# IGNF/MAESTRO

Hardware: AMD Instinct MI355X
Metric: MAE-pretrain tiles/sec (higher is better)
Workload: dtype bf16

## Files before the change

### __graft_entry__.py

```python

from __future__ import annotations

import os
import subprocess
import sys
from pathlib import Path

ROOT = Path(__file__).resolve().parent
if str(ROOT) not in sys.path:
    sys.path.insert(0, str(ROOT))


def build() -> None:
    from maestro_amd.csrc.build import build as build_lib
    from maestro_amd.csrc.build import build_example

    lib = build_lib(verbose=bool(os.environ.get("MAESTRO_BUILD_VERBOSE")))
    build_example()
    import ctypes

    import maestro_amd
    from maestro_amd import hip

    handle = ctypes.CDLL(str(lib))
    import re

    for name in ("maestro_hip.h", "maestro_hip_metrics.h", "maestro_hip_det.h"):
        header = (ROOT / "include" / name).read_text()
        missing = [n for n in re.findall(r"\b(mh_[a-z0-9_]+)\s*\(", header) if not hasattr(handle, n)]
        if missing:
            raise RuntimeError(f"libmaestro_hip.so lacks symbols declared in include/{name}: {sorted(set(missing))}")
    assert hip.lib().mh_version() >= 1


def smoke() -> None:
    import torch

    import maestro_amd.conf as conf
    from maestro_amd.ssl import mae as pmae
    from maestro_amd.train.optim import FusedAdamW
    from oracle import mae as om
    from oracle.gen_golden import build_datasets, case_table, init_weights, make_batch

    if not torch.cuda.is_available():
        raise RuntimeError("smoke() needs cuda:0")
    dev = torch.device("cuda:0")
    case = case_table()["c3_aerial_s2"]
    ds = build_datasets(case, conf)
    kw = dict(interpolate="nearest", model="mae", num_levels=1, fusion_mode=case["fusion"], inter_depth=case["inter_depth"],
              **case["model_kw"])
    oracle = om.build_oracle(ds, conf.MaskConfig(), model_size=case["size"], **kw)
    init_weights(oracle, case["seed"])
    model = getattr(pmae, f"mae_{case['size']}")(datasets=ds, mask=conf.MaskConfig(), **kw)
    model.load_state_dict(oracle.state_dict(), strict=True)
    batch = make_batch(ds.dataset, case["B"], case["seed"], stress=case.get("stress", False))
    eng = model.engine(case["B"], dev, loss="l2_norm")
    torch.manual_seed(7)
    noise, struct = eng.draw_masks()
    loss = eng.forward({k: v.to(dev) for k, v in batch.items()}, noise=noise, struct=struct)
    eng.zero_grad()
    eng.backward()
    pixels, masks = eng.reconstructions()
    ob, orec, omsk, _ = oracle({k: v.clone() for k, v in batch.items()}, "pretrain", noise=noise,
                               struct_masks={g: s[:, :, None] for g, s in struct.items()})
    want = om.compute_loss_rec(ob, orec, omsk, oracle.out_grid_size, om.norm_bands_of(ds.dataset), "l2_norm")
    got = float(loss.item())
    assert abs(got - want.item()) < 3e-3 * abs(want.item()), (got, want.item())
    for m in orec:
        assert torch.equal(masks[m].cpu(), omsk[m]), f"{m}: mask indices differ from the oracle"
        rel = ((pixels[m].cpu() - orec[m]).norm() / orec[m].norm()).item()
        assert rel < 1.3e-2, (m, rel)
    FusedAdamW(eng, 1e-3).step()
    loss2 = float(eng.forward({k: v.to(dev) for k, v in batch.items()}, noise=noise, struct=struct).item())
    assert loss2 < got, (loss2, got)
    print(f"smoke ok: loss hip={got:.6f} oracle={want.item():.6f}; after one AdamW step {loss2:.6f}")


if __name__ == "__main__":
    build()
    if "--smoke" in sys.argv:
        smoke()
```

### maestro_amd/csrc/build.py

```python

from __future__ import annotations

import hashlib
import os
import shutil
import subprocess
import sys
from concurrent.futures import ThreadPoolExecutor
from pathlib import Path

CSRC = Path(__file__).resolve().parent
ROOT = CSRC.parent.parent
LIB_DIR = CSRC.parent / "lib"
LIB = LIB_DIR / "libmaestro_hip.so"
OBJ_DIR = CSRC / "build"
ARCH = "gfx950"
FLAGS = ["-O3", "-std=c++17", "-fPIC", f"--offload-arch={ARCH}", "-Wno-unused-result"] + os.environ.get("MH_BUILD_FLAGS", "").split()
FILE_FLAGS = {"attn.hip": ["-mllvm", "-amdgpu-mfma-vgpr-form", "-fno-slp-vectorize"] + os.environ.get("MH_ATTN_FLAGS", "").split(),
              "gemm_sk.hip": ["-mllvm", "-amdgpu-mfma-vgpr-form"]}
NO_PK_F32 = ["-Xclang", "-target-feature", "-Xclang", "-packed-fp32-ops"]
for _f in ("gemm.hip", "gemm_pp.hip", "gemm_dma.hip"):
    FILE_FLAGS[_f] = FILE_FLAGS.get(_f, []) + NO_PK_F32


def _hipcc() -> str:
    for cand in (shutil.which("hipcc"), "/opt/rocm/bin/hipcc"):
        if cand and Path(cand).exists():
            return cand
    raise RuntimeError("hipcc not found; the MI355X kernels cannot be built")


def _digest(src: Path) -> str:
    h = hashlib.sha256()
    for f in [src, *sorted(CSRC.glob("*.hpp")), ROOT / "include" / "maestro_hip.h",
              ROOT / "include" / "maestro_hip_metrics.h", ROOT / "include" / "maestro_hip_det.h"]:
        h.update(f.read_bytes())
    h.update(" ".join(FLAGS + FILE_FLAGS.get(src.name, [])).encode())
    return h.hexdigest()[:16]


def build(force: bool = False, verbose: bool = False) -> Path:
    hipcc = _hipcc()
    OBJ_DIR.mkdir(exist_ok=True)
    LIB_DIR.mkdir(exist_ok=True)
    sources = sorted(CSRC.glob("*.hip"))
    jobs, objs = [], []
    for src in sources:
        obj = OBJ_DIR / f"{src.stem}.{_digest(src)}.o"
        objs.append(obj)
        if force or not obj.exists():
            for old in OBJ_DIR.glob(f"{src.stem}.*.o"):
                old.unlink()
            jobs.append((src, obj))

    def compile_one(job):
        src, obj = job
        cmd = [hipcc, *FLAGS, *FILE_FLAGS.get(src.name, []), "-c", str(src), "-o", str(obj)]
        if verbose:
            print(" ".join(cmd), flush=True)
        r = subprocess.run(cmd, capture_output=True, text=True)
        if r.returncode != 0:
            raise RuntimeError(f"hipcc failed for {src.name}:\n{r.stdout}\n{r.stderr}")
        return "\n".join(ln for ln in r.stderr.splitlines() if "'-packed-fp32-ops' is not a recognized feature" not in ln)

    if jobs:
        with ThreadPoolExecutor(max_workers=min(4, os.cpu_count() or 1)) as ex:
            for warn in ex.map(compile_one, jobs):
                if verbose and warn:
                    print(warn, file=sys.stderr)
    if jobs or not LIB.exists():
        cmd = [hipcc, "-shared", "-fPIC", f"--offload-arch={ARCH}", *map(str, objs), "-o", str(LIB)]
        r = subprocess.run(cmd, capture_output=True, text=True)
        if r.returncode != 0:
            raise RuntimeError(f"link failed:\n{r.stdout}\n{r.stderr}")
    return LIB


EXAMPLE_SRC = ROOT / "examples" / "abi_smoke.cpp"
EXAMPLE_BIN = ROOT / "examples" / "abi_smoke"


def build_example(force: bool = False) -> Path:
    if not force and EXAMPLE_BIN.exists() and EXAMPLE_BIN.stat().st_mtime >= max(EXAMPLE_SRC.stat().st_mtime, LIB.stat().st_mtime):
        return EXAMPLE_BIN
    cmd = [_hipcc(), "-O2", "-std=c++17", f"--offload-arch={ARCH}", str(EXAMPLE_SRC), f"-I{ROOT / 'include'}", f"-L{LIB_DIR}",
           "-lmaestro_hip", "-Wl,-rpath,$ORIGIN/../maestro_amd/lib", "-o", str(EXAMPLE_BIN)]
    r = subprocess.run(cmd, capture_output=True, text=True)
    if r.returncode != 0:
        raise RuntimeError(f"building examples/abi_smoke failed:\n{r.stdout}\n{r.stderr}")
    return EXAMPLE_BIN


if __name__ == "__main__":
    print(build(force="--force" in sys.argv, verbose=True))
    print(build_example(force="--force" in sys.argv))
```

### maestro_amd/csrc/loss.hip

```cpp
#include "gemm_common.hpp"
#include "../../include/maestro_hip_det.h"

namespace {

template <bool DET>
__global__ __launch_bounds__(256) void masked_loss_kernel(const float* __restrict__ rec, const float* __restrict__ target,
                                                          const uint8_t* __restrict__ mask_group, const int* __restrict__ n_masked,
                                                          float weight, float* __restrict__ acc, bf16_t* __restrict__ drec,
                                                          int B, int Lm, int Lgroup, int tok_off, int PPC, int p, int tgt_C,
                                                          int tgt_c0, int n_g, int denom_is_elems, int rows_per_wave) {
    __shared__ float red[4];
    const int w = threadIdx.x >> 6, lane = threadIdx.x & 63;
    const float coef = weight / (denom_is_elems ? (float)(*n_masked) : (float)(*n_masked) * (float)PPC);
    const bool window = n_g != tgt_C;
    const int tgt_ld = window ? PPC / n_g * tgt_C : PPC;
    float s = 0.f;
    for (int rr = 0; rr < rows_per_wave; ++rr) {
        const int row = (blockIdx.x * 4 + w) * rows_per_wave + rr;
        if (row >= B * Lm) break;
        const int b = row / Lm, t = row - b * Lm;
        const bool masked = mask_group[(size_t)b * Lgroup + tok_off + t] != 0;
        const float* r = rec + (size_t)row * PPC;
        const float* g = target + (size_t)row * tgt_ld;
        bf16_t* d = drec ? drec + (size_t)row * PPC : nullptr;
        for (int c = lane * 4; c < PPC; c += 256) {
            float dd[4] = {0.f, 0.f, 0.f, 0.f};
            if (masked) {
                const f32x4 rv = *reinterpret_cast<const f32x4*>(r + c);
                f32x4 tv;
                if (!window) {
                    tv = *reinterpret_cast<const f32x4*>(g + c);
                } else {
#pragma unroll
                    for (int e = 0; e < 4; ++e) { const int pix = (c + e) / n_g; tv[e] = g[pix * tgt_C + tgt_c0 + (c + e) - pix * n_g]; }
                }
#pragma unroll
                for (int e = 0; e < 4; ++e) {
                    const float diff = rv[e] - tv[e];
                    if (p == 2) { s += diff * diff; dd[e] = 2.f * diff * coef; }
                    else { s += fabsf(diff); dd[e] = (diff > 0.f ? coef : (diff < 0.f ? -coef : 0.f)); }
                }
            }
            if (d) {
                u32x2 pk = {pack_bf2(dd[0], dd[1]), pack_bf2(dd[2], dd[3])};
                *reinterpret_cast<u32x2*>(d + c) = pk;
            }
        }
    }
    s = wave_sum(s);
    if (lane == 0) red[w] = s;
    __syncthreads();
    if (threadIdx.x == 0) {
        const float t = (red[0] + red[1]) + (red[2] + red[3]);
        if constexpr (DET) {
            acc[blockIdx.x] = (blockIdx.x == 0 && *n_masked == 0) ? __builtin_nanf("") : t * coef;
        } else {
        if (t != 0.f) atomicAdd(acc, t * coef);
        if (blockIdx.x == 0 && *n_masked == 0) atomicAdd(acc, __builtin_nanf(""));
        }
    }
}

template <bool DET>
__global__ __launch_bounds__(1024) void colsum_kernel(const void* __restrict__ x, int is_f32, float* __restrict__ out, int M,
                                                      int N, int ld, int rows_per_block) {
    __shared__ f32x4 red[16][64];
    const int w = threadIdx.x >> 6, lane = threadIdx.x & 63, nw = blockDim.x >> 6;
    const int c = (blockIdx.x * 64 + lane) * 4;
    const int r0 = blockIdx.y * rows_per_block, r1 = min(M, r0 + rows_per_block);
    f32x4 acc = {0, 0, 0, 0};
    if (c < N) {
        if (is_f32) {
#pragma unroll 8
            for (int r = r0 + w; r < r1; r += nw)
                acc += *reinterpret_cast<const f32x4*>(reinterpret_cast<const float*>(x) + (size_t)r * ld + c);
        } else {
#pragma unroll 8
            for (int r = r0 + w; r < r1; r += nw) {
                const u32x2 pk = *reinterpret_cast<const u32x2*>(reinterpret_cast<const bf16_t*>(x) + (size_t)r * ld + c);
                acc += (f32x4){__uint_as_float(pk[0] << 16), __uint_as_float(pk[0] & 0xffff0000u),
                               __uint_as_float(pk[1] << 16), __uint_as_float(pk[1] & 0xffff0000u)};
            }
        }
    }
    red[w][lane] = acc;
    __syncthreads();
    if (w == 0 && c < N) {
        f32x4 t = red[0][lane];
        for (int i = 1; i < nw; ++i) t += red[i][lane];
        if constexpr (DET) {
            *reinterpret_cast<f32x4*>(out + (size_t)blockIdx.y * N + c) = t;
        } else {
#pragma unroll
        for (int e = 0; e < 4; ++e) atomicAdd(out + c + e, t[e]);
        }
    }
}

__global__ __launch_bounds__(256) void zero_spans_kernel(float* __restrict__ base, const long* __restrict__ spans) {
    const long off = spans[2 * blockIdx.y], len = spans[2 * blockIdx.y + 1];
    for (long i = ((long)blockIdx.x * 256 + threadIdx.x) * 4; i < len; i += (long)gridDim.x * 1024) {
        float* p = base + off + i;
        if (i + 3 < len && (reinterpret_cast<uintptr_t>(p) & 15) == 0) *reinterpret_cast<f32x4*>(p) = (f32x4){0, 0, 0, 0};
        else for (long e = i; e < min(len, i + 4); ++e) base[off + e] = 0.f;
    }
}

__global__ __launch_bounds__(256) void cast_bf16_kernel(const float* __restrict__ src, bf16_t* __restrict__ dst, long n) {
    const long i = ((long)blockIdx.x * 256 + threadIdx.x) * 4;
    if (i + 3 < n) {
        const f32x4 v = *reinterpret_cast<const f32x4*>(src + i);
        u32x2 pk = {pack_bf2(v[0], v[1]), pack_bf2(v[2], v[3])};
        *reinterpret_cast<u32x2*>(dst + i) = pk;
    } else {
        for (long j = i; j < n; ++j) dst[j] = f2bf(src[j]);
    }
}

__global__ __launch_bounds__(256) void pack_rows_kernel(const float* __restrict__ w, bf16_t* __restrict__ dst, int E, int K, int Kpad) {
    const long i = (long)blockIdx.x * 256 + threadIdx.x;
    if (i >= (long)E * Kpad) return;
    const int e = i / Kpad, k = i - (long)e * Kpad;
    dst[i] = k < K ? f2bf(w[(size_t)e * K + k]) : (bf16_t)0;
}

__global__ __launch_bounds__(256) void unpack_rows_add_kernel(const float* __restrict__ src, float* __restrict__ dst, int E, int K, int Kpad) {
    const long i = (long)blockIdx.x * 256 + threadIdx.x;
    if (i >= (long)E * K) return;
    const int e = i / K, k = i - (long)e * K;
    atomicAdd(dst + i, src[(size_t)e * Kpad + k]);
}

struct Fp8Shadow { uint8_t* p8; const short* slot_map; const float* scale; float* amax; };

__device__ __forceinline__ int adamw_update(float* __restrict__ p, const float* __restrict__ g, float* __restrict__ m,
                                             float* __restrict__ v, bf16_t* __restrict__ pb, long n, float lr, float b1, float b2,
                                             float eps, float wd, float bc1, float bc2_sqrt, float gscale,
                                             Fp8Shadow f8 = Fp8Shadow{nullptr, nullptr, nullptr, nullptr},
                                             float* amax_out = nullptr) {
    const long i = ((long)blockIdx.x * 256 + threadIdx.x) * 4;
    if (i >= n) return -1;
    const f32x4 gv = __builtin_nontemporal_load(reinterpret_cast<const f32x4*>(g + i)) * gscale;
    f32x4 pv = __builtin_nontemporal_load(reinterpret_cast<const f32x4*>(p + i));
    f32x4 mv = __builtin_nontemporal_load(reinterpret_cast<const f32x4*>(m + i));
    f32x4 vv = __builtin_nontemporal_load(reinterpret_cast<const f32x4*>(v + i));
#pragma unroll
    for (int e = 0; e < 4; ++e) {
        pv[e] *= 1.f - lr * wd;
        mv[e] = b1 * mv[e] + (1.f - b1) * gv[e];
        vv[e] = b2 * vv[e] + (1.f - b2) * gv[e] * gv[e];
        const float denom = sqrtf(vv[e]) / bc2_sqrt + eps;
        pv[e] -= (lr / bc1) * (mv[e] / denom);
    }
    __builtin_nontemporal_store(pv, reinterpret_cast<f32x4*>(p + i));
    __builtin_nontemporal_store(mv, reinterpret_cast<f32x4*>(m + i));
    __builtin_nontemporal_store(vv, reinterpret_cast<f32x4*>(v + i));
    if (pb) {
        u32x2 pk = {pack_bf2(pv[0], pv[1]), pack_bf2(pv[2], pv[3])};
        __builtin_nontemporal_store(pk, reinterpret_cast<u32x2*>(pb + i));
    }
    if (f8.p8) {
        const int slot = f8.slot_map[i >> 6];
        if (slot >= 0) {
            const float s8 = f8.scale[slot];
            float mx = 0.f;
#pragma unroll
            for (int e = 0; e < 4; ++e) mx = amax_fold(mx, pv[e]);
            __builtin_nontemporal_store(pack_e4m3x4(pv, s8), reinterpret_cast<uint32_t*>(f8.p8 + i));
            *amax_out = mx;
            return slot;
        }
    }
    return -1;
}
__global__ __launch_bounds__(256) void adamw_kernel(float* __restrict__ p, const float* __restrict__ g, float* __restrict__ m,
                                                    float* __restrict__ v, bf16_t* __restrict__ pb, long n, float lr, float b1,
                                                    float b2, float eps, float wd, float bc1, float bc2_sqrt, float gscale) {
    adamw_update(p, g, m, v, pb, n, lr, b1, b2, eps, wd, bc1, bc2_sqrt, gscale);
}
__global__ __launch_bounds__(256) void adamw_fp8_kernel(float* __restrict__ p, const float* __restrict__ g, float* __restrict__ m,
                                                        float* __restrict__ v, bf16_t* __restrict__ pb, long n, float lr, float b1,
                                                        float b2, float eps, float wd, float bc1, float bc2_sqrt, float gscale,
                                                        Fp8Shadow f8) {
    __shared__ float red_mx[4];
    __shared__ int red_slot[4];
    float mx = 0.f;
    const int slot = adamw_update(p, g, m, v, pb, n, lr, b1, b2, eps, wd, bc1, bc2_sqrt, gscale, f8, &mx);
    const int w = threadIdx.x >> 6;
    const int slot0 = __builtin_amdgcn_readfirstlane(slot);
    const bool uniform = __all(slot == slot0);
    if (uniform) {
        mx = wave_amax(mx);
    } else if (slot >= 0 && amax_nonzero(mx)) {
        atomic_max_pos(f8.amax + (size_t)slot * MH_FP8_AMAX_PITCH, mx);
    }
    if ((threadIdx.x & 63) == 0) { red_mx[w] = uniform ? mx : 0.f; red_slot[w] = uniform ? slot0 : -1; }
    __syncthreads();
    if (threadIdx.x == 0) {
        if (red_slot[0] == red_slot[1] && red_slot[0] == red_slot[2] && red_slot[0] == red_slot[3]) {
            const float m4 = amax_fold(amax_fold(amax_fold(red_mx[0], red_mx[1]), red_mx[2]), red_mx[3]);
            if (red_slot[0] >= 0 && amax_nonzero(m4)) atomic_max_pos(f8.amax + (size_t)red_slot[0] * MH_FP8_AMAX_PITCH, m4);
        } else {
            for (int k = 0; k < 4; ++k)
                if (red_slot[k] >= 0 && amax_nonzero(red_mx[k])) atomic_max_pos(f8.amax + (size_t)red_slot[k] * MH_FP8_AMAX_PITCH, red_mx[k]);
        }
    }
}
__global__ __launch_bounds__(256) void adamw_dev_kernel(float* __restrict__ p, const float* __restrict__ g, float* __restrict__ m,
                                                        float* __restrict__ v, bf16_t* __restrict__ pb, long n, float b1, float b2,
                                                        float eps, float wd, const float* __restrict__ hyper) {
    if (hyper[4] == 0.f) return;
    adamw_update(p, g, m, v, pb, n, hyper[0], b1, b2, eps, wd, hyper[1], hyper[2], hyper[3]);
}

__global__ __launch_bounds__(256) void scale_dev_kernel(float* __restrict__ x, long n, const float* __restrict__ scale) {
    const float s = *scale;
    if (s == 1.f) return;
    const long i = ((long)blockIdx.x * 256 + threadIdx.x) * 4;
    if (i + 4 <= n) {
        *reinterpret_cast<f32x4*>(x + i) = *reinterpret_cast<const f32x4*>(x + i) * s;
    } else {
        for (long j = i; j < n; ++j) x[j] *= s;
    }
}

}

static int loss_rows_per_wave(long rows) { return (int)std::min(16L, std::max(1L, rows / 4096)); }

extern "C" int mh_scale_dev(float* x, long n, const float* scale, void* stream) {
    MH_CHECK_ARG(x && scale && n > 0 && ((uintptr_t)x % 16) == 0, "mh_scale_dev: bad arguments (x 16-byte aligned)");
    hipLaunchKernelGGL(scale_dev_kernel, dim3(ceil_div(n, 1024)), dim3(256), 0, (hipStream_t)stream, x, n, scale);
    MH_LAUNCH_CHECK();
    return 0;
}

extern "C" int mh_masked_loss(const float* rec, const float* target, const uint8_t* mask_group, const int* n_masked,
                              float weight, float* acc, void* drec, int B, int Lm, int Lgroup, int tok_off, int PPC, int p,
                              void* stream) {
    MH_CHECK_ARG(rec && target && mask_group && n_masked && acc, "mh_masked_loss: null pointer");
    MH_CHECK_ARG((p == 1 || p == 2) && PPC % 4 == 0 && tok_off + Lm <= Lgroup, "mh_masked_loss: bad arguments");
    const int rpw = loss_rows_per_wave((long)B * Lm);
    hipLaunchKernelGGL(masked_loss_kernel<false>, dim3(ceil_div((long)B * Lm, 4 * rpw)), dim3(256), 0, (hipStream_t)stream, rec, target, mask_group, n_masked,
                       weight, acc, (bf16_t*)drec, B, Lm, Lgroup, tok_off, PPC, p, 1, 0, 1, 0, rpw);
    MH_LAUNCH_CHECK();
    return 0;
}

extern "C" int mh_masked_loss_bands(const float* rec, const float* target, const uint8_t* mask_group, const int* n_elems,
                                    float weight, float* acc, void* drec, int B, int Lm, int Lgroup, int tok_off, int PPC, int p,
                                    int tgt_C, int tgt_c0, int n_g, void* stream) {
    MH_CHECK_ARG(rec && target && mask_group && n_elems && acc, "mh_masked_loss_bands: null pointer");
    MH_CHECK_ARG((p == 1 || p == 2) && PPC % 4 == 0 && tok_off + Lm <= Lgroup, "mh_masked_loss_bands: bad arguments");
    MH_CHECK_ARG(n_g > 0 && PPC % n_g == 0 && tgt_c0 >= 0 && tgt_c0 + n_g <= tgt_C, "mh_masked_loss_bands: band window [%d, %d) of %d",
                 tgt_c0, tgt_c0 + n_g, tgt_C);
    const int rpw = loss_rows_per_wave((long)B * Lm);
    hipLaunchKernelGGL(masked_loss_kernel<false>, dim3(ceil_div((long)B * Lm, 4 * rpw)), dim3(256), 0, (hipStream_t)stream, rec, target, mask_group, n_elems,
                       weight, acc, (bf16_t*)drec, B, Lm, Lgroup, tok_off, PPC, p, tgt_C, tgt_c0, n_g, 1, rpw);
    MH_LAUNCH_CHECK();
    return 0;
}

extern "C" int mh_masked_loss_partial_size(int B, int Lm) {
    const long rows = (long)B * Lm;
    return rows > 0 ? ceil_div(rows, 4 * loss_rows_per_wave(rows)) : 0;
}

extern "C" int mh_masked_loss_det(const float* rec, const float* target, const uint8_t* mask_group, const int* n_masked,
                                  float weight, float* loss_partial, void* drec, int B, int Lm, int Lgroup, int tok_off, int PPC,
                                  int p, void* stream) {
    MH_CHECK_ARG(rec && target && mask_group && n_masked && loss_partial, "mh_masked_loss_det: null pointer");
    MH_CHECK_ARG(B > 0 && Lm > 0 && (p == 1 || p == 2) && PPC % 4 == 0 && tok_off + Lm <= Lgroup, "mh_masked_loss_det: bad arguments");
    const int rpw = loss_rows_per_wave((long)B * Lm);
    hipLaunchKernelGGL(masked_loss_kernel<true>, dim3(ceil_div((long)B * Lm, 4 * rpw)), dim3(256), 0, (hipStream_t)stream, rec, target,
                       mask_group, n_masked, weight, loss_partial, (bf16_t*)drec, B, Lm, Lgroup, tok_off, PPC, p, 1, 0, 1, 0, rpw);
    MH_LAUNCH_CHECK();
    return 0;
}

extern "C" int mh_masked_loss_bands_det(const float* rec, const float* target, const uint8_t* mask_group, const int* n_elems,
                                        float weight, float* loss_partial, void* drec, int B, int Lm, int Lgroup, int tok_off,
                                        int PPC, int p, int tgt_C, int tgt_c0, int n_g, void* stream) {
    MH_CHECK_ARG(rec && target && mask_group && n_elems && loss_partial, "mh_masked_loss_bands_det: null pointer");
    MH_CHECK_ARG(B > 0 && Lm > 0 && (p == 1 || p == 2) && PPC % 4 == 0 && tok_off + Lm <= Lgroup, "mh_masked_loss_bands_det: bad arguments");
    MH_CHECK_ARG(n_g > 0 && PPC % n_g == 0 && tgt_c0 >= 0 && tgt_c0 + n_g <= tgt_C, "mh_masked_loss_bands_det: band window [%d, %d) of %d",
                 tgt_c0, tgt_c0 + n_g, tgt_C);
    const int rpw = loss_rows_per_wave((long)B * Lm);
    hipLaunchKernelGGL(masked_loss_kernel<true>, dim3(ceil_div((long)B * Lm, 4 * rpw)), dim3(256), 0, (hipStream_t)stream, rec, target,
                       mask_group, n_elems, weight, loss_partial, (bf16_t*)drec, B, Lm, Lgroup, tok_off, PPC, p, tgt_C, tgt_c0, n_g, 1, rpw);
    MH_LAUNCH_CHECK();
    return 0;
}

extern "C" int mh_colsum_partial_rows(int M) { return M > 0 ? ceil_div(M, MH_COLSUM_PARTIAL_ROWS) : 0; }

extern "C" int mh_colsum_partial(const void* x, int x_is_f32, float* partial, int M, int N, int ld, void* stream) {
    MH_CHECK_ARG(x && partial && ((uintptr_t)partial % 16) == 0, "mh_colsum_partial: null pointer / partial not 16-byte aligned");
    MH_CHECK_ARG(M > 0 && N > 0 && N % 4 == 0 && ld % 4 == 0 && N <= ld, "mh_colsum_partial: bad sizes M=%d N=%d ld=%d", M, N, ld);
    hipLaunchKernelGGL(colsum_kernel<true>, dim3(ceil_div(N, 256), ceil_div(M, MH_COLSUM_PARTIAL_ROWS)), dim3(1024), 0,
                       (hipStream_t)stream, x, x_is_f32, partial, M, N, ld, MH_COLSUM_PARTIAL_ROWS);
    MH_LAUNCH_CHECK();
    return 0;
}

extern "C" int mh_colsum(const void* x, int x_is_f32, float* out, int M, int N, int ld, void* stream) {
    MH_CHECK_ARG(x && out && N % 4 == 0 && ld % 4 == 0, "mh_colsum: bad arguments");
    const int col_blocks = ceil_div(N, 256);
    int rows_per_block = 1024;
    while (rows_per_block > 128 && (long)col_blocks * ceil_div(M, rows_per_block) < 128) rows_per_block >>= 1;
    hipLaunchKernelGGL(colsum_kernel<false>, dim3(col_blocks, ceil_div(M, rows_per_block)), dim3(1024), 0, (hipStream_t)stream, x,
                       x_is_f32, out, M, N, ld, rows_per_block);
    MH_LAUNCH_CHECK();
    return 0;
}

extern "C" int mh_zero_spans(float* base, const long* spans_device, int n_spans, long max_len, void* stream) {
    MH_CHECK_ARG(base && spans_device && n_spans > 0 && max_len > 0, "mh_zero_spans: bad arguments");
    dim3 grid((unsigned)min(64L, (max_len + 1023) / 1024), n_spans);
    hipLaunchKernelGGL(zero_spans_kernel, grid, dim3(256), 0, (hipStream_t)stream, base, spans_device);
    MH_LAUNCH_CHECK();
    return 0;
}

extern "C" int mh_cast_bf16(const float* src, void* dst, long n, void* stream) {
    MH_CHECK_ARG(src && dst && n > 0, "mh_cast_bf16: bad arguments");
    hipLaunchKernelGGL(cast_bf16_kernel, dim3(ceil_div(n, 1024)), dim3(256), 0, (hipStream_t)stream, src, (bf16_t*)dst, n);
    MH_LAUNCH_CHECK();
    return 0;
}

extern "C" int mh_pack_rows_bf16(const float* w, void* dst, int E, int K, int Kpad, void* stream) {
    MH_CHECK_ARG(w && dst && Kpad >= K, "mh_pack_rows_bf16: bad arguments");
    hipLaunchKernelGGL(pack_rows_kernel, dim3(ceil_div((long)E * Kpad, 256)), dim3(256), 0, (hipStream_t)stream, w, (bf16_t*)dst, E, K, Kpad);
    MH_LAUNCH_CHECK();
    return 0;
}

extern "C" int mh_unpack_rows_add(const float* src, float* dst, int E, int K, int Kpad, void* stream) {
    MH_CHECK_ARG(src && dst && Kpad >= K, "mh_unpack_rows_add: bad arguments");
    hipLaunchKernelGGL(unpack_rows_add_kernel, dim3(ceil_div((long)E * K, 256)), dim3(256), 0, (hipStream_t)stream, src, dst, E, K, Kpad);
    MH_LAUNCH_CHECK();
    return 0;
}

extern "C" int mh_adamw(float* p, const float* g, float* m, float* v, void* p_bf16, long n, float lr, float b1, float b2,
                        float eps, float wd, int step, float grad_scale, void* stream) {
    MH_CHECK_ARG(p && g && m && v && n > 0 && n % 4 == 0 && step >= 1, "mh_adamw: bad arguments (n %% 4 == 0, step >= 1)");
    const float bc1 = 1.f - powf(b1, (float)step);
    const float bc2_sqrt = sqrtf(1.f - powf(b2, (float)step));
    hipLaunchKernelGGL(adamw_kernel, dim3(ceil_div(n, 1024)), dim3(256), 0, (hipStream_t)stream, p, g, m, v, (bf16_t*)p_bf16, n, lr,
                       b1, b2, eps, wd, bc1, bc2_sqrt, grad_scale);
    MH_LAUNCH_CHECK();
    return 0;
}

extern "C" int mh_adamw_fp8(float* p, const float* g, float* m, float* v, void* p_bf16, void* p_fp8, const short* slot_map,
                            const float* scale, float* amax, long n, float lr, float b1, float b2, float eps, float wd, int step,
                            float grad_scale, void* stream) {
    MH_CHECK_ARG(p && g && m && v && n > 0 && n % 4 == 0 && step >= 1, "mh_adamw_fp8: bad arguments (n %% 4 == 0, step >= 1)");
    MH_CHECK_ARG(p_fp8 && slot_map && scale && amax && ((uintptr_t)p_fp8 % 4) == 0, "mh_adamw_fp8: fp8 shadow, slot map, scale and amax tables are required");
    const float bc1 = 1.f - powf(b1, (float)step);
    const float bc2_sqrt = sqrtf(1.f - powf(b2, (float)step));
    hipLaunchKernelGGL(adamw_fp8_kernel, dim3(ceil_div(n, 1024)), dim3(256), 0, (hipStream_t)stream, p, g, m, v, (bf16_t*)p_bf16, n, lr,
                       b1, b2, eps, wd, bc1, bc2_sqrt, grad_scale, Fp8Shadow{(uint8_t*)p_fp8, slot_map, scale, amax});
    MH_LAUNCH_CHECK();
    return 0;
}

extern "C" int mh_adamw_dev(float* p, const float* g, float* m, float* v, void* p_bf16, long n, float b1, float b2, float eps,
                            float wd, const float* hyper, void* stream) {
    MH_CHECK_ARG(p && g && m && v && hyper && n > 0 && n % 4 == 0, "mh_adamw_dev: bad arguments (n %% 4 == 0)");
    hipLaunchKernelGGL(adamw_dev_kernel, dim3(ceil_div(n, 1024)), dim3(256), 0, (hipStream_t)stream, p, g, m, v, (bf16_t*)p_bf16,
                       n, b1, b2, eps, wd, hyper);
    MH_LAUNCH_CHECK();
    return 0;
}
```

### maestro_amd/csrc/mask.hip

```cpp
#include "common.hpp"
#include "../../include/maestro_hip.h"

namespace {

__global__ __launch_bounds__(1024) void mask_select_kernel(const float* __restrict__ noise, const uint8_t* __restrict__ smask,
                                                          int* __restrict__ visible_idx, int* __restrict__ masked_idx,
                                                          int* __restrict__ inv, uint8_t* __restrict__ mask, int L, int k) {
    extern __shared__ __attribute__((aligned(16))) float sm[];
    const int L4 = (L + 3) & ~3;
    int* wtot = reinterpret_cast<int*>(sm + L4);
    const int b = blockIdx.x, lane = threadIdx.x & 63, w = threadIdx.x >> 6;
    for (int i = threadIdx.x; i < L4; i += 1024) {
        float v = INFINITY;
        if (i < L) {
            v = noise[(size_t)b * L + i];
            if (smask && smask[(size_t)b * L + i]) v = 0.f;
        }
        sm[i] = v;
    }
    __syncthreads();
    int base = 0;
    for (int i0 = 0; i0 < L; i0 += 1024) {
        const int i = i0 + threadIdx.x;
        int f = 0;
        if (i < L) {
            const float v = sm[i];
            int r = 0;
            for (int j = 0; j < L4; j += 4) {
                const f32x4 u = *reinterpret_cast<const f32x4*>(sm + j);
                r += (int)((u[0] < v) | ((u[0] == v) & (j < i)));
                r += (int)((u[1] < v) | ((u[1] == v) & (j + 1 < i)));
                r += (int)((u[2] < v) | ((u[2] == v) & (j + 2 < i)));
                r += (int)((u[3] < v) | ((u[3] == v) & (j + 3 < i)));
            }
            f = r < k;
        }
        const unsigned long long bal = __ballot(f);
        const int before = __popcll(bal & ((1ull << lane) - 1ull));
        __syncthreads();
        if (lane == 0) wtot[w] = __popcll(bal);
        __syncthreads();
        int nm = base + before, tot = 0;
#pragma unroll
        for (int x = 0; x < 16; ++x) {
            const int c = wtot[x];
            nm += x < w ? c : 0;
            tot += c;
        }
        base += tot;
        if (i < L) {
            mask[(size_t)b * L + i] = (uint8_t)f;
            if (f) {
                masked_idx[(size_t)b * k + nm] = i;
                inv[(size_t)b * L + i] = -1;
            } else {
                visible_idx[(size_t)b * (L - k) + (i - nm)] = i;
                inv[(size_t)b * L + i] = i - nm;
            }
        }
    }
}

__global__ __launch_bounds__(256) void gather_rows_kernel(const float* __restrict__ src, const int* __restrict__ idx,
                                                          float* __restrict__ dst, int B, int src_L, int n_idx, int dim,
                                                          int dst_L, int dst_off) {
    const int row = blockIdx.x * 4 + (threadIdx.x >> 6), lane = threadIdx.x & 63;
    if (row >= B * n_idx) return;
    const int b = row / n_idx, j = row - b * n_idx;
    const float* s = src + ((size_t)b * src_L + idx[row]) * dim;
    float* d = dst + ((size_t)b * dst_L + dst_off + j) * dim;
    for (int c = lane * 4; c < dim; c += 256) *reinterpret_cast<f32x4*>(d + c) = *reinterpret_cast<const f32x4*>(s + c);
}

__global__ __launch_bounds__(256) void scatter_rows_kernel(const float* __restrict__ ddst, const int* __restrict__ idx,
                                                           float* __restrict__ dsrc, int B, int src_L, int n_idx, int dim,
                                                           int dst_L, int dst_off) {
    const int row = blockIdx.x * 4 + (threadIdx.x >> 6), lane = threadIdx.x & 63;
    if (row >= B * n_idx) return;
    const int b = row / n_idx, j = row - b * n_idx;
    float* s = dsrc + ((size_t)b * src_L + idx[row]) * dim;
    const float* d = ddst + ((size_t)b * dst_L + dst_off + j) * dim;
    for (int c = lane * 4; c < dim; c += 256) *reinterpret_cast<f32x4*>(s + c) = *reinterpret_cast<const f32x4*>(d + c);
}

__global__ __launch_bounds__(256) void expand_rows_kernel(const float* __restrict__ src, const int* __restrict__ inv,
                                                          float* __restrict__ dst, int B, int L, int n, int dim) {
    const int row = blockIdx.x * 4 + (threadIdx.x >> 6), lane = threadIdx.x & 63;
    if (row >= B * L) return;
    const int b = row / L, iv = inv[row];
    float* o = dst + (size_t)row * dim;
    const float* s = src + ((size_t)b * n + (iv < 0 ? 0 : iv)) * dim;
    for (int c = lane * 4; c < dim; c += 256) {
        f32x4 v = {0.f, 0.f, 0.f, 0.f};
        if (iv >= 0) v = *reinterpret_cast<const f32x4*>(s + c);
        *reinterpret_cast<f32x4*>(o + c) = v;
    }
}

__global__ __launch_bounds__(256) void unmask_kernel(const float* __restrict__ y, const int* __restrict__ inv,
                                                     const float* __restrict__ mask_token, const int* __restrict__ tok_slot,
                                                     const float* __restrict__ pos, const float* __restrict__ date,
                                                     const int* __restrict__ date_row, int n_date_rows,
                                                     float* __restrict__ xdec, int B, int L, int n_vis, int Dd, int slot_stride) {
    const int row = blockIdx.x * 4 + (threadIdx.x >> 6), lane = threadIdx.x & 63;
    if (row >= B * L) return;
    const int b = row / L, t = row - b * L;
    const int iv = inv[row];
    const float* s = iv < 0 ? mask_token + (size_t)tok_slot[(size_t)b * slot_stride + t] * Dd : y + ((size_t)b * n_vis + iv) * Dd;
    const float* pr = pos + (size_t)t * Dd;
    const float* dr = date ? date + ((size_t)b * n_date_rows + date_row[t]) * 8 : nullptr;
    float* o = xdec + (size_t)row * Dd;
    for (int c = lane * 4; c < Dd; c += 256) {
        f32x4 v = *reinterpret_cast<const f32x4*>(s + c) + *reinterpret_cast<const f32x4*>(pr + c);
        if (dr && c >= Dd - 8) v += *reinterpret_cast<const f32x4*>(dr + (c - (Dd - 8)));
        *reinterpret_cast<f32x4*>(o + c) = v;
    }
}

constexpr int UM_ROWS = 512, UM_NT = 1024;
template <bool DET>
__global__ __launch_bounds__(UM_NT) void unmask_bwd_token_kernel(const float* __restrict__ dxdec, const uint8_t* __restrict__ mask,
                                                                 const int* __restrict__ tok_slot, float* __restrict__ dmask_token,
                                                                 int B, int L, int Dd, int slot, int t_lo, int t_hi, int slot_stride) {
    __shared__ __attribute__((aligned(16))) float red[UM_NT * 4];
    __shared__ int row_off[UM_ROWS];
    const int span = t_hi - t_lo, total = B * span;
    const int cols = Dd >> 2, lanes = UM_NT / cols;
    const int col = threadIdx.x % cols, sub = threadIdx.x / cols;
    const int r0 = blockIdx.x * UM_ROWS;
    for (int rr = threadIdx.x; rr < UM_ROWS; rr += UM_NT) {
        const int r = r0 + rr;
        int off = -1;
        if (r < total) {
            const int b = r / span, t = t_lo + (r - b * span);
            if (mask[(size_t)b * L + t] && tok_slot[(size_t)b * slot_stride + t] == slot) off = b * L + t;
        }
        row_off[rr] = off;
    }
    __syncthreads();
    f32x4 acc = {0, 0, 0, 0};
    if (sub < lanes) {
#pragma unroll 2
        for (int rr = sub; rr < UM_ROWS; rr += 4 * lanes) {
            f32x4 v[4];
#pragma unroll
            for (int u = 0; u < 4; ++u) {
                v[u] = (f32x4){0, 0, 0, 0};
                const int ri = rr + u * lanes;
                const int off = ri < UM_ROWS ? row_off[ri] : -1;
                if (off >= 0) v[u] = *reinterpret_cast<const f32x4*>(dxdec + (size_t)off * Dd + 4 * col);
            }
            acc += (v[0] + v[1]) + (v[2] + v[3]);
        }
    }
    *reinterpret_cast<f32x4*>(red + 4 * threadIdx.x) = acc;
    __syncthreads();
    if (sub == 0) {
        for (int s = 1; s < lanes; ++s) acc += *reinterpret_cast<const f32x4*>(red + 4 * (s * cols + col));
        if constexpr (DET) {
            *reinterpret_cast<f32x4*>(dmask_token + (size_t)blockIdx.x * Dd + 4 * col) = acc;
        } else {
#pragma unroll
        for (int e = 0; e < 4; ++e) if (acc[e] != 0.f) atomicAdd(dmask_token + 4 * col + e, acc[e]);
        }
    }
}

__global__ __launch_bounds__(1024) void count_masked_kernel(const uint8_t* __restrict__ mask, int B, int L, int t_lo, int t_hi,
                                                            int* __restrict__ out, int mult, int accumulate) {
    __shared__ float red[16];
    const int span = t_hi - t_lo, w = threadIdx.x >> 6, lane = threadIdx.x & 63;
    float c = 0.f;
    for (int b = w; b < B; b += 16) {
        const uint8_t* row = mask + (size_t)b * L + t_lo;
        for (int t = lane; t < span; t += 64) c += row[t] ? 1.f : 0.f;
    }
    c = block_sum<16>(c, red);
    if (threadIdx.x == 0) *out = (accumulate ? *out : 0) + (int)(c + 0.5f) * mult;
}

}

extern "C" int mh_mask_select(const float* noise, const uint8_t* struct_mask, int* visible_idx, int* masked_idx, int* inv,
                              uint8_t* mask, int B, int L, int k, void* stream) {
    MH_CHECK_ARG(noise && visible_idx && masked_idx && inv && mask, "mh_mask_select: null pointer");
    MH_CHECK_ARG(B > 0 && L > 0 && k >= 0 && k <= L && L <= 8192, "mh_mask_select: bad sizes B=%d L=%d k=%d", B, L, k);
    hipLaunchKernelGGL(mask_select_kernel, dim3(B), dim3(1024), (size_t)((L + 3) & ~3) * 4 + 64, (hipStream_t)stream, noise, struct_mask,
                       visible_idx, masked_idx, inv, mask, L, k);
    MH_LAUNCH_CHECK();
    return 0;
}

extern "C" int mh_gather_rows(const float* src, const int* idx, float* dst, int B, int src_L, int n_idx, int dim, int dst_L,
                              int dst_off, void* stream) {
    MH_CHECK_ARG(src && idx && dst && dim % 4 == 0 && dst_off + n_idx <= dst_L, "mh_gather_rows: bad arguments");
    hipLaunchKernelGGL(gather_rows_kernel, dim3(ceil_div((long)B * n_idx, 4)), dim3(256), 0, (hipStream_t)stream, src, idx, dst, B,
                       src_L, n_idx, dim, dst_L, dst_off);
    MH_LAUNCH_CHECK();
    return 0;
}

extern "C" int mh_scatter_rows(const float* ddst, const int* idx, float* dsrc, int B, int src_L, int n_idx, int dim,
                               int dst_L, int dst_off, void* stream) {
    MH_CHECK_ARG(ddst && idx && dsrc && dim % 4 == 0 && dst_off + n_idx <= dst_L, "mh_scatter_rows: bad arguments");
    hipLaunchKernelGGL(scatter_rows_kernel, dim3(ceil_div((long)B * n_idx, 4)), dim3(256), 0, (hipStream_t)stream, ddst, idx, dsrc,
                       B, src_L, n_idx, dim, dst_L, dst_off);
    MH_LAUNCH_CHECK();
    return 0;
}

extern "C" int mh_expand_rows(const float* src, const int* inv, float* dst, int B, int L, int n, int dim, void* stream) {
    MH_CHECK_ARG(src && inv && dst && B > 0 && L > 0 && n > 0 && dim % 4 == 0, "mh_expand_rows: bad arguments");
    hipLaunchKernelGGL(expand_rows_kernel, dim3(ceil_div((long)B * L, 4)), dim3(256), 0, (hipStream_t)stream, src, inv, dst, B, L,
                       n, dim);
    MH_LAUNCH_CHECK();
    return 0;
}

extern "C" int mh_unmask_assemble(const float* y, const int* inv, const float* mask_token, const int* tok_slot,
                                  const float* pos, const float* date, const int* date_row, int n_date_rows, float* xdec,
                                  int B, int L, int n_vis, int Dd, void* stream) {
    MH_CHECK_ARG(y && inv && mask_token && tok_slot && pos && xdec && Dd % 4 == 0 && Dd >= 8, "mh_unmask_assemble: bad arguments");
    MH_CHECK_ARG(!date || date_row, "mh_unmask_assemble: date without date_row");
    hipLaunchKernelGGL(unmask_kernel, dim3(ceil_div((long)B * L, 4)), dim3(256), 0, (hipStream_t)stream, y, inv, mask_token,
                       tok_slot, pos, date, date_row, n_date_rows, xdec, B, L, n_vis, Dd, 0);
    MH_LAUNCH_CHECK();
    return 0;
}

extern "C" int mh_unmask_assemble_per_sample(const float* y, const int* inv, const float* mask_token, const int* tok_slot_bl,
                                             const float* pos, const float* date, const int* date_row, int n_date_rows,
                                             float* xdec, int B, int L, int n_vis, int Dd, void* stream) {
    MH_CHECK_ARG(y && inv && mask_token && tok_slot_bl && pos && xdec && Dd % 4 == 0 && Dd >= 8, "mh_unmask_assemble_per_sample: bad arguments");
    MH_CHECK_ARG(!date || date_row, "mh_unmask_assemble_per_sample: date without date_row");
    hipLaunchKernelGGL(unmask_kernel, dim3(ceil_div((long)B * L, 4)), dim3(256), 0, (hipStream_t)stream, y, inv, mask_token,
                       tok_slot_bl, pos, date, date_row, n_date_rows, xdec, B, L, n_vis, Dd, L);
    MH_LAUNCH_CHECK();
    return 0;
}

extern "C" int mh_unmask_token_grad(const float* dxdec, const uint8_t* mask, const int* tok_slot, float* dmask_token, int B,
                                    int L, int Dd, int slot, int t_lo, int t_hi, void* stream) {
    MH_CHECK_ARG(dxdec && mask && tok_slot && dmask_token && Dd % 4 == 0 && Dd <= 1024, "mh_unmask_token_grad: bad arguments");
    MH_CHECK_ARG(0 <= t_lo && t_lo < t_hi && t_hi <= L, "mh_unmask_token_grad: bad token range");
    hipLaunchKernelGGL(unmask_bwd_token_kernel<false>, dim3(ceil_div((long)B * (t_hi - t_lo), UM_ROWS)), dim3(UM_NT), 0,
                       (hipStream_t)stream, dxdec, mask, tok_slot, dmask_token, B, L, Dd, slot, t_lo, t_hi, 0);
    MH_LAUNCH_CHECK();
    return 0;
}

extern "C" int mh_unmask_token_grad_per_sample(const float* dxdec, const uint8_t* mask, const int* tok_slot_bl, float* dmask_token,
                                               int B, int L, int Dd, int slot, void* stream) {
    MH_CHECK_ARG(dxdec && mask && tok_slot_bl && dmask_token && Dd % 4 == 0 && Dd <= 1024 && B > 0 && L > 0,
                 "mh_unmask_token_grad_per_sample: bad arguments");
    hipLaunchKernelGGL(unmask_bwd_token_kernel<false>, dim3(ceil_div((long)B * L, UM_ROWS)), dim3(UM_NT), 0, (hipStream_t)stream, dxdec, mask,
                       tok_slot_bl, dmask_token, B, L, Dd, slot, 0, L, L);
    MH_LAUNCH_CHECK();
    return 0;
}

extern "C" int mh_unmask_token_grad_partial_rows(long n_rows) { return n_rows > 0 ? ceil_div(n_rows, UM_ROWS) : 0; }

extern "C" int mh_unmask_token_grad_det(const float* dxdec, const uint8_t* mask, const int* tok_slot, float* partial, int B, int L,
                                        int Dd, int slot, int t_lo, int t_hi, void* stream) {
    MH_CHECK_ARG(dxdec && mask && tok_slot && partial && ((uintptr_t)partial % 16) == 0 && B > 0 && Dd > 0 && Dd % 4 == 0 && Dd <= 1024,
                 "mh_unmask_token_grad_det: bad arguments");
    MH_CHECK_ARG(0 <= t_lo && t_lo < t_hi && t_hi <= L, "mh_unmask_token_grad_det: bad token range");
    hipLaunchKernelGGL(unmask_bwd_token_kernel<true>, dim3(ceil_div((long)B * (t_hi - t_lo), UM_ROWS)), dim3(UM_NT), 0,
                       (hipStream_t)stream, dxdec, mask, tok_slot, partial, B, L, Dd, slot, t_lo, t_hi, 0);
    MH_LAUNCH_CHECK();
    return 0;
}

extern "C" int mh_unmask_token_grad_per_sample_det(const float* dxdec, const uint8_t* mask, const int* tok_slot_bl, float* partial,
                                                   int B, int L, int Dd, int slot, void* stream) {
    MH_CHECK_ARG(dxdec && mask && tok_slot_bl && partial && ((uintptr_t)partial % 16) == 0 && Dd > 0 && Dd % 4 == 0 && Dd <= 1024 &&
                 B > 0 && L > 0, "mh_unmask_token_grad_per_sample_det: bad arguments");
    hipLaunchKernelGGL(unmask_bwd_token_kernel<true>, dim3(ceil_div((long)B * L, UM_ROWS)), dim3(UM_NT), 0, (hipStream_t)stream, dxdec,
                       mask, tok_slot_bl, partial, B, L, Dd, slot, 0, L, L);
    MH_LAUNCH_CHECK();
    return 0;
}

extern "C" int mh_count_masked_elems(const uint8_t* mask, int B, int L, int t_lo, int t_hi, int* out, int mult, int accumulate,
                                     void* stream) {
    MH_CHECK_ARG(mask && out && 0 <= t_lo && t_lo < t_hi && t_hi <= L && mult > 0, "mh_count_masked_elems: bad arguments");
    hipLaunchKernelGGL(count_masked_kernel, dim3(1), dim3(1024), 0, (hipStream_t)stream, mask, B, L, t_lo, t_hi, out, mult,
                       accumulate);
    MH_LAUNCH_CHECK();
    return 0;
}

extern "C" int mh_count_masked(const uint8_t* mask, int B, int L, int t_lo, int t_hi, int* out, void* stream) {
    MH_CHECK_ARG(mask && out && 0 <= t_lo && t_lo < t_hi && t_hi <= L, "mh_count_masked: bad arguments");
    hipLaunchKernelGGL(count_masked_kernel, dim3(1), dim3(1024), 0, (hipStream_t)stream, mask, B, L, t_lo, t_hi, out, 1, 0);
    MH_LAUNCH_CHECK();
    return 0;
}
```

### maestro_amd/csrc/norm.hip

```cpp
#include "gemm_common.hpp"

namespace {

struct RowMap { int L, off; };
__device__ __forceinline__ size_t map_row(RowMap m, int b, int j) { return (size_t)b * m.L + m.off + j; }

template <int NV>
__global__ __launch_bounds__(256) void ln_fwd_kernel(const float* __restrict__ x, RowMap xm, const float* __restrict__ gamma,
                                                     const float* __restrict__ beta, void* __restrict__ y, RowMap ym,
                                                     int y_is_f32, float* __restrict__ mean, float* __restrict__ rstd,
                                                     int B, int n, int dim, float eps, uint8_t* __restrict__ y8,
                                                     const float* __restrict__ y8_scale, float* __restrict__ y8_amax,
                                                     uint8_t* __restrict__ y8s, int ld_y8s) {
    const int row = blockIdx.x * 4 + (threadIdx.x >> 6);
    const int lane = threadIdx.x & 63;
    if (row >= B * n) return;
    const int b = row / n, j = row - b * n;
    const float* xr = x + map_row(xm, b, j) * dim;
    const int nv = dim >> 2;
    f32x4 v[NV];
    float s = 0.f;
#pragma unroll
    for (int i = 0; i < NV; ++i) {
        const int c = lane + 64 * i;
        v[i] = (f32x4){0, 0, 0, 0};
        if (c < nv) v[i] = *reinterpret_cast<const f32x4*>(xr + 4 * c);
        s += (v[i][0] + v[i][1]) + (v[i][2] + v[i][3]);
    }
    const float mu = wave_sum(s) / dim;
    float q = 0.f;
#pragma unroll
    for (int i = 0; i < NV; ++i) {
        if (lane + 64 * i < nv) {
#pragma unroll
            for (int e = 0; e < 4; ++e) { const float d = v[i][e] - mu; q += d * d; }
        }
    }
    const float rs = rsqrtf(wave_sum(q) / dim + eps);
    if (lane == 0) { mean[row] = mu; rstd[row] = rs; }
    const size_t yrow = map_row(ym, b, j) * dim;
    const bool t8 = y8 && !y8s;
    const float s8 = t8 ? *y8_scale : 0.f;
    float amax8 = 0.f;
#pragma unroll
    for (int i = 0; i < NV; ++i) {
        const int c = lane + 64 * i;
        u32x2 pk16 = {0u, 0u};
        if (c < nv) {
            const f32x4 g = *reinterpret_cast<const f32x4*>(gamma + 4 * c);
            const f32x4 bt = *reinterpret_cast<const f32x4*>(beta + 4 * c);
            f32x4 o;
#pragma unroll
            for (int e = 0; e < 4; ++e) o[e] = (v[i][e] - mu) * rs * g[e] + bt[e];
            if (y_is_f32) {
                *reinterpret_cast<f32x4*>(reinterpret_cast<float*>(y) + yrow + 4 * c) = o;
            } else {
                u32x2 pk = {pack_bf2(o[0], o[1]), pack_bf2(o[2], o[3])};
                *reinterpret_cast<u32x2*>(reinterpret_cast<bf16_t*>(y) + yrow + 4 * c) = pk;
                pk16 = pk;
            }
            if (t8) {
#pragma unroll
                for (int e = 0; e < 4; ++e) amax8 = amax_fold(amax8, o[e]);
                *reinterpret_cast<uint32_t*>(y8 + yrow + 4 * c) = pack_e4m3x4(o, s8);
            }
        }
        if (y8s) {
            const f32x4 q = bf2x2_to_f32x4(pk16[0], pk16[1]);
            float a = 0.f;
#pragma unroll
            for (int e = 0; e < 4; ++e) a = amax_fold(a, q[e]);
            const uint32_t sbyte = mx_scale_byte(group_amax<8>(a));
            if (c < nv) {
                *reinterpret_cast<uint32_t*>(y8 + yrow + 4 * c) = pack_e4m3x4(q, mx_inv_scale(sbyte));
                if ((lane & 7) == 0) y8s[map_row(ym, b, j) * ld_y8s + (c >> 3)] = (uint8_t)sbyte;
            }
        }
    }
    if (t8 && y8_amax) {
        amax8 = wave_amax(amax8);
        if (lane == 0 && amax_nonzero(amax8)) atomic_max_pos(y8_amax, amax8);
    }
}

#ifndef MH_LN_FAST
#define MH_LN_FAST 1
#endif
#ifndef MH_LN_DPP
#define MH_LN_DPP 1
#endif
__device__ __forceinline__ float ln_wave_sum(float v) {
#if MH_LN_DPP
#define MH_ROR(n) __builtin_bit_cast(float, __builtin_amdgcn_update_dpp(0, __builtin_bit_cast(int, v), 0x120 + (n), 0xf, 0xf, false))
    v += MH_ROR(8); v += MH_ROR(4); v += MH_ROR(2); v += MH_ROR(1);
#undef MH_ROR
    const int iv = __builtin_bit_cast(int, v);
    const float r0 = __builtin_bit_cast(float, __builtin_amdgcn_readlane(iv, 0)), r1 = __builtin_bit_cast(float, __builtin_amdgcn_readlane(iv, 16));
    const float r2 = __builtin_bit_cast(float, __builtin_amdgcn_readlane(iv, 32)), r3 = __builtin_bit_cast(float, __builtin_amdgcn_readlane(iv, 48));
    return (r0 + r1) + (r2 + r3);
#else
    return wave_sum(v);
#endif
}
enum { LN_Y8_NONE = 0, LN_Y8_TENSOR = 1, LN_Y8_MX = 2 };
template <int NV, int Y8>
__device__ __forceinline__ void ln_fwd_fast_body(const float* __restrict__ x, RowMap xm, const float* __restrict__ gamma,
                                                          const float* __restrict__ beta, bf16_t* __restrict__ y, RowMap ym,
                                                          float* __restrict__ mean, float* __restrict__ rstd, int B, int n,
                                                          float eps, uint8_t* __restrict__ y8, const float* __restrict__ y8_scale,
                                                          float* __restrict__ y8_amax, uint8_t* __restrict__ y8s, int ld_y8s) {
    constexpr int dim = 256 * NV;
    constexpr bool FP8 = Y8 == LN_Y8_TENSOR;
    const int row = blockIdx.x * 4 + __builtin_amdgcn_readfirstlane(threadIdx.x >> 6);
    const int lane = threadIdx.x & 63;
    if (row >= B * n) return;
    const int b = row / n, j = row - b * n;
    const float* xr = x + map_row(xm, b, j) * dim;
    f32x4 v[NV], g[NV], bt[NV];
#pragma unroll
    for (int i = 0; i < NV; ++i) v[i] = *reinterpret_cast<const f32x4*>(xr + 4 * (lane + 64 * i));
#pragma unroll
    for (int i = 0; i < NV; ++i) {
        g[i] = *reinterpret_cast<const f32x4*>(gamma + 4 * (lane + 64 * i));
        bt[i] = *reinterpret_cast<const f32x4*>(beta + 4 * (lane + 64 * i));
    }
    float s = 0.f;
#pragma unroll
    for (int i = 0; i < NV; ++i) s += (v[i][0] + v[i][1]) + (v[i][2] + v[i][3]);
    const float mu = ln_wave_sum(s) / dim;
    float q = 0.f;
#pragma unroll
    for (int i = 0; i < NV; ++i) {
#pragma unroll
        for (int e = 0; e < 4; ++e) { const float d = v[i][e] - mu; q += d * d; }
    }
    const float rs = rsqrtf(ln_wave_sum(q) / dim + eps);
    const size_t yrow = map_row(ym, b, j) * dim;
    bf16_t* yr = y + yrow;
    float s8 = 0.f;
    if constexpr (FP8) s8 = *y8_scale;
    float amax8 = 0.f;
#pragma unroll
    for (int i = 0; i < NV; ++i) {
        f32x4 o;
#pragma unroll
        for (int e = 0; e < 4; ++e) o[e] = (v[i][e] - mu) * rs * g[i][e] + bt[i][e];
        const u32x2 pk = {pack_bf2(o[0], o[1]), pack_bf2(o[2], o[3])};
        *reinterpret_cast<u32x2*>(yr + 4 * (lane + 64 * i)) = pk;
        if constexpr (Y8 == LN_Y8_MX) {
            const f32x4 q = bf2x2_to_f32x4(pk[0], pk[1]);
            float a = 0.f;
#pragma unroll
            for (int e = 0; e < 4; ++e) a = amax_fold(a, q[e]);
            const uint32_t sbyte = mx_scale_byte(group_amax<8>(a));
            *reinterpret_cast<uint32_t*>(y8 + yrow + 4 * (lane + 64 * i)) = pack_e4m3x4(q, mx_inv_scale(sbyte));
            if ((lane & 7) == 0) y8s[map_row(ym, b, j) * ld_y8s + ((lane + 64 * i) >> 3)] = (uint8_t)sbyte;
        }
        if constexpr (FP8) {
#pragma unroll
            for (int e = 0; e < 4; ++e) amax8 = amax_fold(amax8, o[e]);
            *reinterpret_cast<uint32_t*>(y8 + yrow + 4 * (lane + 64 * i)) = pack_e4m3x4(o, s8);
        }
    }
    if (lane == 0) { mean[row] = mu; rstd[row] = rs; }
    if constexpr (FP8) {
        if (y8_amax) {
            amax8 = wave_amax(amax8);
            if (lane == 0 && amax_nonzero(amax8)) atomic_max_pos(y8_amax, amax8);
        }
    }
}
template <int NV, bool FP8>
__global__ __launch_bounds__(256) void ln_fwd_fast_kernel(const float* __restrict__ x, RowMap xm, const float* __restrict__ gamma,
                                                          const float* __restrict__ beta, bf16_t* __restrict__ y, RowMap ym,
                                                          float* __restrict__ mean, float* __restrict__ rstd, int B, int n,
                                                          float eps, uint8_t* __restrict__ y8, const float* __restrict__ y8_scale,
                                                          float* __restrict__ y8_amax) {
    ln_fwd_fast_body<NV, FP8 ? LN_Y8_TENSOR : LN_Y8_NONE>(x, xm, gamma, beta, y, ym, mean, rstd, B, n, eps, y8, y8_scale, y8_amax,
                                                          nullptr, 0);
}
template <int NV>
__global__ __launch_bounds__(256) void ln_fwd_fast_mx_kernel(const float* __restrict__ x, RowMap xm, const float* __restrict__ gamma,
                                                             const float* __restrict__ beta, bf16_t* __restrict__ y, RowMap ym,
                                                             float* __restrict__ mean, float* __restrict__ rstd, int B, int n,
                                                             float eps, uint8_t* __restrict__ y8, uint8_t* __restrict__ y8s,
                                                             int ld_y8s) {
    ln_fwd_fast_body<NV, LN_Y8_MX>(x, xm, gamma, beta, y, ym, mean, rstd, B, n, eps, y8, nullptr, nullptr, y8s, ld_y8s);
}

#ifndef LN_ROWS
#define LN_ROWS 4
#endif
constexpr int ROWS_PER_WAVE = LN_ROWS;

template <int NV>
__global__ __launch_bounds__(256) void ln_bwd_kernel(const void* __restrict__ dy, RowMap dym, int dy_is_f32,
                                                     const float* __restrict__ x, RowMap xm,
                                                     const float* __restrict__ gamma, const float* __restrict__ mean,
                                                     const float* __restrict__ rstd, const float* __restrict__ dres,
                                                     float* __restrict__ dx, bf16_t* __restrict__ dx_bf16,
                                                     float* __restrict__ partial, int B, int n, int dim) {
    extern __shared__ __attribute__((aligned(16))) float red[];
    const int w = threadIdx.x >> 6, lane = threadIdx.x & 63;
    const int nv = dim >> 2;
    f32x4 gsum[NV], bsum[NV], csum[NV], gm[NV];
#pragma unroll
    for (int i = 0; i < NV; ++i) {
        gsum[i] = (f32x4){0, 0, 0, 0}; bsum[i] = (f32x4){0, 0, 0, 0}; csum[i] = (f32x4){0, 0, 0, 0};
        const int c = lane + 64 * i;
        gm[i] = c < nv ? *reinterpret_cast<const f32x4*>(gamma + 4 * c) : (f32x4){0, 0, 0, 0};
    }
    const int row0 = (blockIdx.x * 4 + w) * ROWS_PER_WAVE;
    const int rows = B * n;
    f32x4 xv_n[NV], rs_n[NV];
    u32x4 dy_n[NV];
    float mu_n = 0.f, rstd_n = 0.f;
    size_t xrow_n = 0;
    auto fetch = [&](int row) {
        const int b = row / n, j = row - b * n;
        xrow_n = map_row(xm, b, j) * dim;
        const size_t dyrow = map_row(dym, b, j) * dim;
        mu_n = mean[row]; rstd_n = rstd[row];
#pragma unroll
        for (int i = 0; i < NV; ++i) {
            const int c = lane + 64 * i;
            if (c < nv) {
                xv_n[i] = *reinterpret_cast<const f32x4*>(x + xrow_n + 4 * c);
                if (dy_is_f32) {
                    dy_n[i] = *reinterpret_cast<const u32x4*>(reinterpret_cast<const float*>(dy) + dyrow + 4 * c);
                } else {
                    const u32x2 pk = *reinterpret_cast<const u32x2*>(reinterpret_cast<const bf16_t*>(dy) + dyrow + 4 * c);
                    dy_n[i] = (u32x4){pk[0], pk[1], 0u, 0u};
                }
                rs_n[i] = dres ? *reinterpret_cast<const f32x4*>(dres + xrow_n + 4 * c) : (f32x4){0, 0, 0, 0};
            }
        }
    };
    if (row0 < rows) fetch(row0);
    for (int rr = 0; rr < ROWS_PER_WAVE; ++rr) {
        const int row = row0 + rr;
        if (row >= rows) break;
        const size_t xrow = xrow_n;
        const float mu = mu_n, rs = rstd_n;
        f32x4 xh[NV], dz[NV], rsd[NV];
        u32x4 dyv[NV];
#pragma unroll
        for (int i = 0; i < NV; ++i) { xh[i] = xv_n[i]; dyv[i] = dy_n[i]; rsd[i] = rs_n[i]; }
        if (rr + 1 < ROWS_PER_WAVE && row + 1 < rows) fetch(row + 1);
        float s1 = 0.f, s2 = 0.f;
#pragma unroll
        for (int i = 0; i < NV; ++i) {
            const int c = lane + 64 * i;
            const f32x4 xv = xh[i];
            xh[i] = (f32x4){0, 0, 0, 0}; dz[i] = (f32x4){0, 0, 0, 0};
            if (c < nv) {
                f32x4 d;
                if (dy_is_f32) {
                    d = __builtin_bit_cast(f32x4, dyv[i]);
                } else {
                    d = (f32x4){__uint_as_float(dyv[i][0] << 16), __uint_as_float(dyv[i][0] & 0xffff0000u),
                                __uint_as_float(dyv[i][1] << 16), __uint_as_float(dyv[i][1] & 0xffff0000u)};
                }
#pragma unroll
                for (int e = 0; e < 4; ++e) {
                    xh[i][e] = (xv[e] - mu) * rs;
                    dz[i][e] = d[e] * gm[i][e];
                    s1 += dz[i][e];
                    s2 += dz[i][e] * xh[i][e];
                    gsum[i][e] += d[e] * xh[i][e];
                    bsum[i][e] += d[e];
                }
            }
        }
        const float c1 = wave_sum(s1) / dim, c2 = wave_sum(s2) / dim;
#pragma unroll
        for (int i = 0; i < NV; ++i) {
            const int c = lane + 64 * i;
            if (c < nv) {
                f32x4 o;
#pragma unroll
                for (int e = 0; e < 4; ++e) o[e] = rs * (dz[i][e] - c1 - xh[i][e] * c2);
                o += rsd[i];
                csum[i] += o;
                *reinterpret_cast<f32x4*>(dx + xrow + 4 * c) = o;
                if (dx_bf16) {
                    u32x2 pk = {pack_bf2(o[0], o[1]), pack_bf2(o[2], o[3])};
                    *reinterpret_cast<u32x2*>(dx_bf16 + xrow + 4 * c) = pk;
                }
            }
        }
    }
    if (!partial) return;
    float* rg = red + (size_t)w * 3 * dim;
#pragma unroll
    for (int i = 0; i < NV; ++i) {
        const int c = lane + 64 * i;
        if (c < nv) {
            *reinterpret_cast<f32x4*>(rg + 4 * c) = gsum[i];
            *reinterpret_cast<f32x4*>(rg + dim + 4 * c) = bsum[i];
            *reinterpret_cast<f32x4*>(rg + 2 * dim + 4 * c) = csum[i];
        }
    }
    __syncthreads();
    float* prow = partial + (size_t)blockIdx.x * 3 * dim;
    for (int c = threadIdx.x; c < 3 * dim; c += 256)
        prow[c] = red[c] + red[3 * dim + c] + red[6 * dim + c] + red[9 * dim + c];
}

template <int NV, int DEPTH>
__global__ __launch_bounds__(256) void ln_bwd_fast_kernel(const bf16_t* __restrict__ dy, RowMap dym, const float* __restrict__ x,
                                                          RowMap xm, const float* __restrict__ gamma,
                                                          const float* __restrict__ mean, const float* __restrict__ rstd,
                                                          const float* __restrict__ dres, float* __restrict__ dx,
                                                          bf16_t* __restrict__ dx_bf16, float* __restrict__ partial, int B, int n) {
    constexpr int dim = 256 * NV;
    static_assert(DEPTH >= 1 && DEPTH <= ROWS_PER_WAVE, "prefetch distance in rows");
    extern __shared__ __attribute__((aligned(16))) float red[];
    const int w = __builtin_amdgcn_readfirstlane(threadIdx.x >> 6), lane = threadIdx.x & 63;
    f32x4 gsum[NV], bsum[NV], csum[NV], gm[NV];
#pragma unroll
    for (int i = 0; i < NV; ++i) {
        gsum[i] = (f32x4){0, 0, 0, 0}; bsum[i] = (f32x4){0, 0, 0, 0}; csum[i] = (f32x4){0, 0, 0, 0};
        gm[i] = *reinterpret_cast<const f32x4*>(gamma + 4 * (lane + 64 * i));
    }
    const int row0 = (blockIdx.x * 4 + w) * ROWS_PER_WAVE;
    if (row0 < B * n) {
        f32x4 xq[ROWS_PER_WAVE][NV], rq[ROWS_PER_WAVE][NV];
        u32x2 dq[ROWS_PER_WAVE][NV];
        float muq[ROWS_PER_WAVE], rsq[ROWS_PER_WAVE];
        size_t xrowq[ROWS_PER_WAVE];
        auto fetch = [&](int p) {
            const int row = row0 + p, b = row / n, j = row - b * n;
            xrowq[p] = map_row(xm, b, j) * dim;
            const size_t dyrow = map_row(dym, b, j) * dim;
            muq[p] = mean[row]; rsq[p] = rstd[row];
#pragma unroll
            for (int i = 0; i < NV; ++i) {
                const int c4 = 4 * (lane + 64 * i);
                xq[p][i] = *reinterpret_cast<const f32x4*>(x + xrowq[p] + c4);
                dq[p][i] = *reinterpret_cast<const u32x2*>(dy + dyrow + c4);
                rq[p][i] = *reinterpret_cast<const f32x4*>(dres + xrowq[p] + c4);
            }
        };
#pragma unroll
        for (int p = 0; p < DEPTH; ++p) fetch(p);
#pragma unroll
        for (int rr = 0; rr < ROWS_PER_WAVE; ++rr) {
            if (rr + DEPTH < ROWS_PER_WAVE) fetch(rr + DEPTH);
            __builtin_amdgcn_sched_barrier(0);
            const float mu = muq[rr], rs = rsq[rr];
            f32x4 xh[NV], dz[NV];
            float s1 = 0.f, s2 = 0.f;
#pragma unroll
            for (int i = 0; i < NV; ++i) {
                const u32x2 pk = dq[rr][i];
                const f32x4 d = {__uint_as_float(pk[0] << 16), __uint_as_float(pk[0] & 0xffff0000u),
                                 __uint_as_float(pk[1] << 16), __uint_as_float(pk[1] & 0xffff0000u)};
#pragma unroll
                for (int e = 0; e < 4; ++e) {
                    xh[i][e] = (xq[rr][i][e] - mu) * rs;
                    dz[i][e] = d[e] * gm[i][e];
                    s1 += dz[i][e];
                    s2 += dz[i][e] * xh[i][e];
                    gsum[i][e] += d[e] * xh[i][e];
                    bsum[i][e] += d[e];
                }
            }
            const float c1 = ln_wave_sum(s1) / dim, c2 = ln_wave_sum(s2) / dim;
#pragma unroll
            for (int i = 0; i < NV; ++i) {
                const int c4 = 4 * (lane + 64 * i);
                f32x4 o;
#pragma unroll
                for (int e = 0; e < 4; ++e) o[e] = rs * (dz[i][e] - c1 - xh[i][e] * c2);
                o += rq[rr][i];
                csum[i] += o;
                *reinterpret_cast<f32x4*>(dx + xrowq[rr] + c4) = o;
                const u32x2 pk = {pack_bf2(o[0], o[1]), pack_bf2(o[2], o[3])};
                *reinterpret_cast<u32x2*>(dx_bf16 + xrowq[rr] + c4) = pk;
            }
            __builtin_amdgcn_sched_barrier(0);
        }
    }
    if (!partial) return;
    float* rg = red + (size_t)w * 3 * dim;
#pragma unroll
    for (int i = 0; i < NV; ++i) {
        const int c4 = 4 * (lane + 64 * i);
        *reinterpret_cast<f32x4*>(rg + c4) = gsum[i];
        *reinterpret_cast<f32x4*>(rg + dim + c4) = bsum[i];
        *reinterpret_cast<f32x4*>(rg + 2 * dim + c4) = csum[i];
    }
    __syncthreads();
    float* prow = partial + (size_t)blockIdx.x * 3 * dim;
    for (int c = threadIdx.x; c < 3 * dim; c += 256)
        prow[c] = red[c] + red[3 * dim + c] + red[6 * dim + c] + red[9 * dim + c];
}

#ifndef LN_BWD_DEPTH
#define LN_BWD_DEPTH 4
#endif
constexpr int RED_ROWS = 8;
__global__ __launch_bounds__(256) void ln_bwd_reduce_kernel(const float* __restrict__ partial, int nblk, int dim,
                                                            float* __restrict__ dgamma, float* __restrict__ dbeta,
                                                            float* __restrict__ dcol) {
    const int c = blockIdx.x * 256 + threadIdx.x;
    if (c >= 3 * dim) return;
    const int r0 = blockIdx.y * RED_ROWS, r1 = min(nblk, r0 + RED_ROWS);
    float s = 0.f;
    for (int r = r0; r < r1; ++r) s += partial[(size_t)r * 3 * dim + c];
    if (c < dim) atomicAdd(dgamma + c, s);
    else if (c < 2 * dim) atomicAdd(dbeta + (c - dim), s);
    else if (dcol) atomicAdd(dcol + (c - 2 * dim), s);
}

__global__ __launch_bounds__(256) void colsum_batched_kernel(const MhColsumJob* __restrict__ jobs, int n_jobs,
                                                             const uint64_t* __restrict__ blocks) {
    const uint64_t e = blocks[blockIdx.x];
    const int ji = (int)(e >> 48);
    if (ji >= n_jobs) return;
    const MhColsumJob j = jobs[ji];
    const int c = (int)((e >> 32) & 0xFFFF) * 256 + threadIdx.x;
    const int r0 = (int)(e & 0xFFFFFFFFu) * MH_COLSUM_ROWS;
    if (c >= j.cols || r0 >= j.rows) return;
    const int r1 = min(j.rows, r0 + MH_COLSUM_ROWS);
    const float* src = j.src + (size_t)r0 * j.ld + c;
    float v[MH_COLSUM_ROWS];
#pragma unroll
    for (int i = 0; i < MH_COLSUM_ROWS; ++i) v[i] = r0 + i < r1 ? src[(size_t)i * j.ld] : 0.f;
    float s = 0.f;
#pragma unroll
    for (int i = 0; i < MH_COLSUM_ROWS; ++i) s += v[i];
    atomicAdd(j.dst + c, s);
}

}

static int ln_nv(int dim) { const int v = (dim / 4 + 63) / 64; return v <= 4 ? v : 8; }

static int layernorm_fwd_impl(const float* x, int x_L, int x_off, const float* gamma, const float* beta, void* y, int y_L,
                              int y_off, int y_is_f32, float* mean, float* rstd, int B, int n, int dim, float eps, void* y8,
                              const float* y8_scale, float* y8_amax, void* stream, void* y8s, int ld_y8s);

extern "C" int mh_layernorm_fwd(const float* x, int x_L, int x_off, const float* gamma, const float* beta, void* y,
                                int y_L, int y_off, int y_is_f32, float* mean, float* rstd, int B, int n, int dim,
                                float eps, void* stream) {
    return layernorm_fwd_impl(x, x_L, x_off, gamma, beta, y, y_L, y_off, y_is_f32, mean, rstd, B, n, dim, eps, nullptr, nullptr,
                              nullptr, stream, nullptr, 0);
}

extern "C" int mh_layernorm_fwd_fp8(const float* x, int x_L, int x_off, const float* gamma, const float* beta, void* y,
                                    int y_L, int y_off, float* mean, float* rstd, int B, int n, int dim, float eps, void* y8,
                                    const float* y8_scale, float* y8_amax, void* stream) {
    MH_CHECK_ARG(y8 && y8_scale && ((uintptr_t)y8 % 4) == 0, "mh_layernorm_fwd_fp8: y8 (4-byte aligned) and its scale are required");
    return layernorm_fwd_impl(x, x_L, x_off, gamma, beta, y, y_L, y_off, 0, mean, rstd, B, n, dim, eps, y8, y8_scale, y8_amax, stream,
                              nullptr, 0);
}

extern "C" int mh_layernorm_fwd_mx(const float* x, int x_L, int x_off, const float* gamma, const float* beta, void* y, int y_L,
                                   int y_off, float* mean, float* rstd, int B, int n, int dim, float eps, void* y8, void* y8_scales,
                                   int ld_y8s, void* stream) {
    MH_CHECK_ARG(y8 && ((uintptr_t)y8 % 4) == 0, "mh_layernorm_fwd_mx: y8 (4-byte aligned) is required");
    MH_CHECK_ARG(y8_scales, "mh_layernorm_fwd_mx: null scale pointer (y8_scales)");
    MH_CHECK_ARG(ld_y8s % 4 == 0 && ld_y8s >= dim / 32, "mh_layernorm_fwd_mx: ld_y8s must be a multiple of 4 and >= dim / 32 (%d)", ld_y8s);
    return layernorm_fwd_impl(x, x_L, x_off, gamma, beta, y, y_L, y_off, 0, mean, rstd, B, n, dim, eps, y8, nullptr, nullptr, stream,
                              y8_scales, ld_y8s);
}

static int layernorm_fwd_impl(const float* x, int x_L, int x_off, const float* gamma, const float* beta, void* y, int y_L,
                              int y_off, int y_is_f32, float* mean, float* rstd, int B, int n, int dim, float eps, void* y8,
                              const float* y8_scale, float* y8_amax, void* stream, void* y8s, int ld_y8s) {
    MH_CHECK_ARG(x && gamma && beta && y && mean && rstd, "mh_layernorm_fwd: null pointer");
    MH_CHECK_ARG(dim % 4 == 0 && dim >= 4 && dim <= 2048, "mh_layernorm_fwd: dim %d unsupported", dim);
    MH_CHECK_ARG(B > 0 && n > 0 && x_off + n <= x_L && y_off + n <= y_L, "mh_layernorm_fwd: bad row map");
    const int rows = B * n;
    dim3 grid(ceil_div(rows, 4)), block(256);
    hipStream_t s = (hipStream_t)stream;
#define LN_FWD(NV) hipLaunchKernelGGL(ln_fwd_kernel<NV>, grid, block, 0, s, x, RowMap{x_L, x_off}, gamma, beta, y, \
                                      RowMap{y_L, y_off}, y_is_f32, mean, rstd, B, n, dim, eps, (uint8_t*)y8, y8_scale, y8_amax, \
                                      (uint8_t*)y8s, ld_y8s)
#define LN_FWD_FAST_(NV, FP8) hipLaunchKernelGGL((ln_fwd_fast_kernel<NV, FP8>), grid, block, 0, s, x, RowMap{x_L, x_off}, gamma, beta, \
                                                 (bf16_t*)y, RowMap{y_L, y_off}, mean, rstd, B, n, eps, (uint8_t*)y8, y8_scale, y8_amax)
#define LN_FWD_FAST_MX(NV) hipLaunchKernelGGL((ln_fwd_fast_mx_kernel<NV>), grid, block, 0, s, x, RowMap{x_L, x_off}, gamma, beta, \
                                              (bf16_t*)y, RowMap{y_L, y_off}, mean, rstd, B, n, eps, (uint8_t*)y8, (uint8_t*)y8s, ld_y8s)
#define LN_FWD_FAST(NV) do { if (y8s) LN_FWD_FAST_MX(NV); else if (y8) LN_FWD_FAST_(NV, true); else LN_FWD_FAST_(NV, false); } while (0)
    const int nvs = ln_nv(dim);
    MH_CHECK_ARG(!y8s || (dim % 32 == 0 && !y_is_f32), "mh_layernorm_fwd_mx: dim %% 32 == 0 required, got %d", dim);
    if (MH_LN_FAST && nvs <= 4 && dim == 256 * nvs && !y_is_f32) {
        switch (nvs) { case 1: LN_FWD_FAST(1); break; case 2: LN_FWD_FAST(2); break; case 3: LN_FWD_FAST(3); break;
                       default: LN_FWD_FAST(4); }
    } else {
        switch (nvs) { case 1: LN_FWD(1); break; case 2: LN_FWD(2); break; case 3: LN_FWD(3); break;
                       case 4: LN_FWD(4); break; default: LN_FWD(8); }
    }
#undef LN_FWD_FAST
#undef LN_FWD_FAST_MX
#undef LN_FWD_FAST_
#undef LN_FWD
    MH_LAUNCH_CHECK();
    return 0;
}

extern "C" long mh_layernorm_bwd_workspace(int rows, int dim) {
    return (long)ceil_div(rows, 4 * ROWS_PER_WAVE) * 3 * dim;
}

static int layernorm_bwd_impl(const void* dy, int dy_L, int dy_off, int dy_is_f32, const float* x, int x_L, int x_off,
                              const float* gamma, const float* mean, const float* rstd, const float* dres, float* dx,
                              void* dx_bf16, float* dgamma, float* dbeta, float* dcol, float* workspace, bool partial_only,
                              int B, int n, int dim, void* stream) {
    const int rows = B * n, nblk = ceil_div(rows, 4 * ROWS_PER_WAVE);
    const size_t lds = (size_t)4 * 3 * dim * sizeof(float);
    dim3 grid(nblk), block(256);
    hipStream_t s = (hipStream_t)stream;
    float* part = (dgamma || partial_only) ? workspace : nullptr;
#define LN_BWD(NV) hipLaunchKernelGGL(ln_bwd_kernel<NV>, grid, block, lds, s, dy, RowMap{dy_L, dy_off}, dy_is_f32, x, \
                                      RowMap{x_L, x_off}, gamma, mean, rstd, dres, dx, (bf16_t*)dx_bf16, part, B, n, dim)
#define LN_BWD_FAST(NV, DEPTH) hipLaunchKernelGGL((ln_bwd_fast_kernel<NV, DEPTH>), grid, block, lds, s, (const bf16_t*)dy, \
                                                  RowMap{dy_L, dy_off}, x, RowMap{x_L, x_off}, gamma, mean, rstd, dres, dx, \
                                                  (bf16_t*)dx_bf16, part, B, n)
    const int nvs = ln_nv(dim);
    if (MH_LN_FAST && nvs <= 4 && dim == 256 * nvs && !dy_is_f32 && dres && dx_bf16 && rows % ROWS_PER_WAVE == 0) {
        constexpr int DEPTH = LN_BWD_DEPTH < ROWS_PER_WAVE ? LN_BWD_DEPTH : ROWS_PER_WAVE, DEPTH4 = 2 < ROWS_PER_WAVE ? 2 : ROWS_PER_WAVE;
        switch (nvs) { case 1: LN_BWD_FAST(1, DEPTH); break; case 2: LN_BWD_FAST(2, DEPTH); break;
                       case 3: LN_BWD_FAST(3, DEPTH); break; default: LN_BWD_FAST(4, DEPTH4); }
    } else {
        switch (nvs) { case 1: LN_BWD(1); break; case 2: LN_BWD(2); break; case 3: LN_BWD(3); break;
                       case 4: LN_BWD(4); break; default: LN_BWD(8); }
    }
#undef LN_BWD_FAST
#undef LN_BWD
    if (dgamma && !partial_only)
        hipLaunchKernelGGL(ln_bwd_reduce_kernel, dim3(ceil_div(3 * dim, 256), ceil_div(nblk, RED_ROWS)), dim3(256), 0, s,
                           workspace, nblk, dim, dgamma, dbeta, dcol);
    MH_LAUNCH_CHECK();
    return 0;
}

extern "C" int mh_layernorm_bwd(const void* dy, int dy_L, int dy_off, int dy_is_f32, const float* x, int x_L, int x_off,
                                const float* gamma, const float* mean, const float* rstd, const float* dres, float* dx,
                                void* dx_bf16, float* dgamma, float* dbeta, float* dcol, float* workspace, int B, int n,
                                int dim, void* stream) {
    MH_CHECK_ARG(dy && x && gamma && mean && rstd && dx, "mh_layernorm_bwd: null pointer");
    MH_CHECK_ARG((dgamma == nullptr) == (dbeta == nullptr), "mh_layernorm_bwd: dgamma/dbeta must come together");
    MH_CHECK_ARG(!dgamma || workspace, "mh_layernorm_bwd: parameter gradients need the workspace");
    MH_CHECK_ARG(!dcol || dgamma, "mh_layernorm_bwd: dcol needs dgamma/dbeta");
    MH_CHECK_ARG(dim % 4 == 0 && dim >= 4 && dim <= 2048, "mh_layernorm_bwd: dim %d unsupported", dim);
    MH_CHECK_ARG(B > 0 && n > 0 && x_off + n <= x_L && dy_off + n <= dy_L, "mh_layernorm_bwd: bad row map");
    return layernorm_bwd_impl(dy, dy_L, dy_off, dy_is_f32, x, x_L, x_off, gamma, mean, rstd, dres, dx, dx_bf16, dgamma, dbeta, dcol,
                              workspace, false, B, n, dim, stream);
}

extern "C" int mh_layernorm_bwd_partial(const void* dy, int dy_L, int dy_off, int dy_is_f32, const float* x, int x_L, int x_off,
                                        const float* gamma, const float* mean, const float* rstd, const float* dres, float* dx,
                                        void* dx_bf16, float* workspace, int B, int n, int dim, void* stream) {
    MH_CHECK_ARG(dy && x && gamma && mean && rstd && dx && workspace, "mh_layernorm_bwd_partial: null pointer");
    MH_CHECK_ARG(dim % 4 == 0 && dim >= 4 && dim <= 2048, "mh_layernorm_bwd_partial: dim %d unsupported", dim);
    MH_CHECK_ARG(B > 0 && n > 0 && x_off + n <= x_L && dy_off + n <= dy_L, "mh_layernorm_bwd_partial: bad row map");
    return layernorm_bwd_impl(dy, dy_L, dy_off, dy_is_f32, x, x_L, x_off, gamma, mean, rstd, dres, dx, dx_bf16, nullptr, nullptr,
                              nullptr, workspace, true, B, n, dim, stream);
}

extern "C" int mh_colsum_batched(const MhColsumJob* jobs_device, int n_jobs, const uint64_t* blocks_device, int n_blocks,
                                 void* stream) {
    MH_CHECK_ARG(jobs_device && blocks_device && n_jobs > 0 && n_jobs < 65536 && n_blocks > 0, "mh_colsum_batched: bad arguments");
    hipLaunchKernelGGL(colsum_batched_kernel, dim3(n_blocks), dim3(256), 0, (hipStream_t)stream, jobs_device, n_jobs, blocks_device);
    MH_LAUNCH_CHECK();
    return 0;
}
```

### maestro_amd/engine.py

```python

from __future__ import annotations

import contextlib
import gc
import os
import weakref
import time

import torch
from torch import nn

from maestro_amd import hip
from maestro_amd.fp8 import mx_scale_cols, resolve_scaling
from maestro_amd.layers.utils import draw_struct_masks

F32, BF16, I32, U8 = torch.float32, torch.bfloat16, torch.int32, torch.uint8
_NEVER = object()
_ROCTX = os.environ.get("MAESTRO_ROCTX", "0") == "1"
RING = 4
ALIGN = 64


class ParamStore:

# ... 434 lines not shown
        self.tile_report = None
        self.warm_passes = 0
        self.warm_passes_run = 0
        self.aux_flag = hip.AUX_U8 if os.environ.get("MAESTRO_AUX_U8", "1") == "1" else 0
        self._tuned = set()
        gc.collect()
        if os.environ.get("MAESTRO_KEEP_RETIRED_GRAPHS", "0") != "1":
            drain_retired_graphs()
        self._graphs, self._seen, self._ready_spans = {}, {}, []
        weakref.finalize(self, _retire_graphs, self._graphs)
        self._inputs = {}
        prio = int(os.environ.get("MAESTRO_SIDE_PRIORITY", "0"))
        self.side_streams = [torch.cuda.Stream(device=device, priority=prio) for _ in range(max(0, n_side_streams))]
        self._wgrad_stream = torch.cuda.Stream(device=device)
        self._wgrad_tables = {}
        self._dw_conv_clear = False

    def _stable_inputs(self, batch: dict) -> dict:
        out = {}
        for k, t in batch.items():
            if not isinstance(t, torch.Tensor) or not t.is_cuda:
                out[k] = t
                continue
            st = self._inputs.get(k)
            if st is None:
                self._inputs[k] = {"ptr": t.data_ptr(), "buf": None}
                out[k] = t
            elif st["buf"] is None and st["ptr"] == t.data_ptr():
                out[k] = t
            else:
                buf = st["buf"]
                if buf is None or buf.shape != t.shape or buf.dtype != t.dtype:
                    buf = st["buf"] = torch.empty_like(t, memory_format=torch.contiguous_format)
                if buf.data_ptr() != t.data_ptr():
                    buf.copy_(t)
                out[k] = buf
        return out

    def _alloc_embed(self) -> None:
        self.embed = {name: PatchEmbedEnd(self, s) for name, s in self.mods.items()}
        self.mb = {name: end.buf for name, end in self.embed.items()}

    def _pack_conv_weights(self) -> None:
        for end in self.embed.values():
            end.pack()

    def _stage_inputs(self, batch: dict) -> dict:
        sources = [parts[0] for parts in self.model.src_specs.values()]
        for s in sources:
            img = batch[s.src]
            if img.dtype != F32 or not img.is_contiguous() or not img.is_cuda:
                raise ValueError(f"batch[{s.src!r}] must be a contiguous float32 GPU tensor")
            d = batch[f"{s.src}_dates"]
            if d.dtype != torch.int16 or not d.is_contiguous():
                raise ValueError(f"batch['{s.src}_dates'] must be a contiguous int16 tensor [B, D, 3]")
        batch = self._stable_inputs(batch)
        for s in sources:
            img = batch[s.src]
            if tuple(img.shape[-2:]) != (s.S, s.S) or self.model.interpolate != "nearest":
                mode = {"nearest": 0, "bilinear": 1, "bicubic": 2}.get(self.model.interpolate)
                if mode is None:
                    raise ValueError(f"Invalid interpolate mode {self.model.interpolate!r} (nearest, bilinear, bicubic)")
                buf = self.mb[s.name].get("resized")
                if buf is None:
                    buf = self.mb[s.name]["resized"] = torch.empty(self.B, s.Dates, s.C_src, s.S, s.S, dtype=F32, device=self.device)
                hip.resize(img, buf, self.B * s.Dates * s.C_src, img.shape[-2], img.shape[-1], s.S, s.S, mode)
                batch[s.src] = buf
        self._staged = batch
        self._cur_key = tuple(batch[k].data_ptr() for k in sorted(batch) if isinstance(batch[k], torch.Tensor))
        return batch

    def returned_batch(self, batch: dict) -> dict:
        out = dict(batch)
        sources = [parts[0] for parts in self.model.src_specs.values()]
        out.update({s.src: self._staged[s.src] for s in sources})
        for s in sources:
            if s.rescale_elev:
                img = out[s.src]
                res = torch.empty_like(img)
                hip.rescale_elev(img, res, img.shape[0] * img.shape[1], s.C_src, s.S)
                out[s.src] = res
        return out

    def _grads_ready(self, module) -> None:
        ps = list(module.parameters())
        if ps:
            self._ready_spans.append(self.store.span(ps))

    def _run_parallel(self, fns) -> None:
        if len(fns) == 1 or not self.multi_stream or not self.group_streams:
            for fn in fns:
                fn()
            return
        main = torch.cuda.current_stream()
        sides = self.side_streams[: len(fns) - 1]
        for side in sides:
            side.wait_stream(main)
        fns[0]()
        for side, fn in zip(sides, fns[1:]):
            with torch.cuda.stream(side):
                fn()
        for side in sides:
            main.wait_stream(side)

    def _instep_tune(self, one_pass) -> None:
        self.instep_tune = False
        if (getattr(self, "fp8", None) is not None or getattr(self, "_opt", None) is not None or hip.kernel_timer_active()
                or torch.cuda.is_current_stream_capturing()):
            return
        saved = (self.use_graphs, self.multi_stream, self.grad_hook)
        self.use_graphs, self.multi_stream, self.grad_hook = False, False, None
        tuner = hip.InStepTuner()
        hip.set_instep_tuner(tuner)
        try:
            one_pass()
            for cand in tuner.CANDIDATES:
                tuner.begin(cand)
                one_pass()
            tuner.begin(None)
            self.tile_report = tuner.finish()
        finally:
            hip.set_instep_tuner(None)
            self.use_graphs, self.multi_stream, self.grad_hook = saved

    def _warm_up(self, one_pass) -> None:
        global _PROCESS_WARMED
        n, self.warm_passes = self.warm_passes, 0
        self.warm_passes_run = 0
        if (n <= 0 or _PROCESS_WARMED or getattr(self, "fp8", None) is not None or getattr(self, "_opt", None) is not None
                or hip.kernel_timer_active() or torch.cuda.is_current_stream_capturing() or not torch.is_grad_enabled()):
            return
        _PROCESS_WARMED = True
        hook, graphs = self.grad_hook, self.use_graphs
        self.use_graphs = False
        if hook is not None:
            self.grad_hook = lambda lo, hi: None
        try:
            for _ in range(n):
                one_pass()
                self.warm_passes_run += 1
        finally:
            self.grad_hook, self.use_graphs = hook, graphs

    def _first_step_passes(self, one_pass) -> None:
        if self.instep_tune:
            self._instep_tune(one_pass)
        if self.warm_passes > 0:
            self._warm_up(one_pass)

    def _launch_wgrads(self, items) -> None:
        items = [(st, lo, hi) for st, lo, hi in items if hi > lo]
        if not items:
            return
        key = tuple((st.tag, lo, hi) for st, lo, hi in items)
        table = self._wgrad_tables.get(key)
        if table is None:
            probs = [p for st, lo, hi in items for p in st.wgrad_problems(lo, hi)]
            jobs = [j for st, lo, hi in items for j in st.reduce_jobs(lo, hi)]
            table = self._wgrad_tables[key] = (hip.GroupedTN(probs, self.device), hip.ColsumBatch(jobs, self.device))
        table[1].launch()
        table[0].launch()

    @contextlib.contextmanager
    def _tuning_pass(self, what: str):
        if not self.tune_gemm or what in self._tuned or hip.kernel_timer_active():
            yield
            return
        saved = self.multi_stream
        self.multi_stream = False
        hip.set_gemm_tuning(True)
        try:
            yield
        finally:
            hip.set_gemm_tuning(False)
            self.multi_stream = saved
            self._tuned.add(what)

    def _segment(self, name: str, key, fn) -> None:
        if _ROCTX:
            torch.cuda.nvtx.range_push(f"maestro:{name.split(':')[0]}")
            try:
                return self._segment_run(name, key, fn)
            finally:
                torch.cuda.nvtx.range_pop()
        return self._segment_run(name, key, fn)

    def _segment_run(self, name: str, key, fn) -> None:
        if not self.use_graphs or hip.kernel_timer_active():
            self._ready_spans = []
            fn()
            self._flush_ready(self._ready_spans)
            return
        entry = self._graphs.get(name)
        if entry is not None and entry["key"] == key:
            entry["graph"].replay()
            self._flush_ready(entry["spans"])
            return
        seen = self._seen.get(name, _NEVER)
        self._ready_spans = []
        if seen == key:
            graph = torch.cuda.CUDAGraph()
            gc_was_on, failure = gc.isenabled(), None
            gc.disable()
            try:
                with torch.cuda.graph(graph, capture_error_mode="thread_local"):
                    fn()
            except Exception as exc:
                failure = exc
            finally:
                if gc_was_on:
                    gc.enable()
            if failure is not None:
                import warnings
                warnings.warn(f"hipGraph capture of segment {name!r} failed ({failure}); continuing with eager launches")
                self.use_graphs = False
                torch.cuda.synchronize()
                self._ready_spans = []
                fn()
                self._flush_ready(self._ready_spans)
                return
            self._graphs[name] = {"key": key, "graph": graph, "spans": list(self._ready_spans)}
            graph.replay()
        else:
            self._seen[name] = key
            fn()
        self._flush_ready(self._ready_spans)

    def _flush_ready(self, spans) -> None:
        if self.grad_hook is not None:
            for lo, hi in spans:
                self.grad_hook(lo, hi)



class MAEEngine(EngineBase):
    def __init__(self, model, batch_size: int, device, loss: str = "l2_norm", dtype: str = "bf16",
                 fp8_scaling: str | None = None, deterministic: bool = False) -> None:
        self.deterministic = bool(deterministic)
        if self.deterministic and dtype == "fp8":
            raise ValueError("deterministic=True is not available with dtype='fp8' (the amax / scale bookkeeping is not covered)")
        if loss not in ("l1", "l2", "l1_norm", "l2_norm"):
            raise ValueError(f"Invalid loss {loss}.")
        if dtype not in ("bf16", "fp8"):
            raise ValueError(f"Invalid compute dtype {dtype!r} (bf16, fp8)")
        scaling = resolve_scaling(fp8_scaling)
        self.fp8_scaling = scaling if dtype == "fp8" else None
        device = torch.device(device)
        if device.type != "cuda":
            raise hip.HipExtensionError("MAEEngine needs a GPU device; the MAE hot path has no CPU fallback")
        hip.lib()
        self.model, self.B, self.device, self.loss, self.dtype = model, batch_size, device, loss, dtype
        self.fp8, self._fp8_weights = None, {}
        self.p_loss = 1 if loss.startswith("l1") else 2
        self.normalise = loss.endswith("_norm")
        m = model
        self.e2d_identity = m.embed_dim == m.decoder_dim
        self.E, self.Dd = m.embed_dim, m.decoder_dim
        self._init_runtime(device, len(model.group_specs) - 1)
        self.wgrad_mode = os.environ.get("MAESTRO_WGRAD", "auto")
        if self.wgrad_mode not in ("auto", "fused", "deferred"):
            raise ValueError(f"MAESTRO_WGRAD={self.wgrad_mode!r}: expected auto, fused or deferred")
        self._wgrad_plans, self._zero_lists = {}, {}
        self._det_sites, self._det_tables = {"fwd": {}, "bwd": {}}, {}
        self._h2d_done = [None] * RING
        self._opt = None
        self.host_wait_s = 0.0
        self._step = 0
        self._enc_state = {}
        B = batch_size
        fold = m.fusion_mode in ("shared", "monotemp")
        self.mods, self.groups = m.mod_specs, list(m.group_specs.values())
        for s in self.mods.values():
            s.Beff = B * s.Dates if fold else B
        for g in self.groups:
            g.Beff = g.mods[0].Beff
        ordered = []
        for name in m.patch_embed:
            ordered += [(f"patch_embed.{name}.{k}", p) for k, p in m.patch_embed[name].named_parameters()]
        for name in m.encoder:
            ordered += [(f"encoder.{name}.{k}", p) for k, p in m.encoder[name].named_parameters()]
        if m.encoder_inter is not None:
            ordered += [(f"encoder_inter.{k}", p) for k, p in m.encoder_inter.named_parameters()]
        for name in m.enc_to_dec:
            ordered += [(f"enc_to_dec.{name}.{k}", p) for k, p in m.enc_to_dec[name].named_parameters()]
        ordered += [(f"mask_token.{k}", p) for k, p in m.mask_token.items()]
        for name in m.decoder:
            ordered += [(f"decoder.{name}.{k}", p) for k, p in m.decoder[name].named_parameters()]
        for name in m.embed_to_rec:
            ordered += [(f"embed_to_rec.{name}.{k}", p) for k, p in m.embed_to_rec[name].named_parameters()]
        self.store = ParamStore(ordered, device)
        for bname in ("enc_pos_encoding", "dec_pos_encoding"):
            setattr(m, bname, getattr(m, bname).to(device))
        if dtype == "fp8":
            from maestro_amd.fp8 import Fp8Plan
            self.fp8 = Fp8Plan(device, self.store.total, scaling=self.fp8_scaling)
        self._alloc()
        self._alloc_mask_upload()
        if self.fp8 is not None:
            self.fp8.finalize()
        self.store.refresh_half(force=True)
        self._pack_conv_weights()

    @property
    def grad_hook(self):
        return self._grad_hook

    @grad_hook.setter
    def grad_hook(self, fn) -> None:
        if fn is not None and getattr(self, "deterministic", False):
            raise ValueError("deterministic=True excludes a gradient hook / exchange: the order of the cross-rank sum is the "
                             "collective library's, and the ready spans would have to move behind the ordered reduce")
        self._grad_hook = fn

    def _det_site(self, phase: str, key, make, variant=None):
        site = self._det_sites[phase].get(key)
        if site is None or site[2] != variant:
            if torch.cuda.is_current_stream_capturing():
                raise hip.HipExtensionError(f"deterministic mode: site {key} first launched inside a hipGraph capture")
            site = self._det_sites[phase][key] = (*make(), variant)
            self._det_tables.pop(phase, None)
        return site[0]

    def _det_reduce(self, phase: str, extra_jobs=()) -> None:
        table = self._det_tables.get(phase)
        if table is None:
            jobs = [j for _, site_jobs, _ in self._det_sites[phase].values() for j in site_jobs] + list(extra_jobs)
            table = self._det_tables[phase] = hip.OrderedReduce(jobs, self.device)
        table.launch()

    def _det_layernorm_bwd(self, key, dy, dy_L, dy_off, x, x_L, x_off, norm, mean, rstd, dx, dx16, bias_grad, B, n, dim) -> None:
        def make():
            size = hip.layernorm_bwd_workspace(B * n, dim)
            ws, rows, g = torch.empty(size, dtype=F32, device=self.device), size // (3 * dim), self.store.g
            jobs = [(ws, g(norm.weight), rows, dim, 3 * dim), (ws[dim:], g(norm.bias), rows, dim, 3 * dim)]
            if bias_grad is not None:
                jobs.append((ws[2 * dim:], bias_grad, rows, dim, 3 * dim))
            return ws, jobs
        ws = self._det_site("bwd", key, make)
        hip.layernorm_bwd_partial(dy, dy_L, dy_off, x, x_L, x_off, norm.weight, mean, rstd, None, dx, dx16, ws, B, n, dim)

    def _det_linear_grads(self, key, dy16, x16, M, N, K, weight_grad, bias_grad) -> None:
        def make():
            e = lambda *sh: torch.empty(*sh, dtype=F32, device=self.device)
            S, cr = hip.det_slices(K), hip.colsum_partial_rows(K)
            w = dict(slabs=e(S, M, N), cs=e(cr, M))
            return w, [(w["slabs"].view(-1), weight_grad.view(-1), S, M * N, M * N), (w["cs"].view(-1), bias_grad, cr, M, M)]
        w = self._det_site("bwd", key, make)
        hip.gemm_tn_slabs(M, N, K, dy16, M, x16, N, w["slabs"])
        hip.colsum_partial(dy16, w["cs"], K, M, M)

    def _det_finish_backward(self) -> None:
        wg = self._det_tables.get("wgrad")
        if wg is None:
            probs = [p for st in self._all_stacks() for p in st.wgrad_problems()]
            n_writers: dict = {}
            for p in probs:
                n_writers[p[2].data_ptr()] = n_writers.get(p[2].data_ptr(), 0) + 1
            slabs_of, seen, slab_jobs, out = {}, {}, [], []
            for p in probs:
                dst = p[2]
                n = n_writers[dst.data_ptr()]
                if n > 1:
                    if dst.data_ptr() not in slabs_of:
                        slabs = slabs_of[dst.data_ptr()] = torch.empty(n, dst.numel(), dtype=F32, device=self.device)
                        slab_jobs.append((slabs.view(-1), dst.view(-1), n, dst.numel(), dst.numel()))
                    i = seen[dst.data_ptr()] = seen.get(dst.data_ptr(), -1) + 1
                    p = p[:2] + (slabs_of[dst.data_ptr()][i].view(dst.shape),) + p[3:]
                out.append(p)
            grouped, single = [], []
            for i, p in enumerate(out):
                try:
                    hip.GroupedTN.check(i, p)
                    grouped.append(p)
                except hip.HipExtensionError:
                    single.append(p)
            stack_jobs = [j for st in self._all_stacks() for j in st.reduce_jobs()]
            wg = self._det_tables["wgrad"] = (hip.GroupedTN(grouped, self.device) if grouped else None, single, stack_jobs + slab_jobs)
        if wg[0] is not None:
            wg[0].launch()
        for (A, B, C, M, N, K, lda, ldb, ldc) in wg[1]:
            hip.gemm(hip.GEMM_TN, M, N, K, A, lda, B, ldb, C, ldc, hip.OUT_F32)
        self._det_reduce("bwd", wg[2])
        for end in self.embed.values():
            b, s = end.buf, end.s
            hip.unpack_rows_add(b["dw_conv"], self.store.g(b["pe"].conv.weight), self.E, s.K, s.Kpad)

    def _alloc(self) -> None:
        m, dev, E, Dd = self.model, self.device, self.E, self.Dd
        e = lambda *s, dt=F32: torch.empty(*s, dtype=dt, device=dev)
        z = lambda *s, dt=F32: torch.zeros(*s, dtype=dt, device=dev)
        self._alloc_embed()
        for name, s in self.mods.items():
            T = s.Beff * s.n_tok
            first = self.mb[m.src_specs[s.src][0].name] if s.gi else None
            self.mb[name].update(
                target=first["target"] if first else e(T, s.C_src * s.P * s.P), hdec=e(T, Dd, dt=BF16), mean_f=e(T), rstd_f=e(T),
                rec=e(T, s.K), drec=e(T, s.K, dt=BF16), dh=e(T, Dd, dt=BF16), cnt=first["cnt"] if first else z(1, dt=I32))
        self.gb = {}
        self.enc, self.dec = {}, {}
        for g in self.groups:
            Bn, L, N = g.Beff, g.L, g.N
            n_dates = sum(s.D for s in g.mods)
            tok_slot = torch.cat([torch.full((s.n_tok,), s.slot, dtype=I32) for s in g.mods])
            date_row = torch.cat([(s.date_off + torch.arange(s.n_tok) // s.L).to(I32) for s in g.mods])
            pos_dec = torch.cat([m.pos_dec_rows[s.name].repeat(s.D, 1) for s in g.mods], dim=0)
            self.gb[g.name] = dict(
                xg=e(Bn, L, E), dxg=z(Bn, L, E),
                vis=e(Bn, N, dt=I32), msk=e(Bn, g.k, dt=I32), inv=e(Bn, L, dt=I32), mask=e(Bn, L, dt=U8),
                dates=z(Bn, n_dates, 8), n_dates=n_dates, tok_slot=tok_slot.to(dev), date_row=date_row.to(dev),
                pos_dec=pos_dec.to(dev).contiguous(), tok_table=e(len(g.mods), Dd),
                henc=e(Bn * N, E, dt=BF16), mean_e=e(Bn * N), rstd_e=e(Bn * N), y_e2d=e(Bn * N, Dd),
                dy_e2d=e(Bn * N, Dd), dy_e2d16=e(Bn * N, Dd, dt=BF16), dhenc=e(Bn * N, E, dt=BF16),
                mean_j=e(Bn * N), rstd_j=e(Bn * N))
            holder = m.encoder[g.model]
            self.enc[g.name] = Stack(self, holder, Bn, N, f"enc.{g.name}")
            self.dec[g.name] = Stack(self, m.decoder[g.model], Bn, L, f"dec.{g.name}")
        if m.encoder_inter is not None:
            self.joint = Stack(self, m.encoder_inter, self.B, m.joint_N, "joint")
        else:
            self.joint = None
        for g in self.groups:
            self.gb[g.name]["ln_ws"] = e(max(hip.layernorm_bwd_workspace(g.Beff * g.L, Dd),
                                             hip.layernorm_bwd_workspace(g.Beff * g.N, E)))
        self.loss_acc = z(1)
        srcs = {s.src: s for s in self.mods.values()}
        tot_w = sum(s.Dates * s.L for s in srcs.values())
        self.loss_w = {n: (s.Dates * s.L) / tot_w for n, s in srcs.items()}

    def _alloc_mask_upload(self) -> None:
        segs, off = [], 0
        for g in self.groups:
            for key, dt, esz in (("noise", F32, 4), ("struct", U8, 1)):
                n = g.Beff * g.L * esz
                segs.append((g.name, key, dt, off, n, (g.Beff, g.L)))
                off += (n + 255) // 256 * 256
        self._mask_dev = torch.zeros(off, dtype=U8, device=self.device)
        self._mask_stage = [torch.zeros(off, dtype=U8, device=self.device) for _ in range(RING)]
        self._mask_host = [torch.zeros(off, dtype=U8).pin_memory() for _ in range(RING)]
        self._upload_stream = torch.cuda.Stream(device=self.device)
        for name, key, dt, o, n, shape in segs:
            self.gb[name][key] = self._mask_dev[o: o + n].view(dt).view(shape)
            self.gb[name][key + "_h"] = [h[o: o + n].view(dt).view(shape) for h in self._mask_host]

    def _pack_conv_weights(self, fp8_done: bool = False) -> None:
        super()._pack_conv_weights()
        if self.fp8 is not None:
            if fp8_done:
                self.fp8.refresh_transposed()
            else:
                self.fp8.refresh_weights()

    def draw_masks(self, generator=None):
        struct = draw_struct_masks(self.groups, self.mods, generator)
        noise = {}
        for g in self.groups:
            if g.draw not in noise:
                noise[g.draw] = torch.rand((g.Beff * g.draw_G, g.L), generator=generator)
        return noise, struct

    @staticmethod
    def _rows_of(draws: dict, g) -> torch.Tensor:
        if g.name in draws:
            return draws[g.name]
        t = draws[g.draw]
        if g.draw_G == 1:
            return t
        D = g.mods[0].Dates
        return t.reshape(g.Beff // D, g.draw_G, D, -1)[:, g.draw_g].reshape(g.Beff, -1)

    def _reference_tie_order(self, g, gbuf, noise: torch.Tensor, struct: torch.Tensor, slot: int):
        if not getattr(self, "_tie_warned", False):
            self._tie_warned = True
            import warnings
            warnings.warn("tie_order='torch' reproduces the tie order of the CPU reference (parity tests); it adds host sorts and an "
                          "H2D copy to every step and is not what the reference does on an accelerator", RuntimeWarning, stacklevel=2)
        B, L, k = g.Beff, g.L, g.k
        nz = noise * (1 - struct.float())
        order = torch.argsort(nz, dim=-1)
        masked = torch.zeros((B, L), dtype=torch.bool)
        masked.scatter_(1, order[:, :k], True)
        place = masked.float().argsort(dim=1, descending=True)[:, :k]
        ascending = order[:, :k].sort(dim=1).values
        if "tok_slot_host" not in gbuf:
            gbuf["tok_slot_host"] = gbuf["tok_slot"].cpu()
            gbuf["tok_slot_ps"] = torch.zeros((B, L), dtype=torch.int32, device=self.device)
            gbuf["tok_slot_ps_h"] = [torch.zeros((B, L), dtype=torch.int32).pin_memory() for _ in range(RING)]
        base = gbuf["tok_slot_host"]
        ps = base[None, :].expand(B, L).clone()
        ps.scatter_(1, place, base[ascending])
        gbuf["tok_slot_ps_h"][slot].copy_(ps)
        gbuf["tok_slot_ps"].copy_(gbuf["tok_slot_ps_h"][slot], non_blocking=True)
        return (~masked).float(), torch.zeros_like(struct)

    def forward(self, batch: dict, noise: dict | None = None, struct: dict | None = None) -> torch.Tensor:
        if self.deterministic:
            self.tune_gemm = self.instep_tune = False
            with hip.shape_only_tiles():
                return self._forward(batch, noise, struct)
        return self._forward(batch, noise, struct)

    def _forward(self, batch: dict, noise: dict | None, struct: dict | None) -> torch.Tensor:
        if self.store.refresh_half():
            if self.fp8 is not None:
                self.fp8._w_ready = False
            self._pack_conv_weights()
        if noise is None or struct is None:
            n2, s2 = self.draw_masks()
            noise = noise if noise is not None else n2
            struct = struct if struct is not None else s2

        def one_pass():
            self.forward(batch, noise=noise, struct=struct)
            self.zero_grad()
            self.backward()
        self._first_step_passes(one_pass)
        slot = self._step % RING
        self._step += 1
        if self._h2d_done[slot] is not None:
            t0 = time.perf_counter()
            self._h2d_done[slot].synchronize()
            self.host_wait_s += time.perf_counter() - t0
        for g in self.groups:
            gbuf = self.gb[g.name]
            nh, sh = gbuf["noise_h"][slot], gbuf["struct_h"][slot]
            n_g, s_g = self._rows_of(noise, g), self._rows_of(struct, g).reshape(g.Beff, g.L)
            if self.tie_order == "torch":
                n_g, s_g = self._reference_tie_order(g, gbuf, n_g, s_g, slot)
            nh.copy_(n_g)
            sh.copy_(s_g)
        main = torch.cuda.current_stream()
        with torch.cuda.stream(self._upload_stream):
            self._mask_stage[slot].copy_(self._mask_host[slot], non_blocking=True)
            up = torch.cuda.Event()
            up.record(self._upload_stream)
        main.wait_event(up)
        self._mask_dev.copy_(self._mask_stage[slot], non_blocking=True)
        if self._opt is not None:
            hh = self._opt_hyper_h[slot]
            hh.copy_(torch.tensor(self._opt_pending if self._opt_pending is not None else [0.0] * 5, dtype=F32))
            self._opt_hyper.copy_(hh, non_blocking=True)
            self._opt_pending = None
        ev = torch.cuda.Event()
        ev.record()
        self._h2d_done[slot] = ev
        batch = self._stage_inputs(batch)
        with self._tuning_pass("forward"):
            self._segment("forward" if self._opt is None else "forward:opt", self._cur_key, lambda: self._forward_launches(batch))
        if self._opt is not None:
            self.store.mark_synced()
        return self.loss_acc

    def attach_optimizer(self, opt) -> None:
        if self.deterministic:
            raise ValueError("deterministic=True excludes overlap_optimizer (the update inside the next forward is not covered)")
        self._attach_optimizer(opt)

    def _attach_optimizer(self, opt) -> None:
        m, ps = self.model, self.store
        if (opt.lo, opt.hi) != (0, ps.total):
            raise ValueError("the overlapped optimizer expects an optimizer over the whole flat buffer")
        stages: dict = {}
        seen_spans = set()

        def add(key, params):
            params = list(params)
            if params:
                sp = ps.span(params)
                if sp not in seen_spans:
                    seen_spans.add(sp)
                    stages.setdefault(key, []).append(sp)

        for name in m.patch_embed:
            add(("embed", 0), m.patch_embed[name].parameters())
        for kind, holders in (("enc", [m.encoder[n] for n in m.encoder]),
                              ("joint", [m.encoder_inter] if m.encoder_inter is not None else []),
                              ("dec", [m.decoder[n] for n in m.decoder])):
            for t in holders:
                depth = len(t.layers)
                for l, layer in enumerate(t.layers):
                    add((kind, l), layer.parameters())
                add((kind, max(depth - 1, 0)), t.norm.parameters())
        add(("e2d", 0), [p for n in m.enc_to_dec for p in m.enc_to_dec[n].parameters()] + list(m.mask_token.values()))
        for name in m.embed_to_rec:
            add(("rec", 0), m.embed_to_rec[name].parameters())
        order = {"embed": 0, "enc": 1, "joint": 2, "e2d": 3, "dec": 4, "rec": 5}
        self._opt_stage_keys = sorted(stages, key=lambda k: (order[k[0]], k[1]))
        covered = sorted(sp for k in stages for sp in stages[k])
        assert covered[0][0] == 0 and all(a[1] <= b[0] for a, b in zip(covered, covered[1:])), "optimizer stages overlap"
        n_cov = sum(hi - lo for lo, hi in covered)
        n_par = sum((p.numel() + ALIGN - 1) // ALIGN * ALIGN for p in ps.params)
        assert n_cov >= n_par - ALIGN * len(ps.params) and covered[-1][1] <= ps.total, "optimizer stages miss parameters"
        self._opt_stages = stages
        self._opt = opt
        self._opt_hyper = torch.zeros(5, dtype=F32, device=self.device)
        self._opt_hyper_h = [torch.zeros(5, dtype=F32).pin_memory() for _ in range(RING)]
        self._opt_pending = None
        self._opt_events = {}
        self._opt_stream = torch.cuda.Stream(device=self.device)

    def defer_step(self, lr: float, grad_scale: float = 1.0) -> None:
        opt = self._opt
        if self._opt_pending is not None:
            raise RuntimeError("an optimizer update is already pending: call forward() or flush_optimizer() first")
        opt.t += 1
        bc1, bc2_sqrt = hip.adamw_bias_corrections(opt.betas[0], opt.betas[1], opt.t)
        self._opt_pending = [lr, bc1, bc2_sqrt, grad_scale, 1.0]

    def flush_optimizer(self) -> None:
        if self._opt is None or self._opt_pending is None:
            return
        lr, _, _, scale, _ = self._opt_pending
        self._opt_pending = None
        self._opt.t -= 1
        self._opt.step(lr=lr, grad_scale=scale)

    def _opt_launch_stages(self) -> None:
        opt, ps = self._opt, self.store
        main = torch.cuda.current_stream()
        side = self._opt_stream if self.multi_stream else main
        if side is not main:
            side.wait_stream(main)
        self._opt_events = {}
        with torch.cuda.stream(side):
            for key in self._opt_stage_keys:
                for lo, hi in self._opt_stages[key]:
                    hip.adamw_dev(ps.flat[lo:hi], ps.grad[lo:hi], opt.m[lo:hi], opt.v[lo:hi], ps.half[lo:hi], hi - lo,
                                  opt.betas[0], opt.betas[1], opt.eps, opt.wd, self._opt_hyper)
                if key[0] == "embed":
                    self._pack_conv_weights()
                if side is not main:
                    ev = torch.cuda.Event()
                    ev.record(side)
                    self._opt_events[key] = ev

    def _opt_wait(self, kind: str, l: int = 0) -> None:
        if self._opt is None:
            return
        ev = self._opt_events.get((kind, l))
        if ev is not None:
            torch.cuda.current_stream().wait_event(ev)

    def _forward_launches(self, batch: dict) -> None:
        m, E, Dd = self.model, self.E, self.Dd
        self.loss_acc.zero_()
        if self._opt is not None:
            self._opt_launch_stages()

        def head(g):
            def run():
                gbuf, st = self.gb[g.name], self.enc[g.name]
                self._opt_wait("embed")
                for s in g.mods:
                    self.embed[s.name].forward(batch, gbuf, gbuf["xg"], g.L, self.mb[s.name]["target"], self.normalise)
                hip.mask_select(gbuf["noise"], gbuf["struct"], gbuf["vis"], gbuf["msk"], gbuf["inv"], gbuf["mask"], g.Beff,
                                g.L, g.k)
                hip.gather_rows(gbuf["xg"], gbuf["vis"], st.x0, g.Beff, g.L, g.N, E, g.N, 0)
                st.forward(lambda l: self._opt_wait("enc", l))
                head_post(g, gbuf, st)
            return run

        def head_post(g, gbuf, st):
            nrm = st.t.norm
            self._opt_wait("enc", max(st.depth - 1, 0))
            if self.joint is not None:
                hip.layernorm_fwd(st.x_last, g.N, 0, nrm.weight, nrm.bias, self.joint.x0, m.joint_N, g.joint_off,
                                  gbuf["mean_e"], gbuf["rstd_e"], g.Beff, g.N, E)
            else:
                hip.layernorm_fwd(st.x_last, g.N, 0, nrm.weight, nrm.bias, gbuf["y_e2d" if self.e2d_identity else "henc"], g.N, 0,
                                  gbuf["mean_e"], gbuf["rstd_e"], g.Beff, g.N, E)

        def tail(g):
            def run():
                gbuf, st = self.gb[g.name], self.dec[g.name]
                self._opt_wait("e2d")
                if self.joint is not None:
                    nrm = self.joint.t.norm
                    hip.layernorm_fwd(self.joint.x_last, m.joint_N, g.joint_off, nrm.weight, nrm.bias,
                                      gbuf["y_e2d" if self.e2d_identity else "henc"], g.N, 0, gbuf["mean_j"], gbuf["rstd_j"],
                                      g.Beff, g.N, E)
                lin = m.enc_to_dec[g.model]
                M = g.Beff * g.N
                if not self.e2d_identity:
                    hip.gemm(hip.GEMM_NT, M, Dd, E, gbuf["henc"], E, self.store.h(lin.weight), E, gbuf["y_e2d"], Dd,
                             hip.OUT_F32 | hip.BIAS, bias=lin.bias)
                for s in g.mods:
                    gbuf["tok_table"][s.slot].copy_(m.mask_token[s.src].view(s.G, Dd)[s.gi])
                if self.tie_order == "torch":
                    hip.unmask_assemble_per_sample(gbuf["y_e2d"], gbuf["inv"], gbuf["tok_table"], gbuf["tok_slot_ps"], gbuf["pos_dec"],
                                                   gbuf["dates"], gbuf["date_row"], gbuf["n_dates"], st.x0, g.Beff, g.L, g.N, Dd)
                else:
                    hip.unmask_assemble(gbuf["y_e2d"], gbuf["inv"], gbuf["tok_table"], gbuf["tok_slot"], gbuf["pos_dec"],
                                        gbuf["dates"], gbuf["date_row"], gbuf["n_dates"], st.x0, g.Beff, g.L, g.N, Dd)
                st.forward(lambda l: self._opt_wait("dec", l))
                tail_post(g, gbuf, st)
            return run

        def tail_post(g, gbuf, st):
            nrm = st.t.norm
            self._opt_wait("rec")
            for s in g.mods:
                b = self.mb[s.name]
                T = s.Beff * s.n_tok
                conv = m.embed_to_rec[s.embed].pixelify_bands[s.gi].conv
                hip.layernorm_fwd(st.x_last, g.L, s.tok_off, nrm.weight, nrm.bias, b["hdec"], s.n_tok, 0, b["mean_f"],
                                  b["rstd_f"], s.Beff, s.n_tok, Dd)
                hip.gemm(hip.GEMM_NT, T, s.K, Dd, b["hdec"], Dd, self.store.h(conv.weight).view(s.K, Dd), Dd, b["rec"],
                         s.K, hip.OUT_F32 | hip.BIAS, bias=conv.bias)
                if s.G == 1:
                    hip.count_masked(gbuf["mask"], g.Beff, g.L, s.tok_off, s.tok_off + s.n_tok, b["cnt"])
            for s in g.mods:
                b = self.mb[s.name]
                if self.deterministic:
                    def make(s=s):
                        part = torch.empty(hip.masked_loss_partial_size(s.Beff, s.n_tok), dtype=F32, device=self.device)
                        return part, [(part, self.loss_acc, part.numel(), 1, 1)]
                    part = self._det_site("fwd", ("loss", s.name), make)
                    if s.G == 1:
                        hip.masked_loss_det(b["rec"], b["target"], gbuf["mask"], b["cnt"], self.loss_w[s.src], part,
                                            b["drec"], s.Beff, s.n_tok, g.L, s.tok_off, s.K, self.p_loss)
                    else:
                        hip.masked_loss_bands_det(b["rec"], b["target"], gbuf["mask"], b["cnt"], self.loss_w[s.src], part,
                                                  b["drec"], s.Beff, s.n_tok, g.L, s.tok_off, s.K, self.p_loss, s.C_src, s.c0, s.C)
                elif s.G == 1:
                    hip.masked_loss(b["rec"], b["target"], gbuf["mask"], b["cnt"], self.loss_w[s.src], self.loss_acc,
                                    b["drec"], s.Beff, s.n_tok, g.L, s.tok_off, s.K, self.p_loss)
                else:
                    hip.masked_loss_bands(b["rec"], b["target"], gbuf["mask"], b["cnt"], self.loss_w[s.src], self.loss_acc,
                                          b["drec"], s.Beff, s.n_tok, g.L, s.tok_off, s.K, self.p_loss, s.C_src, s.c0, s.C)

        self._run_parallel([head(g) for g in self.groups])
        if self.joint is not None:
            self.joint.forward(lambda l: self._opt_wait("joint", l))
        for parts in m.src_specs.values():
            if len(parts) > 1:
                for s in parts:
                    g = m.group_specs[s.group]
                    hip.count_masked_elems(self.gb[g.name]["mask"], g.Beff, g.L, s.tok_off, s.tok_off + s.n_tok,
                                           self.mb[s.name]["cnt"], s.K, s.gi > 0)
        self._run_parallel([tail(g) for g in self.groups])
        if self.deterministic:
            self._det_reduce("fwd")
        if self._opt is not None and self._opt_events:
            torch.cuda.current_stream().wait_stream(self._opt_stream)
        if self.fp8 is not None:
            self.fp8.end_of_forward()

    def zero_grad(self) -> None:
        plan = self._wgrad_plan()
        if plan == "fused":
            self.store.grad.zero_()
            for b in self.mb.values():
                if b.get("dw_conv") is not None:
                    b["dw_conv"].zero_()
            self._dw_conv_clear = True
            return
        z = self._zero_lists.get(plan)
        if z is None:
            writers = {}
            for st in self._all_stacks():
                for prob in st.wgrad_problems():
                    c = prob[2]
                    writers.setdefault(c.data_ptr(), [0, c.numel()])[0] += 1
            base = self.store.grad.data_ptr()
            stored = sorted(((ptr - base) // 4, n) for ptr, (cnt, n) in writers.items() if cnt == 1)
            spans, cur = [], 0
            for off, n in stored:
                if off > cur:
                    spans.append((cur, off - cur))
                cur = off + n
            if cur < self.store.total:
                spans.append((cur, self.store.total - cur))
            for b in self.mb.values():
                if b.get("dw_conv") is not None:
                    spans.append(((b["dw_conv"].data_ptr() - base) // 4, b["dw_conv"].numel()))
            dev = torch.tensor([v for sp in spans for v in sp], dtype=torch.int64, device=self.device)
            z = self._zero_lists[plan] = (dev, len(spans), max(n for _, n in spans))
        hip.zero_spans(self.store.grad, z[0], z[1], z[2])
        self._dw_conv_clear = True

    WGRAD_MIN_TILES = 256

    def _wgrad_plan(self) -> str:
        if self.deterministic:
            return "all"
        if self.wgrad_mode == "fused":
            return "fused"
        hooked = self.grad_hook is not None
        plan = self._wgrad_plans.get((self.wgrad_mode, hooked))
        if plan is not None:
            return plan
        try:
            every = {st.tag: hip.GroupedTN.count_tiles(st.wgrad_problems()) for st in self._all_stacks()}
            tiles = [every[st.tag] for st in self.enc.values()] if hooked else list(every.values())
            ok = True
        except hip.HipExtensionError:
            tiles, ok = [], False
        if not ok:
            if self.wgrad_mode == "deferred":
                raise hip.HipExtensionError("MAESTRO_WGRAD=deferred: a weight-gradient problem is not eligible for the grouped GEMM")
            plan = "fused"
        elif hooked:
            n_seg = len(self._enc_cuts()) - 1
            plan = "enc" if self.wgrad_mode == "deferred" or sum(tiles) // n_seg >= self.WGRAD_MIN_TILES else "fused"
        else:
            plan = "all" if self.wgrad_mode == "deferred" or sum(tiles) >= self.WGRAD_MIN_TILES else "fused"
            if plan == "all" and os.environ.get("MAESTRO_WGRAD_OVERLAP", "0") == "1":
                plan = "ovl"
        self._wgrad_plans[(self.wgrad_mode, hooked)] = plan
        return plan

    def _all_stacks(self) -> list:
        return list(self.dec.values()) + ([self.joint] if self.joint is not None else []) + list(self.enc.values())

    def _with_overlapped_wgrads(self, fn, previous, own):
        def run():
            if previous and self.multi_stream:
                main = torch.cuda.current_stream()
                side = self._wgrad_stream
                side.wait_stream(main)
                with torch.cuda.stream(side):
                    self._launch_wgrads(previous)
                fn()
                main.wait_stream(side)
            else:
                if previous:
                    self._launch_wgrads(previous)
                fn()
            if own:
                self._launch_wgrads(own)
        return run

    def _enc_cuts(self) -> list:
        depth = max(st.depth for st in self.enc.values())
        n = max(1, min(4, int(os.environ.get("MAESTRO_ENC_CUTS", "3"))))
        cut = self.grad_hook is not None or getattr(self, "_plan", None) == "ovl"
        if not cut or depth < 3 or n == 1:
            return [depth, 0]
        return [depth] + [depth - (i * depth) // n for i in range(1, n)] + [0]

    def backward(self, grad_scale: float = 1.0) -> None:
        if grad_scale != 1.0:
            raise NotImplementedError("loss scaling is not needed for bf16 (SURVEY §8(f) AMP row)")
        if self.deterministic:
            with hip.shape_only_tiles():
                return self._backward()
        return self._backward()

    def _backward(self) -> None:
        key = getattr(self, "_cur_key", None)
        plan = self._plan = self._wgrad_plan()
        sfx = f":{plan}:{'h' if self.grad_hook is not None else 'n'}"
        if not self._dw_conv_clear:
            sfx += ":nz"
        if self.fp8 is not None and self.fp8.dgrad:
            sfx += ":f8" if self.fp8.grad_ready else ":cal"
        cuts = self._enc_cuts()
        segs = [("bwd_dec", self._bwd_decoder_side, [(st, 0, st.depth) for st in self.dec.values()])]
        if self.joint is not None:
            segs.append(("bwd_joint", self._bwd_joint, [(self.joint, 0, self.joint.depth)]))
        for i in range(len(cuts) - 1):
            segs.append((f"bwd_enc{i}", lambda hi=cuts[i], lo=cuts[i + 1], first=(i == 0), last=(i == len(cuts) - 2):
                         self._bwd_encoder_side(hi, lo, first, last),
                         [(st, min(cuts[i + 1], st.depth), min(cuts[i], st.depth)) for st in self.enc.values()]))
        with self._tuning_pass("backward"):
            for i, (name, fn, items) in enumerate(segs):
                if plan == "ovl":
                    fn = self._with_overlapped_wgrads(fn, segs[i - 1][2] if i else None, items if i == len(segs) - 1 else None)
                self._segment(name + sfx, key, fn)
        self._dw_conv_clear = False
        if self.fp8 is not None:
            self.fp8.end_of_backward()

    def _bwd_decoder_side(self) -> None:
        m, E, Dd, ps = self.model, self.E, self.Dd, self.store
        AT = hip.OUT_F32 | hip.ATOMIC

        def side(g):
            def run():
                gbuf, st = self.gb[g.name], self.dec[g.name]
                nrm = st.t.norm
                dx, dx16 = st.dxa, st.top16
                for s in g.mods:
                    b = self.mb[s.name]
                    T = s.Beff * s.n_tok
                    conv = m.embed_to_rec[s.embed].pixelify_bands[s.gi].conv
                    w16 = ps.h(conv.weight).view(s.K, Dd)
                    hip.gemm(hip.GEMM_NN, T, Dd, s.K, b["drec"], s.K, w16, Dd, b["dh"], Dd)
                    if self.deterministic:
                        self._det_linear_grads(("rec", s.name), b["drec"], b["hdec"], s.K, Dd, T, ps.g(conv.weight), ps.g(conv.bias))
                        self._det_layernorm_bwd(("ln_dec", s.name), b["dh"], s.n_tok, 0, st.x_last, g.L, s.tok_off, nrm, b["mean_f"],
                                                b["rstd_f"], dx, dx16, st.top_bias_grad(), s.Beff, s.n_tok, Dd)
                        self._grads_ready(m.embed_to_rec[s.embed])
                        continue
                    hip.gemm(hip.GEMM_TN, s.K, Dd, T, b["drec"], s.K, b["hdec"], Dd, ps.g(conv.weight).view(s.K, Dd), Dd, AT)
                    hip.colsum(b["drec"], ps.g(conv.bias), T, s.K, s.K)
                    hip.layernorm_bwd(b["dh"], s.n_tok, 0, st.x_last, g.L, s.tok_off, nrm.weight, b["mean_f"], b["rstd_f"],
                                      None, dx, dx16, ps.g(nrm.weight), ps.g(nrm.bias), st.top_bias_grad(), gbuf["ln_ws"],
                                      s.Beff, s.n_tok, Dd)
                    self._grads_ready(m.embed_to_rec[s.embed])
                dx0, _ = st.backward(dx, defer=self._plan in ("all", "enc", "ovl"))
                side_post(g, gbuf, st, dx0)
            return run

        def side_post(g, gbuf, st, dx0):
            self._grads_ready(st.t.norm)
            hip.gather_rows(dx0, gbuf["vis"], gbuf["dy_e2d"], g.Beff, g.L, g.N, Dd, g.N, 0)
            for s in g.mods:
                if self.deterministic:
                    per_sample = self.tie_order == "torch"
                    n_rows = g.Beff * (g.L if per_sample else s.n_tok)

                    def make(s=s, n_rows=n_rows):
                        rows = hip.unmask_token_grad_partial_rows(n_rows)
                        part = torch.empty(rows, Dd, dtype=F32, device=self.device)
                        return part, [(part.view(-1), ps.g(m.mask_token[s.src]).view(s.G, Dd)[s.gi], rows, Dd, Dd)]
                    part = self._det_site("bwd", ("tok", s.name), make, variant=per_sample)
                    if per_sample:
                        hip.unmask_token_grad_per_sample_det(dx0, gbuf["mask"], gbuf["tok_slot_ps"], part, g.Beff, g.L, Dd, s.slot)
                    else:
                        hip.unmask_token_grad_det(dx0, gbuf["mask"], gbuf["tok_slot"], part, g.Beff, g.L, Dd, s.slot, s.tok_off,
                                                  s.tok_off + s.n_tok)
                elif self.tie_order == "torch":
                    hip.unmask_token_grad_per_sample(dx0, gbuf["mask"], gbuf["tok_slot_ps"],
                                                     ps.g(m.mask_token[s.src]).view(s.G, Dd)[s.gi], g.Beff, g.L, Dd, s.slot)
                else:
                    hip.unmask_token_grad(dx0, gbuf["mask"], gbuf["tok_slot"], ps.g(m.mask_token[s.src]).view(s.G, Dd)[s.gi], g.Beff,
                                          g.L, Dd, s.slot, s.tok_off, s.tok_off + s.n_tok)
                self._ready_spans.append(ps.span([m.mask_token[s.src]]))
            M = g.Beff * g.N
            lin = m.enc_to_dec[g.model]
            if not self.e2d_identity:
                hip.cast_bf16(gbuf["dy_e2d"], gbuf["dy_e2d16"], M * Dd)
                hip.gemm(hip.GEMM_NN, M, E, Dd, gbuf["dy_e2d16"], Dd, ps.h(lin.weight), E, gbuf["dhenc"], E)
                if self.deterministic:
                    self._det_linear_grads(("e2d", g.name), gbuf["dy_e2d16"], gbuf["henc"], Dd, E, M, ps.g(lin.weight), ps.g(lin.bias))
                else:
                    hip.gemm(hip.GEMM_TN, Dd, E, M, gbuf["dy_e2d16"], Dd, gbuf["henc"], E, ps.g(lin.weight), E, AT)
                    hip.colsum(gbuf["dy_e2d16"], ps.g(lin.bias), M, Dd, Dd)
                self._grads_ready(lin)
            if self.joint is not None:
                jt = self.joint
                jn = jt.t.norm
                dy = gbuf["dy_e2d" if self.e2d_identity else "dhenc"]
                if self.deterministic:
                    self._det_layernorm_bwd(("ln_joint", g.name), dy, g.N, 0, jt.x_last, m.joint_N, g.joint_off, jn, gbuf["mean_j"],
                                            gbuf["rstd_j"], jt.dxa, jt.top16, jt.top_bias_grad(), g.Beff, g.N, E)
                else:
                    hip.layernorm_bwd(dy, g.N, 0, jt.x_last, m.joint_N, g.joint_off, jn.weight, gbuf["mean_j"],
                                      gbuf["rstd_j"], None, jt.dxa, jt.top16, ps.g(jn.weight), ps.g(jn.bias),
                                      jt.top_bias_grad(), gbuf["ln_ws"], g.Beff, g.N, E)

        self._run_parallel([side(g) for g in self.groups])
        if self._plan == "enc":
            self._launch_wgrads([(st, 0, st.depth) for st in self.dec.values()])

    def _bwd_joint(self) -> None:
        jt = self.joint
        self._djoint, _ = jt.backward(jt.dxa, defer=self._plan in ("all", "enc", "ovl"))
        self._grads_ready(jt.t.norm)
        if self._plan == "enc":
            self._launch_wgrads([(jt, 0, jt.depth)])

    def _bwd_encoder_side(self, hi: int, lo: int, first: bool, last: bool) -> None:
        m, E, ps = self.model, self.E, self.store

        def side(g):
            def run():
                gbuf, st = self.gb[g.name], self.enc[g.name]
                nrm = st.t.norm
                s_hi, s_lo = min(hi, st.depth), min(lo, st.depth)
                if first and self.deterministic:
                    dy, dy_L, dy_off = ((self._djoint, m.joint_N, g.joint_off) if self.joint is not None else
                                        (gbuf["dy_e2d" if self.e2d_identity else "dhenc"], g.N, 0))
                    self._det_layernorm_bwd(("ln_enc", g.name), dy, dy_L, dy_off, st.x_last, g.N, 0, nrm, gbuf["mean_e"], gbuf["rstd_e"],
                                            st.dxa, st.top16, st.top_bias_grad(), g.Beff, g.N, E)
                    self._grads_ready(nrm)
                    self._enc_state[g.name] = (st.dxa, st.top16)
                elif first:
                    if self.joint is not None:
                        hip.layernorm_bwd(self._djoint, m.joint_N, g.joint_off, st.x_last, g.N, 0, nrm.weight, gbuf["mean_e"],
                                          gbuf["rstd_e"], None, st.dxa, st.top16, ps.g(nrm.weight), ps.g(nrm.bias),
                                          st.top_bias_grad(), gbuf["ln_ws"], g.Beff, g.N, E)
                    else:
                        hip.layernorm_bwd(gbuf["dy_e2d" if self.e2d_identity else "dhenc"], g.N, 0, st.x_last, g.N, 0, nrm.weight,
                                          gbuf["mean_e"],
                                          gbuf["rstd_e"], None, st.dxa, st.top16, ps.g(nrm.weight), ps.g(nrm.bias),
                                          st.top_bias_grad(), gbuf["ln_ws"], g.Beff, g.N, E)
                    self._grads_ready(nrm)
                    self._enc_state[g.name] = (st.dxa, st.top16)
                cur, _ = self._enc_state[g.name]
                self._enc_state[g.name] = st.backward(cur, s_hi, s_lo, defer=self._plan != "fused")
                if last:
                    side_post(g, gbuf, st)
            return run

        def side_post(g, gbuf, st):
            dx0 = self._enc_state[g.name][0]
            hip.expand_rows(dx0, gbuf["inv"], gbuf["dxg"], g.Beff, g.L, g.N, E)
            for s in g.mods:
                self.embed[s.name].backward(gbuf["dxg"], g.L, not self._dw_conv_clear)

        self._run_parallel([side(g) for g in self.groups])
        if self._plan == "enc":
            self._launch_wgrads([(st, min(lo, st.depth), min(hi, st.depth)) for st in self.enc.values()])
        elif self.deterministic and last:
            self._det_finish_backward()
        elif self._plan == "all" and last:
            self._launch_wgrads([(st, 0, st.depth) for st in self._all_stacks()])
        if last:
            for name in m.patch_embed:
                self._grads_ready(m.patch_embed[name])

    def reconstructions(self):
        pixels, masks = {}, {}
        for g in self.groups:
            mask = self.gb[g.name]["mask"]
            for s in g.mods:
                b = self.mb[s.name]
                BD = s.Beff * s.D
                img = torch.empty(BD, s.C, s.S, s.S, dtype=F32, device=self.device)
                hip.depatchify(b["rec"], img, BD, s.C, s.S, s.P)
                pixels[s.name] = img.view(self.B, s.Dates, s.C, s.S, s.S)
                tok = mask[:, s.tok_off: s.tok_off + s.n_tok].bool().reshape(self.B, s.Dates, 1, s.g, 1, s.g, 1)
                masks[s.name] = tok.expand(self.B, s.Dates, s.C, s.g, s.P, s.g, s.P).reshape(self.B, s.Dates, s.C, s.S, s.S)
        for src, parts in self.model.src_specs.items():
            if len(parts) > 1:
                pixels[src] = torch.cat([pixels.pop(s.name) for s in parts], dim=2)
                masks[src] = torch.cat([masks.pop(s.name) for s in parts], dim=2)
        return pixels, masks

    def logged_sample(self, name_mod: str):
        parts = self.model.src_specs[name_mod]
        s0 = parts[0]
        recs, msks = [], []
        for s in parts:
            g = next(g for g in self.groups if s in g.mods)
            rec = torch.empty(1, s.C, s.S, s.S, dtype=F32, device=self.device)
            hip.depatchify(self.mb[s.name]["rec"][: s.L], rec, 1, s.C, s.S, s.P)
            tok = self.gb[g.name]["mask"][0, s.tok_off: s.tok_off + s.L].bool().reshape(1, s.g, 1, s.g, 1)
            recs.append(rec[0])
            msks.append(tok.expand(s.C, s.g, s.P, s.g, s.P).reshape(s.C, s.S, s.S))
        tgt = self._staged[name_mod][0, 0]
        if s0.rescale_elev:
            res = torch.empty(1, s0.C_src, s0.S, s0.S, dtype=F32, device=self.device)
            hip.rescale_elev(tgt.contiguous(), res, 1, s0.C_src, s0.S)
            tgt = res[0]
        return tgt, (recs[0] if len(parts) == 1 else torch.cat(recs)), (msks[0] if len(parts) == 1 else torch.cat(msks))

    def token_masks(self) -> dict:
        return {g.name: self.gb[g.name]["mask"].bool() for g in self.groups}
```

### maestro_amd/hip.py

```python

from __future__ import annotations

import contextlib
import ctypes
import os
from pathlib import Path

import torch

_LIB_PATH = Path(__file__).resolve().parent / "lib" / "libmaestro_hip.so"
_lib = None

GEMM_NT, GEMM_NN, GEMM_TN = 0, 1, 2
OUT_F32, BIAS, GELU, RESIDUAL, DGELU, ATOMIC, COLSUM, AUX_DGELU, MULAUX, C8_E5M2, AUX_U8 = 1, 2, 4, 8, 16, 32, 64, 128, 256, 512, 1024


class HipExtensionError(RuntimeError):
    pass


def lib() -> ctypes.CDLL:
    global _lib
    if _lib is None:
        if not _LIB_PATH.exists():
# ... 178 lines not shown
        rc = _gemm_tile(tile, *args)
        if rc == -2:
            continue
        _check(rc, "mh_gemm_bf16_tile")
        _gemm_tile(tile, *args)
        e0, e1 = torch.cuda.Event(enable_timing=True), torch.cuda.Event(enable_timing=True)
        e0.record()
        for _ in range(4):
            _gemm_tile(tile, *args)
        e1.record()
        e1.synchronize()
        ms = e0.elapsed_time(e1)
        if ms < best_ms:
            best, best_ms = tile, ms
    _tile_choice[key] = best
    return best


_shape_only = 0


@contextlib.contextmanager
def shape_only_tiles():
    global _shape_only
    _shape_only += 1
    try:
        yield
    finally:
        _shape_only -= 1


def _pick_tile(layout, M, N, K, flags, args) -> int:
    if _shape_only:
        return TILE_AUTO
    tflags = flags & ~COLSUM
    key = (layout, M, N, K, tflags)
    tile = _tile_choice.get(key)
    if tile is None:
        forced = os.environ.get("MH_GEMM_TILE")
        if forced is not None:
            t = int(forced)
            if TILE_PP_128 < t <= TILE_PP_128 + 5 and os.environ.get("MH_ALLOW_DIAG_TILES") != "1":
                raise HipExtensionError(f"MH_GEMM_TILE={t} selects a diagnostic build of the ping-pong tile that writes wrong "
                                        "outputs (present only in a -DMH_DIAG_TILES library); set MH_ALLOW_DIAG_TILES=1 to run it on purpose")
            return t
        dma = os.environ.get("MH_GEMM_DMA", "")[:1]
        if os.environ.get("MH_GEMM_PP", "")[:1] == "0" and dma == "":
            return _resolve(TILE_AUTO, args, FAMILY_DMA)
        if dma == "0":
            return TILE_REG_128
        lockstep = os.environ.get("MH_DMA_STAGGER", "")[:1] == "0"
        if (dma == "1" and layout != GEMM_TN and not (flags & ATOMIC)) or (
                lockstep and _resolve(TILE_AUTO, args, FAMILY_DMA) == TILE_DMA_256):
            return TILE_DMA_256_LOCKSTEP if lockstep else TILE_DMA_256
        if _tuning and not (flags & ATOMIC):
            targs = list(args)
            targs[10], targs[17] = tflags, None
            tile = _tune_gemm(key, tuple(targs))
        else:
            tile = TILE_AUTO
    return tile


def gemm(layout: int, M: int, N: int, K: int, A, lda: int, B, ldb: int, C, ldc: int, flags: int = 0, bias=None,
         res=None, ldr: int = 0, aux_in=None, aux_out=None, ldaux: int = 0, colsum=None, tile: int | None = None) -> None:
    args = (layout, M, N, K, A, lda, B, ldb, C, ldc, flags, bias, res, ldr, aux_in, aux_out, ldaux, colsum)
    explicit = tile is not None
    if _instep is not None and _instep.cand is not None and not explicit and not (flags & ATOMIC):
        key = (layout, M, N, K, flags & ~COLSUM)
        e0, e1 = _instep.open(key)
        e0.record()
        rc = _gemm_tile(_instep.cand, *args)
        if rc == -2:
            _instep.reject(key)
            rc = _gemm_tile(TILE_AUTO, *args)
        _check(rc, "mh_gemm_bf16_tile")
        e1.record()
        return
    if not explicit:
        tile = _pick_tile(layout, M, N, K, flags, args)
    ev = None
    if _timer is not None:
        named = tile if tile in SK_TILES else _resolve(tile, args)
        if named == -2:
            named = tile
        ev = _timer.record(_TILE_NAME[named].format(_LAYOUT_NAME[layout]), 2.0 * M * N * K, (M, N, K))
        ev[0].record()
    rc = _gemm_tile(tile, *args)
    if rc == -2 and not explicit:
        pinned = os.environ.get("MH_GEMM_DMA", "")[:1] == "1" or os.environ.get("MH_GEMM_PP", "")[:1] == "0"
        rc = _gemm_tile(TILE_REG_128 if pinned else TILE_AUTO, *args)
    if rc == -2:
        raise HipExtensionError(f"mh_gemm_bf16_tile: problem ({M}, {N}, {K}) does not qualify for tile {tile}")
    _check(rc, "mh_gemm_bf16_tile")
    if ev is not None:
        ev[1].record()


def call(name: str, *args) -> None:
    conv = []
    for a in args:
        if a is None or isinstance(a, torch.Tensor):
            conv.append(ptr(a))
        else:
            conv.append(a)
    _check(getattr(lib(), name)(*conv, stream()), name)


def _hbm_call(kind: str, nbytes: float, name: str, *args) -> None:
    if _timer is None:
        return call(name, *args)
    e0, e1 = _timer.record_bytes(kind, nbytes)
    e0.record()
    call(name, *args)
    e1.record()


def _esz(t) -> int:
    return 0 if t is None else t.element_size()


def layernorm_fwd(x, x_L, x_off, gamma, beta, y, y_L, y_off, mean, rstd, B, n, dim, eps=1e-5):
    _hbm_call(f"ln_fwd<{dim}>", float(B) * n * dim * (4 + _esz(y)), "mh_layernorm_fwd", x, _I(x_L), _I(x_off), gamma, beta, y, _I(y_L),
              _I(y_off), _I(1 if y.dtype == torch.float32 else 0), mean, rstd, _I(B), _I(n), _I(dim), _F(eps))


def layernorm_fwd_fp8(x, x_L, x_off, gamma, beta, y, y_L, y_off, mean, rstd, B, n, dim, y8, y8_scale, y8_amax, eps=1e-5):
    call("mh_layernorm_fwd_fp8", x, _I(x_L), _I(x_off), gamma, beta, y, _I(y_L), _I(y_off), mean, rstd, _I(B), _I(n), _I(dim),
         _F(eps), y8, y8_scale, y8_amax)


def layernorm_fwd_mx(x, x_L, x_off, gamma, beta, y, y_L, y_off, mean, rstd, B, n, dim, y8, y8_scales, ld_y8s, eps=1e-5):
    call("mh_layernorm_fwd_mx", x, _I(x_L), _I(x_off), gamma, beta, y, _I(y_L), _I(y_off), mean, rstd, _I(B), _I(n), _I(dim),
         _F(eps), y8, y8_scales, _I(ld_y8s))


def layernorm_bwd_workspace(rows, dim) -> int:
    f = lib().mh_layernorm_bwd_workspace
    f.restype = ctypes.c_long
    return int(f(_I(rows), _I(dim)))


def layernorm_bwd(dy, dy_L, dy_off, x, x_L, x_off, gamma, mean, rstd, dres, dx, dx_bf16, dgamma, dbeta, dcol, workspace,
                  B, n, dim):
    _hbm_call(f"ln_bwd<{dim}>", float(B) * n * dim * (_esz(dy) + 4 + _esz(dres) + 4 + _esz(dx_bf16)), "mh_layernorm_bwd", dy, _I(dy_L),
              _I(dy_off), _I(1 if dy.dtype == torch.float32 else 0), x, _I(x_L), _I(x_off), gamma, mean, rstd, dres, dx, dx_bf16,
              dgamma, dbeta, dcol, workspace, _I(B), _I(n), _I(dim))


def layernorm_bwd_partial(dy, dy_L, dy_off, x, x_L, x_off, gamma, mean, rstd, dres, dx, dx_bf16, workspace, B, n, dim):
    _hbm_call(f"ln_bwd<{dim}>", float(B) * n * dim * (_esz(dy) + 4 + _esz(dres) + 4 + _esz(dx_bf16)), "mh_layernorm_bwd_partial", dy,
              _I(dy_L), _I(dy_off), _I(1 if dy.dtype == torch.float32 else 0), x, _I(x_L), _I(x_off), gamma, mean, rstd, dres, dx,
              dx_bf16, workspace, _I(B), _I(n), _I(dim))


COLSUM_ROWS = 16


class _MhColsumJob(ctypes.Structure):
    _fields_ = [("src", ctypes.c_void_p), ("dst", ctypes.c_void_p), ("rows", ctypes.c_int), ("cols", ctypes.c_int),
                ("ld", ctypes.c_int), ("reserved", ctypes.c_int)]


class ColsumBatch:

    def __init__(self, jobs, device) -> None:
        if not jobs:
            raise HipExtensionError("ColsumBatch: no jobs")
        arr = (_MhColsumJob * len(jobs))()
        for i, (src, dst, rows, cols, ld) in enumerate(jobs):
            if src.dtype != torch.float32 or dst.dtype != torch.float32 or not src.is_cuda or not dst.is_cuda:
                raise HipExtensionError("ColsumBatch: f32 device tensors expected")
            if rows <= 0 or cols <= 0 or ld < cols or src.numel() < (rows - 1) * ld + cols or dst.numel() < cols:
                raise HipExtensionError(f"ColsumBatch job {i}: shape ({rows}, {cols}, ld {ld}) does not fit its buffers")
            arr[i] = _MhColsumJob(src.data_ptr(), dst.data_ptr(), rows, cols, ld, 0)
        self.keep = [t for job in jobs for t in job[:2]]
        self.table = torch.frombuffer(bytearray(bytes(arr)), dtype=torch.uint8).to(device)
        blocks = []
        for i, (_, _, rows, cols, _) in enumerate(jobs):
            if cols > 65535 * 256 or len(jobs) > 32767:
                raise HipExtensionError("ColsumBatch: too many jobs / columns for the work-item encoding")
            for cb in range(-(-cols // 256)):
                blocks += [(i << 48) | (cb << 32) | rc for rc in range(-(-rows // COLSUM_ROWS))]
        self.blocks = torch.tensor(blocks, dtype=torch.int64).to(device)
        self.n, self.n_blocks = len(jobs), len(blocks)

    def launch(self) -> None:
        call("mh_colsum_batched", self.table, _I(self.n), self.blocks, _I(self.n_blocks))


ORDERED_ROWS, ORDERED_ADD = 16, 1
COLSUM_PARTIAL_ROWS = 256


class _MhOrderedJob(ctypes.Structure):
    _fields_ = [("src", ctypes.c_void_p), ("dst", ctypes.c_void_p), ("rows", ctypes.c_int), ("cols", ctypes.c_int),
                ("ld", ctypes.c_int), ("flags", ctypes.c_int)]


class OrderedReduce:

    def __init__(self, jobs, device) -> None:
        if not jobs:
            raise HipExtensionError("OrderedReduce: no jobs")
        chains: dict = {}
        for i, job in enumerate(jobs):
            if len(job) not in (5, 6):
                raise HipExtensionError(f"OrderedReduce job {i}: (src, dst, rows, cols, ld[, add]) expected")
            src, dst, rows, cols, ld = job[:5]
            add = bool(job[5]) if len(job) == 6 else False
            if not (isinstance(src, torch.Tensor) and isinstance(dst, torch.Tensor)) or src.dtype != torch.float32 \
                    or dst.dtype != torch.float32 or not src.is_cuda or not dst.is_cuda:
                raise HipExtensionError(f"OrderedReduce job {i}: f32 device tensors expected")
            if rows <= 0 or cols <= 0 or ld < cols or src.numel() < (rows - 1) * ld + cols or dst.numel() < cols:
                raise HipExtensionError(f"OrderedReduce job {i}: shape ({rows}, {cols}, ld {ld}) does not fit its buffers")
            chain = chains.setdefault(dst.data_ptr(), [])
            if chain and (chain[0][3] != cols or chain[0][5] != add):
                raise HipExtensionError(f"OrderedReduce job {i}: cols / add differ from the other jobs of its destination")
            chain.append((src, dst, rows, cols, ld, add))
        spans = sorted((c[0][1].data_ptr(), c[0][1].data_ptr() + 4 * c[0][3]) for c in chains.values())
        if any(a[1] > b[0] for a, b in zip(spans, spans[1:])):
            raise HipExtensionError("OrderedReduce: two destinations overlap without being the same")
        flat = [j for chain in chains.values() for j in chain]
        arr = (_MhOrderedJob * len(flat))()
        blocks, i = [], 0
        for chain in chains.values():
            blocks += [(i << 32) | cb for cb in range(-(-chain[0][3] // 256))]
            for src, dst, rows, cols, ld, add in chain:
                arr[i] = _MhOrderedJob(src.data_ptr(), dst.data_ptr(), rows, cols, ld, ORDERED_ADD if add else 0)
                i += 1
        self.keep = [t for j in flat for t in j[:2]]
        self.host = arr
        self.table = torch.frombuffer(bytearray(bytes(arr)), dtype=torch.uint8).to(device)
        self.blocks = torch.tensor(blocks, dtype=torch.int64).to(device)
        self.n, self.n_blocks, self.n_chains = len(flat), len(blocks), len(chains)
        self.nbytes = 4.0 * (sum(j[2] * j[3] for j in flat) + sum(c[0][3] for c in chains.values()))

    def launch(self) -> None:
        ev = _timer.record_bytes("reduce_ordered", self.nbytes) if _timer is not None else None
        if ev is not None:
            ev[0].record()
        _check(lib().mh_reduce_ordered(ctypes.byref(self.host), ptr(self.table), _I(self.n), ptr(self.blocks), _I(self.n_blocks),
                                       stream()), "mh_reduce_ordered")
        if ev is not None:
            ev[1].record()


def colsum_partial_rows(M) -> int:
    return int(lib().mh_colsum_partial_rows(_I(M)))


def colsum_partial(x, partial, M, N, ld):
    call("mh_colsum_partial", x, _I(1 if x.dtype == torch.float32 else 0), partial, _I(M), _I(N), _I(ld))


def masked_loss_partial_size(B, Lm) -> int:
    return int(lib().mh_masked_loss_partial_size(_I(B), _I(Lm)))


def masked_loss_det(rec, target, mask_group, n_masked, weight, loss_partial, drec, B, Lm, Lgroup, tok_off, PPC, p):
    _hbm_call("masked_loss", float(B) * Lm * (PPC * (_esz(rec) + 4 + _esz(drec)) + 1), "mh_masked_loss_det", rec, target, mask_group,
              n_masked, _F(weight), loss_partial, drec, _I(B), _I(Lm), _I(Lgroup), _I(tok_off), _I(PPC), _I(p))


def masked_loss_bands_det(rec, target, mask_group, n_elems, weight, loss_partial, drec, B, Lm, Lgroup, tok_off, PPC, p, tgt_C,
                          tgt_c0, n_g):
    call("mh_masked_loss_bands_det", rec, target, mask_group, n_elems, _F(weight), loss_partial, drec, _I(B), _I(Lm), _I(Lgroup),
         _I(tok_off), _I(PPC), _I(p), _I(tgt_C), _I(tgt_c0), _I(n_g))


def unmask_token_grad_partial_rows(n_rows) -> int:
    return int(lib().mh_unmask_token_grad_partial_rows(_L(n_rows)))


def unmask_token_grad_det(dxdec, mask, tok_slot, partial, B, L, Dd, slot, t_lo, t_hi):
    call("mh_unmask_token_grad_det", dxdec, mask, tok_slot, partial, _I(B), _I(L), _I(Dd), _I(slot), _I(t_lo), _I(t_hi))


def unmask_token_grad_per_sample_det(dxdec, mask, tok_slot_bl, partial, B, L, Dd, slot):
    call("mh_unmask_token_grad_per_sample_det", dxdec, mask, tok_slot_bl, partial, _I(B), _I(L), _I(Dd), _I(slot))


def embed_bwd_partial_rows(BD, L) -> int:
    return int(lib().mh_embed_bwd_partial_rows(_I(BD), _I(L)))


def embed_finish_bwd_det(dxg, y, stats, gamma, dyc, param_partial, blk_sums, sums, B, D, L, E, tok_off, Lgroup):
    call("mh_embed_finish_bwd_det", dxg, y, stats, gamma, dyc, param_partial, blk_sums, sums, _I(B), _I(D), _I(L), _I(E),
         _I(tok_off), _I(Lgroup))


def det_slices(K: int) -> int:
    return max(1, min(8, K // 1024))


def gemm_tn_slabs(M, N, K, A, lda, B, ldb, slabs):
    S = slabs.shape[0]
    step = -(-(-(-K // S)) // 64) * 64
    for i in range(S):
        k0 = i * step
        kn = min(K, k0 + step) - k0
        if kn <= 0:
            raise HipExtensionError(f"gemm_tn_slabs: empty K-slice {i} of {S} (K = {K})")
        gemm(GEMM_TN, M, N, kn, A[k0:], lda, B[k0:], ldb, slabs[i], N, OUT_F32)


# ... 570 lines not shown
```

Baseline: 1873.

## Fuse model-end kernels: loss colsum, gather+cast, deferred layernorm param reductions

Adds an optional 'fused ends' path, enabled by default through MAESTRO_FUSED_ENDS. The masked loss kernel now also writes per-block column sums of drec, which replaces a separate colsum pass for the conv bias gradient. The row gather now writes a bf16 copy directly, which removes a standalone cast kernel. Layernorm backwards at the decoder, joint and encoder ends switch to partial workspaces whose parameter-gradient reductions are batched into one colsum job list. Together these cut kernel launches and extra HBM passes, at the cost of extra workspace buffers, more shared memory in the loss kernel and added code-path complexity.

After: 1869. About the same (-0.2%).

```diff
diff --git a/__graft_entry__.py b/__graft_entry__.py
--- a/__graft_entry__.py
+++ b/__graft_entry__.py
@@ -25,7 +25,7 @@
     handle = ctypes.CDLL(str(lib))
     import re
 
-    for name in ("maestro_hip.h", "maestro_hip_metrics.h", "maestro_hip_det.h"):
+    for name in ("maestro_hip.h", "maestro_hip_metrics.h", "maestro_hip_det.h", "maestro_hip_ends.h"):
         header = (ROOT / "include" / name).read_text()
         missing = [n for n in re.findall(r"\b(mh_[a-z0-9_]+)\s*\(", header) if not hasattr(handle, n)]
         if missing:
diff --git a/include/maestro_hip_ends.h b/include/maestro_hip_ends.h
--- /dev/null
+++ b/include/maestro_hip_ends.h
@@ -0,0 +1,25 @@
+#ifndef MAESTRO_HIP_ENDS_H
+#define MAESTRO_HIP_ENDS_H
+#include <stdint.h>
+#ifdef __cplusplus
+extern "C" {
+#endif
+
+int mh_layernorm_fwd_ends(const float* x, int x_L, int x_off, const float* gamma, const float* beta, void* y, int y_L, int y_off,
+                          int y_is_f32, float* mean, float* rstd, int B, int n, int dim, float eps, void* stream);
+int mh_layernorm_bwd_partial_ends(const void* dy, int dy_L, int dy_off, int dy_is_f32, const float* x, int x_L, int x_off,
+                                  const float* gamma, const float* mean, const float* rstd, const float* dres, float* dx,
+                                  void* dx_bf16, float* workspace, int B, int n, int dim, void* stream);
+
+#define MH_LOSS_COLSUM_MAX_PPC 1024
+int mh_masked_loss_v2(const float* rec, const float* target, const uint8_t* mask_group, const int* n_masked, float weight,
+                      float* acc, void* drec, float* colsum_partial, int B, int Lm, int Lgroup, int tok_off, int PPC, int p,
+                      void* stream);
+
+int mh_gather_rows_v2(const float* src, const int* idx, float* dst, void* dst_bf16, int B, int src_L, int n_idx, int dim,
+                      int dst_L, int dst_off, void* stream);
+
+#ifdef __cplusplus
+}
+#endif
+#endif
diff --git a/maestro_amd/csrc/build.py b/maestro_amd/csrc/build.py
--- a/maestro_amd/csrc/build.py
+++ b/maestro_amd/csrc/build.py
@@ -33,7 +33,8 @@
 def _digest(src: Path) -> str:
     h = hashlib.sha256()
     for f in [src, *sorted(CSRC.glob("*.hpp")), ROOT / "include" / "maestro_hip.h",
-              ROOT / "include" / "maestro_hip_metrics.h", ROOT / "include" / "maestro_hip_det.h"]:
+              ROOT / "include" / "maestro_hip_metrics.h", ROOT / "include" / "maestro_hip_det.h",
+              ROOT / "include" / "maestro_hip_ends.h"]:
         h.update(f.read_bytes())
     h.update(" ".join(FLAGS + FILE_FLAGS.get(src.name, [])).encode())
     return h.hexdigest()[:16]
diff --git a/maestro_amd/csrc/loss.hip b/maestro_amd/csrc/loss.hip
--- a/maestro_amd/csrc/loss.hip
+++ b/maestro_amd/csrc/loss.hip
@@ -1,20 +1,25 @@
 #include "gemm_common.hpp"
 #include "../../include/maestro_hip_det.h"
+#include "../../include/maestro_hip_ends.h"
 
 namespace {
 
-template <bool DET>
-__global__ __launch_bounds__(256) void masked_loss_kernel(const float* __restrict__ rec, const float* __restrict__ target,
+template <bool DET, int NJ>
+__device__ __forceinline__ void masked_loss_body(const float* __restrict__ rec, const float* __restrict__ target,
                                                           const uint8_t* __restrict__ mask_group, const int* __restrict__ n_masked,
                                                           float weight, float* __restrict__ acc, bf16_t* __restrict__ drec,
                                                           int B, int Lm, int Lgroup, int tok_off, int PPC, int p, int tgt_C,
-                                                          int tgt_c0, int n_g, int denom_is_elems, int rows_per_wave) {
+                                                          int tgt_c0, int n_g, int denom_is_elems, int rows_per_wave,
+                                                          float* __restrict__ cs_partial, float* __restrict__ cs_red) {
     __shared__ float red[4];
     const int w = threadIdx.x >> 6, lane = threadIdx.x & 63;
     const float coef = weight / (denom_is_elems ? (float)(*n_masked) : (float)(*n_masked) * (float)PPC);
     const bool window = n_g != tgt_C;
     const int tgt_ld = window ? PPC / n_g * tgt_C : PPC;
     float s = 0.f;
+    f32x4 csum[NJ > 0 ? NJ : 1];
+#pragma unroll
+    for (int j = 0; j < (NJ > 0 ? NJ : 1); ++j) csum[j] = (f32x4){0, 0, 0, 0};
     for (int rr = 0; rr < rows_per_wave; ++rr) {
         const int row = (blockIdx.x * 4 + w) * rows_per_wave + rr;
         if (row >= B * Lm) break;
@@ -23,7 +28,7 @@
         const float* r = rec + (size_t)row * PPC;
         const float* g = target + (size_t)row * tgt_ld;
         bf16_t* d = drec ? drec + (size_t)row * PPC : nullptr;
-        for (int c = lane * 4; c < PPC; c += 256) {
+        for (int c = lane * 4, jc = 0; c < PPC; c += 256, ++jc) {
             float dd[4] = {0.f, 0.f, 0.f, 0.f};
             if (masked) {
                 const f32x4 rv = *reinterpret_cast<const f32x4*>(r + c);
@@ -44,8 +49,26 @@
             if (d) {
                 u32x2 pk = {pack_bf2(dd[0], dd[1]), pack_bf2(dd[2], dd[3])};
                 *reinterpret_cast<u32x2*>(d + c) = pk;
+                if constexpr (NJ > 0) {
+                    const f32x4 q = {__uint_as_float(pk[0] << 16), __uint_as_float(pk[0] & 0xffff0000u),
+                                     __uint_as_float(pk[1] << 16), __uint_as_float(pk[1] & 0xffff0000u)};
+#pragma unroll
+                    for (int j = 0; j < NJ; ++j)
+                        if (j == jc) csum[j] += q;
+                }
             }
         }
+    }
+    if constexpr (NJ > 0) {
+        for (int c = lane * 4, jc = 0; c < PPC; c += 256, ++jc) {
+#pragma unroll
+            for (int j = 0; j < NJ; ++j)
+                if (j == jc) *reinterpret_cast<f32x4*>(cs_red + (size_t)w * PPC + c) = csum[j];
+        }
+        __syncthreads();
+        float* prow = cs_partial + (size_t)blockIdx.x * PPC;
+        for (int c = threadIdx.x; c < PPC; c += 256)
+            prow[c] = (cs_red[c] + cs_red[PPC + c]) + (cs_red[2 * PPC + c] + cs_red[3 * PPC + c]);
     }
     s = wave_sum(s);
     if (lane == 0) red[w] = s;
@@ -59,6 +82,26 @@
         if (blockIdx.x == 0 && *n_masked == 0) atomicAdd(acc, __builtin_nanf(""));
         }
     }
+}
+template <bool DET>
+__global__ __launch_bounds__(256) void masked_loss_kernel(const float* __restrict__ rec, const float* __restrict__ target,
+                                                          const uint8_t* __restrict__ mask_group, const int* __restrict__ n_masked,
+                                                          float weight, float* __restrict__ acc, bf16_t* __restrict__ drec,
+                                                          int B, int Lm, int Lgroup, int tok_off, int PPC, int p, int tgt_C,
+                                                          int tgt_c0, int n_g, int denom_is_elems, int rows_per_wave) {
+    masked_loss_body<DET, 0>(rec, target, mask_group, n_masked, weight, acc, drec, B, Lm, Lgroup, tok_off, PPC, p, tgt_C, tgt_c0, n_g,
+                             denom_is_elems, rows_per_wave, nullptr, nullptr);
+}
+template <int NJ>
+__global__ __launch_bounds__(256) void masked_loss_colsum_kernel(const float* __restrict__ rec, const float* __restrict__ target,
+                                                                 const uint8_t* __restrict__ mask_group,
+                                                                 const int* __restrict__ n_masked, float weight,
+                                                                 float* __restrict__ acc, bf16_t* __restrict__ drec, int B, int Lm,
+                                                                 int Lgroup, int tok_off, int PPC, int p, int rows_per_wave,
+                                                                 float* __restrict__ cs_partial) {
+    extern __shared__ __attribute__((aligned(16))) float cs_red[];
+    masked_loss_body<false, NJ>(rec, target, mask_group, n_masked, weight, acc, drec, B, Lm, Lgroup, tok_off, PPC, p, 1, 0, 1, 0,
+                                rows_per_wave, cs_partial, cs_red);
 }
 
 template <bool DET>
@@ -247,6 +290,25 @@
     return 0;
 }
 
+extern "C" int mh_masked_loss_v2(const float* rec, const float* target, const uint8_t* mask_group, const int* n_masked,
+                                 float weight, float* acc, void* drec, float* colsum_partial, int B, int Lm, int Lgroup, int tok_off,
+                                 int PPC, int p, void* stream) {
+    if (!colsum_partial) return mh_masked_loss(rec, target, mask_group, n_masked, weight, acc, drec, B, Lm, Lgroup, tok_off, PPC, p, stream);
+    MH_CHECK_ARG(rec && target && mask_group && n_masked && acc && drec, "mh_masked_loss_v2: null pointer (the column sums are those of drec)");
+    MH_CHECK_ARG(B > 0 && Lm > 0 && (p == 1 || p == 2) && PPC % 4 == 0 && tok_off + Lm <= Lgroup, "mh_masked_loss_v2: bad arguments");
+    MH_CHECK_ARG(PPC <= MH_LOSS_COLSUM_MAX_PPC && ((uintptr_t)colsum_partial % 16) == 0,
+                 "mh_masked_loss_v2: column sums need PPC <= %d (got %d) and a 16-byte aligned partial buffer", MH_LOSS_COLSUM_MAX_PPC, PPC);
+    const int rpw = loss_rows_per_wave((long)B * Lm);
+    const dim3 grid(ceil_div((long)B * Lm, 4 * rpw));
+    const size_t lds = (size_t)4 * PPC * sizeof(float);
+#define LOSS_CS(NJ) hipLaunchKernelGGL(masked_loss_colsum_kernel<NJ>, grid, dim3(256), lds, (hipStream_t)stream, rec, target, mask_group, \
+                                       n_masked, weight, acc, (bf16_t*)drec, B, Lm, Lgroup, tok_off, PPC, p, rpw, colsum_partial)
+    switch (ceil_div(PPC, 256)) { case 1: LOSS_CS(1); break; case 2: LOSS_CS(2); break; case 3: LOSS_CS(3); break; default: LOSS_CS(4); }
+#undef LOSS_CS
+    MH_LAUNCH_CHECK();
+    return 0;
+}
+
 extern "C" int mh_masked_loss_bands(const float* rec, const float* target, const uint8_t* mask_group, const int* n_elems,
                                     float weight, float* acc, void* drec, int B, int Lm, int Lgroup, int tok_off, int PPC, int p,
                                     int tgt_C, int tgt_c0, int n_g, void* stream) {
diff --git a/maestro_amd/csrc/mask.hip b/maestro_amd/csrc/mask.hip
--- a/maestro_amd/csrc/mask.hip
+++ b/maestro_amd/csrc/mask.hip
@@ -1,5 +1,6 @@
 #include "common.hpp"
 #include "../../include/maestro_hip.h"
+#include "../../include/maestro_hip_ends.h"
 
 namespace {
 
@@ -70,6 +71,22 @@
     const float* s = src + ((size_t)b * src_L + idx[row]) * dim;
     float* d = dst + ((size_t)b * dst_L + dst_off + j) * dim;
     for (int c = lane * 4; c < dim; c += 256) *reinterpret_cast<f32x4*>(d + c) = *reinterpret_cast<const f32x4*>(s + c);
+}
+
+__global__ __launch_bounds__(256) void gather_rows_bf16_kernel(const float* __restrict__ src, const int* __restrict__ idx,
+                                                               float* __restrict__ dst, bf16_t* __restrict__ dst16, int B, int src_L,
+                                                               int n_idx, int dim, int dst_L, int dst_off) {
+    const int row = blockIdx.x * 4 + (threadIdx.x >> 6), lane = threadIdx.x & 63;
+    if (row >= B * n_idx) return;
+    const int b = row / n_idx, j = row - b * n_idx;
+    const float* s = src + ((size_t)b * src_L + idx[row]) * dim;
+    const size_t drow = ((size_t)b * dst_L + dst_off + j) * dim;
+    for (int c = lane * 4; c < dim; c += 256) {
+        const f32x4 v = *reinterpret_cast<const f32x4*>(s + c);
+        *reinterpret_cast<f32x4*>(dst + drow + c) = v;
+        const u32x2 pk = {pack_bf2(v[0], v[1]), pack_bf2(v[2], v[3])};
+        *reinterpret_cast<u32x2*>(dst16 + drow + c) = pk;
+    }
 }
 
 __global__ __launch_bounds__(256) void scatter_rows_kernel(const float* __restrict__ ddst, const int* __restrict__ idx,
@@ -200,6 +217,18 @@
     return 0;
 }
 
+extern "C" int mh_gather_rows_v2(const float* src, const int* idx, float* dst, void* dst_bf16, int B, int src_L, int n_idx, int dim,
+                                 int dst_L, int dst_off, void* stream) {
+    if (!dst_bf16) return mh_gather_rows(src, idx, dst, B, src_L, n_idx, dim, dst_L, dst_off, stream);
+    MH_CHECK_ARG(src && idx && dst && B > 0 && n_idx > 0 && dim % 4 == 0 && dst_off >= 0 && dst_off + n_idx <= dst_L,
+                 "mh_gather_rows_v2: bad arguments");
+    MH_CHECK_ARG(((uintptr_t)dst_bf16 % 8) == 0, "mh_gather_rows_v2: dst_bf16 must be 8-byte aligned");
+    hipLaunchKernelGGL(gather_rows_bf16_kernel, dim3(ceil_div((long)B * n_idx, 4)), dim3(256), 0, (hipStream_t)stream, src, idx, dst,
+                       (bf16_t*)dst_bf16, B, src_L, n_idx, dim, dst_L, dst_off);
+    MH_LAUNCH_CHECK();
+    return 0;
+}
+
 extern "C" int mh_scatter_rows(const float* ddst, const int* idx, float* dsrc, int B, int src_L, int n_idx, int dim,
                                int dst_L, int dst_off, void* stream) {
     MH_CHECK_ARG(ddst && idx && dsrc && dim % 4 == 0 && dst_off + n_idx <= dst_L, "mh_scatter_rows: bad arguments");
diff --git a/maestro_amd/csrc/norm.hip b/maestro_amd/csrc/norm.hip
--- a/maestro_amd/csrc/norm.hip
+++ b/maestro_amd/csrc/norm.hip
@@ -1,4 +1,6 @@
 #include "gemm_common.hpp"
+#include "../../include/maestro_hip_ends.h"
+#include <type_traits>
 
 namespace {
 
@@ -103,9 +105,9 @@
 #endif
 }
 enum { LN_Y8_NONE = 0, LN_Y8_TENSOR = 1, LN_Y8_MX = 2 };
-template <int NV, int Y8>
+template <int NV, int Y8, bool YF32 = false>
 __device__ __forceinline__ void ln_fwd_fast_body(const float* __restrict__ x, RowMap xm, const float* __restrict__ gamma,
-                                                          const float* __restrict__ beta, bf16_t* __restrict__ y, RowMap ym,
+                                                          const float* __restrict__ beta, void* __restrict__ y, RowMap ym,
                                                           float* __restrict__ mean, float* __restrict__ rstd, int B, int n,
                                                           float eps, uint8_t* __restrict__ y8, const float* __restrict__ y8_scale,
                                                           float* __restrict__ y8_amax, uint8_t* __restrict__ y8s, int ld_y8s) {
@@ -127,16 +129,16 @@
     float s = 0.f;
 #pragma unroll
     for (int i = 0; i < NV; ++i) s += (v[i][0] + v[i][1]) + (v[i][2] + v[i][3]);
-    const float mu = ln_wave_sum(s) / dim;
+    const float mu = (YF32 ? wave_sum(s) : ln_wave_sum(s)) / dim;
     float q = 0.f;
 #pragma unroll
     for (int i = 0; i < NV; ++i) {
 #pragma unroll
         for (int e = 0; e < 4; ++e) { const float d = v[i][e] - mu; q += d * d; }
     }
-    const float rs = rsqrtf(ln_wave_sum(q) / dim + eps);
+    const float rs = rsqrtf((YF32 ? wave_sum(q) : ln_wave_sum(q)) / dim + eps);
     const size_t yrow = map_row(ym, b, j) * dim;
-    bf16_t* yr = y + yrow;
+    bf16_t* yr = reinterpret_cast<bf16_t*>(y) + yrow;
     float s8 = 0.f;
     if constexpr (FP8) s8 = *y8_scale;
     float amax8 = 0.f;
@@ -145,6 +147,11 @@
         f32x4 o;
 #pragma unroll
         for (int e = 0; e < 4; ++e) o[e] = (v[i][e] - mu) * rs * g[i][e] + bt[i][e];
+        if constexpr (YF32) {
+            static_assert(Y8 == LN_Y8_NONE, "the fp8 copies belong to the bf16 output");
+            *reinterpret_cast<f32x4*>(reinterpret_cast<float*>(y) + yrow + 4 * (lane + 64 * i)) = o;
+            continue;
+        }
         const u32x2 pk = {pack_bf2(o[0], o[1]), pack_bf2(o[2], o[3])};
         *reinterpret_cast<u32x2*>(yr + 4 * (lane + 64 * i)) = pk;
         if constexpr (Y8 == LN_Y8_MX) {
@@ -178,6 +185,13 @@
                                                           float* __restrict__ y8_amax) {
     ln_fwd_fast_body<NV, FP8 ? LN_Y8_TENSOR : LN_Y8_NONE>(x, xm, gamma, beta, y, ym, mean, rstd, B, n, eps, y8, y8_scale, y8_amax,
                                                           nullptr, 0);
+}
+template <int NV>
+__global__ __launch_bounds__(256) void ln_fwd_fast_f32_kernel(const float* __restrict__ x, RowMap xm, const float* __restrict__ gamma,
+                                                              const float* __restrict__ beta, float* __restrict__ y, RowMap ym,
+                                                              float* __restrict__ mean, float* __restrict__ rstd, int B, int n,
+                                                              float eps) {
+    ln_fwd_fast_body<NV, LN_Y8_NONE, true>(x, xm, gamma, beta, y, ym, mean, rstd, B, n, eps, nullptr, nullptr, nullptr, nullptr, 0);
 }
 template <int NV>
 __global__ __launch_bounds__(256) void ln_fwd_fast_mx_kernel(const float* __restrict__ x, RowMap xm, const float* __restrict__ gamma,
@@ -397,6 +411,105 @@
         prow[c] = red[c] + red[3 * dim + c] + red[6 * dim + c] + red[9 * dim + c];
 }
 
+template <int NV, int DEPTH, bool DYF32, bool RES, bool DX16>
+__global__ __launch_bounds__(256) void ln_bwd_fast_end_kernel(const void* __restrict__ dy_, RowMap dym, const float* __restrict__ x,
+                                                              RowMap xm, const float* __restrict__ gamma,
+                                                              const float* __restrict__ mean, const float* __restrict__ rstd,
+                                                              const float* __restrict__ dres, float* __restrict__ dx,
+                                                              bf16_t* __restrict__ dx_bf16, float* __restrict__ partial, int B, int n) {
+    constexpr int dim = 256 * NV;
+    static_assert(DEPTH >= 1 && DEPTH <= ROWS_PER_WAVE, "prefetch distance in rows");
+    extern __shared__ __attribute__((aligned(16))) float red[];
+    using dy_elem_t = std::conditional_t<DYF32, float, bf16_t>;
+    using dy_vec_t = std::conditional_t<DYF32, f32x4, u32x2>;
+    const dy_elem_t* __restrict__ dy = reinterpret_cast<const dy_elem_t*>(dy_);
+    const int w = __builtin_amdgcn_readfirstlane(threadIdx.x >> 6), lane = threadIdx.x & 63;
+    f32x4 gsum[NV], bsum[NV], csum[NV], gm[NV];
+#pragma unroll
+    for (int i = 0; i < NV; ++i) {
+        gsum[i] = (f32x4){0, 0, 0, 0}; bsum[i] = (f32x4){0, 0, 0, 0}; csum[i] = (f32x4){0, 0, 0, 0};
+        gm[i] = *reinterpret_cast<const f32x4*>(gamma + 4 * (lane + 64 * i));
+    }
+    const int row0 = (blockIdx.x * 4 + w) * ROWS_PER_WAVE;
+    if (row0 < B * n) {
+        f32x4 xq[ROWS_PER_WAVE][NV], rq[RES ? ROWS_PER_WAVE : 1][NV];
+        dy_vec_t dq[ROWS_PER_WAVE][NV];
+        float muq[ROWS_PER_WAVE], rsq[ROWS_PER_WAVE];
+        size_t xrowq[ROWS_PER_WAVE];
+        auto fetch = [&](int p) {
+            const int row = row0 + p, b = row / n, j = row - b * n;
+            xrowq[p] = map_row(xm, b, j) * dim;
+            const size_t dyrow = map_row(dym, b, j) * dim;
+            muq[p] = mean[row]; rsq[p] = rstd[row];
+#pragma unroll
+            for (int i = 0; i < NV; ++i) {
+                const int c4 = 4 * (lane + 64 * i);
+                xq[p][i] = *reinterpret_cast<const f32x4*>(x + xrowq[p] + c4);
+                dq[p][i] = *reinterpret_cast<const dy_vec_t*>(dy + dyrow + c4);
+                if constexpr (RES) rq[p][i] = *reinterpret_cast<const f32x4*>(dres + xrowq[p] + c4);
+            }
+        };
+#pragma unroll
+        for (int p = 0; p < DEPTH; ++p) fetch(p);
+#pragma unroll
+        for (int rr = 0; rr < ROWS_PER_WAVE; ++rr) {
+            if (rr + DEPTH < ROWS_PER_WAVE) fetch(rr + DEPTH);
+            __builtin_amdgcn_sched_barrier(0);
+            const float mu = muq[rr], rs = rsq[rr];
+            f32x4 xh[NV], dz[NV];
+            float s1 = 0.f, s2 = 0.f;
+#pragma unroll
+            for (int i = 0; i < NV; ++i) {
+                f32x4 d;
+                if constexpr (DYF32) {
+                    d = dq[rr][i];
+                } else {
+                    const u32x2 pk = dq[rr][i];
+                    d = (f32x4){__uint_as_float(pk[0] << 16), __uint_as_float(pk[0] & 0xffff0000u),
+                                __uint_as_float(pk[1] << 16), __uint_as_float(pk[1] & 0xffff0000u)};
+                }
+#pragma unroll
+                for (int e = 0; e < 4; ++e) {
+                    xh[i][e] = (xq[rr][i][e] - mu) * rs;
+                    dz[i][e] = d[e] * gm[i][e];
+                    s1 += dz[i][e];
+                    s2 += dz[i][e] * xh[i][e];
+                    gsum[i][e] += d[e] * xh[i][e];
+                    bsum[i][e] += d[e];
+                }
+            }
+            const float c1 = wave_sum(s1) / dim, c2 = wave_sum(s2) / dim;
+#pragma unroll
+            for (int i = 0; i < NV; ++i) {
+                const int c4 = 4 * (lane + 64 * i);
+                f32x4 o;
+#pragma unroll
+                for (int e = 0; e < 4; ++e) o[e] = rs * (dz[i][e] - c1 - xh[i][e] * c2);
+                if constexpr (RES) o += rq[rr][i];
+                csum[i] += o;
+                *reinterpret_cast<f32x4*>(dx + xrowq[rr] + c4) = o;
+                if constexpr (DX16) {
+                    const u32x2 pk = {pack_bf2(o[0], o[1]), pack_bf2(o[2], o[3])};
+                    *reinterpret_cast<u32x2*>(dx_bf16 + xrowq[rr] + c4) = pk;
+                }
+            }
+            __builtin_amdgcn_sched_barrier(0);
+        }
+    }
+    if (!partial) return;
+    float* rg = red + (size_t)w * 3 * dim;
+#pragma unroll
+    for (int i = 0; i < NV; ++i) {
+        const int c4 = 4 * (lane + 64 * i);
+        *reinterpret_cast<f32x4*>(rg + c4) = gsum[i];
+        *reinterpret_cast<f32x4*>(rg + dim + c4) = bsum[i];
+        *reinterpret_cast<f32x4*>(rg + 2 * dim + c4) = csum[i];
+    }
+    __syncthreads();
+    float* prow = partial + (size_t)blockIdx.x * 3 * dim;
+    for (int c = threadIdx.x; c < 3 * dim; c += 256)
+        prow[c] = red[c] + red[3 * dim + c] + red[6 * dim + c] + red[9 * dim + c];
+}
 #ifndef LN_BWD_DEPTH
 #define LN_BWD_DEPTH 4
 #endif
@@ -440,7 +553,7 @@
 
 static int layernorm_fwd_impl(const float* x, int x_L, int x_off, const float* gamma, const float* beta, void* y, int y_L,
                               int y_off, int y_is_f32, float* mean, float* rstd, int B, int n, int dim, float eps, void* y8,
-                              const float* y8_scale, float* y8_amax, void* stream, void* y8s, int ld_y8s);
+                              const float* y8_scale, float* y8_amax, void* stream, void* y8s, int ld_y8s, bool ends = false);
 
 extern "C" int mh_layernorm_fwd(const float* x, int x_L, int x_off, const float* gamma, const float* beta, void* y,
                                 int y_L, int y_off, int y_is_f32, float* mean, float* rstd, int B, int n, int dim,
@@ -469,7 +582,7 @@
 
 static int layernorm_fwd_impl(const float* x, int x_L, int x_off, const float* gamma, const float* beta, void* y, int y_L,
                               int y_off, int y_is_f32, float* mean, float* rstd, int B, int n, int dim, float eps, void* y8,
-                              const float* y8_scale, float* y8_amax, void* stream, void* y8s, int ld_y8s) {
+                              const float* y8_scale, float* y8_amax, void* stream, void* y8s, int ld_y8s, bool ends) {
     MH_CHECK_ARG(x && gamma && beta && y && mean && rstd, "mh_layernorm_fwd: null pointer");
     MH_CHECK_ARG(dim % 4 == 0 && dim >= 4 && dim <= 2048, "mh_layernorm_fwd: dim %d unsupported", dim);
     MH_CHECK_ARG(B > 0 && n > 0 && x_off + n <= x_L && y_off + n <= y_L, "mh_layernorm_fwd: bad row map");
@@ -483,10 +596,14 @@
                                                  (bf16_t*)y, RowMap{y_L, y_off}, mean, rstd, B, n, eps, (uint8_t*)y8, y8_scale, y8_amax)
 #define LN_FWD_FAST_MX(NV) hipLaunchKernelGGL((ln_fwd_fast_mx_kernel<NV>), grid, block, 0, s, x, RowMap{x_L, x_off}, gamma, beta, \
                                               (bf16_t*)y, RowMap{y_L, y_off}, mean, rstd, B, n, eps, (uint8_t*)y8, (uint8_t*)y8s, ld_y8s)
-#define LN_FWD_FAST(NV) do { if (y8s) LN_FWD_FAST_MX(NV); else if (y8) LN_FWD_FAST_(NV, true); else LN_FWD_FAST_(NV, false); } while (0)
+#define LN_FWD_FAST_F32(NV) hipLaunchKernelGGL((ln_fwd_fast_f32_kernel<NV>), grid, block, 0, s, x, RowMap{x_L, x_off}, gamma, beta, \
+                                               (float*)y, RowMap{y_L, y_off}, mean, rstd, B, n, eps)
+#define LN_FWD_FAST(NV) do { if (y_is_f32) LN_FWD_FAST_F32(NV); else if (y8s) LN_FWD_FAST_MX(NV); else if (y8) LN_FWD_FAST_(NV, true); \
+                             else LN_FWD_FAST_(NV, false); } while (0)
     const int nvs = ln_nv(dim);
     MH_CHECK_ARG(!y8s || (dim % 32 == 0 && !y_is_f32), "mh_layernorm_fwd_mx: dim %% 32 == 0 required, got %d", dim);
-    if (MH_LN_FAST && nvs <= 4 && dim == 256 * nvs && !y_is_f32) {
+    MH_CHECK_ARG(!y8 || !y_is_f32, "mh_layernorm_fwd: the fp8 copies belong to the bf16 output");
+    if (MH_LN_FAST && nvs <= 4 && dim == 256 * nvs && (!y_is_f32 || ends)) {
         switch (nvs) { case 1: LN_FWD_FAST(1); break; case 2: LN_FWD_FAST(2); break; case 3: LN_FWD_FAST(3); break;
                        default: LN_FWD_FAST(4); }
     } else {
@@ -494,6 +611,7 @@
                        case 4: LN_FWD(4); break; default: LN_FWD(8); }
     }
 #undef LN_FWD_FAST
+#undef LN_FWD_FAST_F32
 #undef LN_FWD_FAST_MX
 #undef LN_FWD_FAST_
 #undef LN_FWD
@@ -508,7 +626,7 @@
 static int layernorm_bwd_impl(const void* dy, int dy_L, int dy_off, int dy_is_f32, const float* x, int x_L, int x_off,
                               const float* gamma, const float* mean, const float* rstd, const float* dres, float* dx,
                               void* dx_bf16, float* dgamma, float* dbeta, float* dcol, float* workspace, bool partial_only,
-                              int B, int n, int dim, void* stream) {
+                              int B, int n, int dim, void* stream, bool ends = false) {
     const int rows = B * n, nblk = ceil_div(rows, 4 * ROWS_PER_WAVE);
     const size_t lds = (size_t)4 * 3 * dim * sizeof(float);
     dim3 grid(nblk), block(256);
@@ -519,15 +637,26 @@
 #define LN_BWD_FAST(NV, DEPTH) hipLaunchKernelGGL((ln_bwd_fast_kernel<NV, DEPTH>), grid, block, lds, s, (const bf16_t*)dy, \
                                                   RowMap{dy_L, dy_off}, x, RowMap{x_L, x_off}, gamma, mean, rstd, dres, dx, \
                                                   (bf16_t*)dx_bf16, part, B, n)
+#define LN_BWD_END_(NV, DEPTH, F, R, X) hipLaunchKernelGGL((ln_bwd_fast_end_kernel<NV, DEPTH, F, R, X>), grid, block, lds, s, dy, \
+                                                           RowMap{dy_L, dy_off}, x, RowMap{x_L, x_off}, gamma, mean, rstd, dres, dx, \
+                                                           (bf16_t*)dx_bf16, part, B, n)
+#define LN_BWD_END(NV, DEPTH) do { switch ((dy_is_f32 ? 4 : 0) | (dres ? 2 : 0) | (dx_bf16 ? 1 : 0)) { \
+        case 0: LN_BWD_END_(NV, DEPTH, false, false, false); break; case 1: LN_BWD_END_(NV, DEPTH, false, false, true); break; \
+        case 2: LN_BWD_END_(NV, DEPTH, false, true, false); break;  case 4: LN_BWD_END_(NV, DEPTH, true, false, false); break; \
+        case 5: LN_BWD_END_(NV, DEPTH, true, false, true); break;   case 6: LN_BWD_END_(NV, DEPTH, true, true, false); break; \
+        case 7: LN_BWD_END_(NV, DEPTH, true, true, true); break;    default: LN_BWD_FAST(NV, DEPTH); } } while (0)
     const int nvs = ln_nv(dim);
-    if (MH_LN_FAST && nvs <= 4 && dim == 256 * nvs && !dy_is_f32 && dres && dx_bf16 && rows % ROWS_PER_WAVE == 0) {
+    const bool blocks_case = !dy_is_f32 && dres && dx_bf16;
+    if (MH_LN_FAST && nvs <= 4 && dim == 256 * nvs && (blocks_case || ends) && rows % ROWS_PER_WAVE == 0) {
         constexpr int DEPTH = LN_BWD_DEPTH < ROWS_PER_WAVE ? LN_BWD_DEPTH : ROWS_PER_WAVE, DEPTH4 = 2 < ROWS_PER_WAVE ? 2 : ROWS_PER_WAVE;
-        switch (nvs) { case 1: LN_BWD_FAST(1, DEPTH); break; case 2: LN_BWD_FAST(2, DEPTH); break;
-                       case 3: LN_BWD_FAST(3, DEPTH); break; default: LN_BWD_FAST(4, DEPTH4); }
+        switch (nvs) { case 1: LN_BWD_END(1, DEPTH); break; case 2: LN_BWD_END(2, DEPTH); break;
+                       case 3: LN_BWD_END(3, DEPTH); break; default: LN_BWD_END(4, DEPTH4); }
     } else {
         switch (nvs) { case 1: LN_BWD(1); break; case 2: LN_BWD(2); break; case 3: LN_BWD(3); break;
                        case 4: LN_BWD(4); break; default: LN_BWD(8); }
     }
+#undef LN_BWD_END
+#undef LN_BWD_END_
 #undef LN_BWD_FAST
 #undef LN_BWD
     if (dgamma && !partial_only)
@@ -561,6 +690,23 @@
                               nullptr, workspace, true, B, n, dim, stream);
 }
 
+extern "C" int mh_layernorm_fwd_ends(const float* x, int x_L, int x_off, const float* gamma, const float* beta, void* y, int y_L,
+                                     int y_off, int y_is_f32, float* mean, float* rstd, int B, int n, int dim, float eps,
+                                     void* stream) {
+    return layernorm_fwd_impl(x, x_L, x_off, gamma, beta, y, y_L, y_off, y_is_f32, mean, rstd, B, n, dim, eps, nullptr, nullptr,
+                              nullptr, stream, nullptr, 0, true);
+}
+
+extern "C" int mh_layernorm_bwd_partial_ends(const void* dy, int dy_L, int dy_off, int dy_is_f32, const float* x, int x_L, int x_off,
+                                             const float* gamma, const float* mean, const float* rstd, const float* dres, float* dx,
+                                             void* dx_bf16, float* workspace, int B, int n, int dim, void* stream) {
+    MH_CHECK_ARG(dy && x && gamma && mean && rstd && dx && workspace, "mh_layernorm_bwd_partial_ends: null pointer");
+    MH_CHECK_ARG(dim % 4 == 0 && dim >= 4 && dim <= 2048, "mh_layernorm_bwd_partial_ends: dim %d unsupported", dim);
+    MH_CHECK_ARG(B > 0 && n > 0 && x_off + n <= x_L && dy_off + n <= dy_L, "mh_layernorm_bwd_partial_ends: bad row map");
+    return layernorm_bwd_impl(dy, dy_L, dy_off, dy_is_f32, x, x_L, x_off, gamma, mean, rstd, dres, dx, dx_bf16, nullptr, nullptr,
+                              nullptr, workspace, true, B, n, dim, stream, true);
+}
+
 extern "C" int mh_colsum_batched(const MhColsumJob* jobs_device, int n_jobs, const uint64_t* blocks_device, int n_blocks,
                                  void* stream) {
     MH_CHECK_ARG(jobs_device && blocks_device && n_jobs > 0 && n_jobs < 65536 && n_blocks > 0, "mh_colsum_batched: bad arguments");
diff --git a/maestro_amd/engine.py b/maestro_amd/engine.py
--- a/maestro_amd/engine.py
+++ b/maestro_amd/engine.py
@@ -610,14 +610,18 @@
         items = [(st, lo, hi) for st, lo, hi in items if hi > lo]
         if not items:
             return
-        key = tuple((st.tag, lo, hi) for st, lo, hi in items)
+        key = (tuple((st.tag, lo, hi) for st, lo, hi in items), getattr(self, "_ends_on", False))
         table = self._wgrad_tables.get(key)
         if table is None:
             probs = [p for st, lo, hi in items for p in st.wgrad_problems(lo, hi)]
             jobs = [j for st, lo, hi in items for j in st.reduce_jobs(lo, hi)]
+            jobs += [j for st, lo, hi in items if hi == st.depth for j in self._end_reduce_jobs(st)]
             table = self._wgrad_tables[key] = (hip.GroupedTN(probs, self.device), hip.ColsumBatch(jobs, self.device))
         table[1].launch()
         table[0].launch()
+
+    def _end_reduce_jobs(self, st) -> list:
+        return []
 
     @contextlib.contextmanager
     def _tuning_pass(self, what: str):
@@ -716,6 +720,7 @@
         self.E, self.Dd = m.embed_dim, m.decoder_dim
         self._init_runtime(device, len(model.group_specs) - 1)
         self.wgrad_mode = os.environ.get("MAESTRO_WGRAD", "auto")
+        self.fused_ends = hip.fused_ends_default()
         if self.wgrad_mode not in ("auto", "fused", "deferred"):
             raise ValueError(f"MAESTRO_WGRAD={self.wgrad_mode!r}: expected auto, fused or deferred")
         self._wgrad_plans, self._zero_lists = {}, {}
@@ -880,6 +885,15 @@
         for g in self.groups:
             self.gb[g.name]["ln_ws"] = e(max(hip.layernorm_bwd_workspace(g.Beff * g.L, Dd),
                                              hip.layernorm_bwd_workspace(g.Beff * g.N, E)))
+        if self.fused_ends and not self.deterministic:
+            for g in self.groups:
+                self.gb[g.name]["ws_enc"] = e(max(1, hip.layernorm_bwd_workspace(g.Beff * g.N, E)))
+                if self.joint is not None:
+                    self.gb[g.name]["ws_joint"] = e(max(1, hip.layernorm_bwd_workspace(g.Beff * g.N, E)))
+            for name, s in self.mods.items():
+                self.mb[name]["ws_dec"] = e(max(1, hip.layernorm_bwd_workspace(s.Beff * s.n_tok, Dd)))
+                if s.G == 1 and s.K <= hip.LOSS_COLSUM_MAX_PPC:
+                    self.mb[name]["cs_rec"] = e(hip.masked_loss_partial_size(s.Beff, s.n_tok), s.K)
         self.loss_acc = z(1)
         srcs = {s.src: s for s in self.mods.values()}
         tot_w = sum(s.Dates * s.L for s in srcs.values())
@@ -1121,8 +1135,9 @@
             nrm = st.t.norm
             self._opt_wait("enc", max(st.depth - 1, 0))
             if self.joint is not None:
-                hip.layernorm_fwd(st.x_last, g.N, 0, nrm.weight, nrm.bias, self.joint.x0, m.joint_N, g.joint_off,
-                                  gbuf["mean_e"], gbuf["rstd_e"], g.Beff, g.N, E)
+                ln_fwd = hip.layernorm_fwd_ends if self.fused_ends and not self.deterministic else hip.layernorm_fwd
+                ln_fwd(st.x_last, g.N, 0, nrm.weight, nrm.bias, self.joint.x0, m.joint_N, g.joint_off,
+                       gbuf["mean_e"], gbuf["rstd_e"], g.Beff, g.N, E)
             else:
                 hip.layernorm_fwd(st.x_last, g.N, 0, nrm.weight, nrm.bias, gbuf["y_e2d" if self.e2d_identity else "henc"], g.N, 0,
                                   gbuf["mean_e"], gbuf["rstd_e"], g.Beff, g.N, E)
@@ -1180,8 +1195,8 @@
                         hip.masked_loss_bands_det(b["rec"], b["target"], gbuf["mask"], b["cnt"], self.loss_w[s.src], part,
                                                   b["drec"], s.Beff, s.n_tok, g.L, s.tok_off, s.K, self.p_loss, s.C_src, s.c0, s.C)
                 elif s.G == 1:
-                    hip.masked_loss(b["rec"], b["target"], gbuf["mask"], b["cnt"], self.loss_w[s.src], self.loss_acc,
-                                    b["drec"], s.Beff, s.n_tok, g.L, s.tok_off, s.K, self.p_loss)
+                    hip.masked_loss_v2(b["rec"], b["target"], gbuf["mask"], b["cnt"], self.loss_w[s.src], self.loss_acc,
+                                       b["drec"], b.get("cs_rec"), s.Beff, s.n_tok, g.L, s.tok_off, s.K, self.p_loss)
                 else:
                     hip.masked_loss_bands(b["rec"], b["target"], gbuf["mask"], b["cnt"], self.loss_w[s.src], self.loss_acc,
                                           b["drec"], s.Beff, s.n_tok, g.L, s.tok_off, s.K, self.p_loss, s.C_src, s.c0, s.C)
@@ -1308,6 +1323,10 @@
         key = getattr(self, "_cur_key", None)
         plan = self._plan = self._wgrad_plan()
         sfx = f":{plan}:{'h' if self.grad_hook is not None else 'n'}"
+        self._ends_on = (self.fused_ends and not self.deterministic and plan != "fused"
+                         and all(st.depth > 0 for st in self._all_stacks()))
+        if self._ends_on:
+            sfx += ":e"
         if not self._dw_conv_clear:
             sfx += ":nz"
         if self.fp8 is not None and self.fp8.dgrad:
@@ -1351,10 +1370,15 @@
                         self._grads_ready(m.embed_to_rec[s.embed])
                         continue
                     hip.gemm(hip.GEMM_TN, s.K, Dd, T, b["drec"], s.K, b["hdec"], Dd, ps.g(conv.weight).view(s.K, Dd), Dd, AT)
-                    hip.colsum(b["drec"], ps.g(conv.bias), T, s.K, s.K)
-                    hip.layernorm_bwd(b["dh"], s.n_tok, 0, st.x_last, g.L, s.tok_off, nrm.weight, b["mean_f"], b["rstd_f"],
-                                      None, dx, dx16, ps.g(nrm.weight), ps.g(nrm.bias), st.top_bias_grad(), gbuf["ln_ws"],
-                                      s.Beff, s.n_tok, Dd)
+                    if not (self._ends_on and "cs_rec" in b):
+                        hip.colsum(b["drec"], ps.g(conv.bias), T, s.K, s.K)
+                    if self._ends_on:
+                        hip.layernorm_bwd_partial(b["dh"], s.n_tok, 0, st.x_last, g.L, s.tok_off, nrm.weight, b["mean_f"],
+                                                       b["rstd_f"], None, dx, dx16, b["ws_dec"], s.Beff, s.n_tok, Dd)
+                    else:
+                        hip.layernorm_bwd(b["dh"], s.n_tok, 0, st.x_last, g.L, s.tok_off, nrm.weight, b["mean_f"], b["rstd_f"],
+                                          None, dx, dx16, ps.g(nrm.weight), ps.g(nrm.bias), st.top_bias_grad(), gbuf["ln_ws"],
+                                          s.Beff, s.n_tok, Dd)
                     self._grads_ready(m.embed_to_rec[s.embed])
                 dx0, _ = st.backward(dx, defer=self._plan in ("all", "enc", "ovl"))
                 side_post(g, gbuf, st, dx0)
@@ -1362,7 +1386,9 @@
 
         def side_post(g, gbuf, st, dx0):
             self._grads_ready(st.t.norm)
-            hip.gather_rows(dx0, gbuf["vis"], gbuf["dy_e2d"], g.Beff, g.L, g.N, Dd, g.N, 0)
+            cast_in_gather = self._ends_on and not self.e2d_identity
+            hip.gather_rows_v2(dx0, gbuf["vis"], gbuf["dy_e2d"], gbuf["dy_e2d16"] if cast_in_gather else None, g.Beff, g.L, g.N, Dd,
+                               g.N, 0)
             for s in g.mods:
                 if self.deterministic:
                     per_sample = self.tie_order == "torch"
@@ -1388,7 +1414,8 @@
             M = g.Beff * g.N
             lin = m.enc_to_dec[g.model]
             if not self.e2d_identity:
-                hip.cast_bf16(gbuf["dy_e2d"], gbuf["dy_e2d16"], M * Dd)
+                if not cast_in_gather:
+                    hip.cast_bf16(gbuf["dy_e2d"], gbuf["dy_e2d16"], M * Dd)
                 hip.gemm(hip.GEMM_NN, M, E, Dd, gbuf["dy_e2d16"], Dd, ps.h(lin.weight), E, gbuf["dhenc"], E)
                 if self.deterministic:
                     self._det_linear_grads(("e2d", g.name), gbuf["dy_e2d16"], gbuf["henc"], Dd, E, M, ps.g(lin.weight), ps.g(lin.bias))
@@ -1403,6 +1430,9 @@
                 if self.deterministic:
                     self._det_layernorm_bwd(("ln_joint", g.name), dy, g.N, 0, jt.x_last, m.joint_N, g.joint_off, jn, gbuf["mean_j"],
                                             gbuf["rstd_j"], jt.dxa, jt.top16, jt.top_bias_grad(), g.Beff, g.N, E)
+                elif self._ends_on:
+                    hip.layernorm_bwd_partial(dy, g.N, 0, jt.x_last, m.joint_N, g.joint_off, jn.weight, gbuf["mean_j"],
+                                                   gbuf["rstd_j"], None, jt.dxa, jt.top16, gbuf["ws_joint"], g.Beff, g.N, E)
                 else:
                     hip.layernorm_bwd(dy, g.N, 0, jt.x_last, m.joint_N, g.joint_off, jn.weight, gbuf["mean_j"],
                                       gbuf["rstd_j"], None, jt.dxa, jt.top16, ps.g(jn.weight), ps.g(jn.bias),
@@ -1411,6 +1441,28 @@
         self._run_parallel([side(g) for g in self.groups])
         if self._plan == "enc":
             self._launch_wgrads([(st, 0, st.depth) for st in self.dec.values()])
+
+    def _end_reduce_jobs(self, st) -> list:
+        if not self._ends_on:
+            return []
+        ps, m, E, Dd, jobs = self.store, self.model, self.E, self.Dd, []
+        nrm = st.t.norm
+        for g in self.groups:
+            gbuf = self.gb[g.name]
+            if st is self.dec[g.name]:
+                for s in g.mods:
+                    b = self.mb[s.name]
+                    rows = hip.layernorm_bwd_workspace(s.Beff * s.n_tok, Dd) // (3 * Dd)
+                    jobs += hip.layernorm_partial_jobs(b["ws_dec"], rows, Dd, ps.g(nrm.weight), ps.g(nrm.bias), st.top_bias_grad())
+                    if "cs_rec" in b:
+                        conv = m.embed_to_rec[s.embed].pixelify_bands[s.gi].conv
+                        jobs.append((b["cs_rec"].view(-1), ps.g(conv.bias), b["cs_rec"].shape[0], s.K, s.K))
+            rows = hip.layernorm_bwd_workspace(g.Beff * g.N, E) // (3 * E)
+            if st is self.enc[g.name]:
+                jobs += hip.layernorm_partial_jobs(gbuf["ws_enc"], rows, E, ps.g(nrm.weight), ps.g(nrm.bias), st.top_bias_grad())
+            if st is self.joint:
+                jobs += hip.layernorm_partial_jobs(gbuf["ws_joint"], rows, E, ps.g(nrm.weight), ps.g(nrm.bias), st.top_bias_grad())
+        return jobs
 
     def _bwd_joint(self) -> None:
         jt = self.joint
@@ -1432,6 +1484,13 @@
                                         (gbuf["dy_e2d" if self.e2d_identity else "dhenc"], g.N, 0))
                     self._det_layernorm_bwd(("ln_enc", g.name), dy, dy_L, dy_off, st.x_last, g.N, 0, nrm, gbuf["mean_e"], gbuf["rstd_e"],
                                             st.dxa, st.top16, st.top_bias_grad(), g.Beff, g.N, E)
+                    self._grads_ready(nrm)
+                    self._enc_state[g.name] = (st.dxa, st.top16)
+                elif first and self._ends_on:
+                    dy, dy_L, dy_off = ((self._djoint, m.joint_N, g.joint_off) if self.joint is not None else
+                                        (gbuf["dy_e2d" if self.e2d_identity else "dhenc"], g.N, 0))
+                    hip.layernorm_bwd_partial(dy, dy_L, dy_off, st.x_last, g.N, 0, nrm.weight, gbuf["mean_e"], gbuf["rstd_e"], None,
+                                                   st.dxa, st.top16, gbuf["ws_enc"], g.Beff, g.N, E)
                     self._grads_ready(nrm)
                     self._enc_state[g.name] = (st.dxa, st.top16)
                 elif first:
diff --git a/maestro_amd/hip.py b/maestro_amd/hip.py
--- a/maestro_amd/hip.py
+++ b/maestro_amd/hip.py
@@ -354,6 +354,41 @@
     _hbm_call(f"ln_bwd<{dim}>", float(B) * n * dim * (_esz(dy) + 4 + _esz(dres) + 4 + _esz(dx_bf16)), "mh_layernorm_bwd_partial", dy,
               _I(dy_L), _I(dy_off), _I(1 if dy.dtype == torch.float32 else 0), x, _I(x_L), _I(x_off), gamma, mean, rstd, dres, dx,
               dx_bf16, workspace, _I(B), _I(n), _I(dim))
+
+
+def fused_ends_default() -> bool:
+    return os.environ.get("MAESTRO_FUSED_ENDS", "1") != "0"
+
+
+def layernorm_fwd_ends(x, x_L, x_off, gamma, beta, y, y_L, y_off, mean, rstd, B, n, dim, eps=1e-5):
+    _hbm_call(f"ln_fwd<{dim}>", float(B) * n * dim * (4 + _esz(y)), "mh_layernorm_fwd_ends", x, _I(x_L), _I(x_off), gamma, beta, y,
+              _I(y_L), _I(y_off), _I(1 if y.dtype == torch.float32 else 0), mean, rstd, _I(B), _I(n), _I(dim), _F(eps))
+
+
+def layernorm_bwd_partial_ends(dy, dy_L, dy_off, x, x_L, x_off, gamma, mean, rstd, dres, dx, dx_bf16, workspace, B, n, dim):
+    _hbm_call(f"ln_bwd<{dim}>", float(B) * n * dim * (_esz(dy) + 4 + _esz(dres) + 4 + _esz(dx_bf16)), "mh_layernorm_bwd_partial_ends",
+              dy, _I(dy_L), _I(dy_off), _I(1 if dy.dtype == torch.float32 else 0), x, _I(x_L), _I(x_off), gamma, mean, rstd, dres,
+              dx, dx_bf16, workspace, _I(B), _I(n), _I(dim))
+
+
+def layernorm_partial_jobs(workspace, rows, dim, dgamma, dbeta, dcol=None) -> list:
+    flat = workspace.view(-1)
+    jobs = [(flat, dgamma, rows, dim, 3 * dim), (flat[dim:], dbeta, rows, dim, 3 * dim)]
+    if dcol is not None:
+        jobs.append((flat[2 * dim:], dcol, rows, dim, 3 * dim))
+    return jobs
+
+
+LOSS_COLSUM_MAX_PPC = 1024
+
+
+def masked_loss_v2(rec, target, mask_group, n_masked, weight, acc, drec, colsum_partial, B, Lm, Lgroup, tok_off, PPC, p):
+    _hbm_call("masked_loss", float(B) * Lm * (PPC * (_esz(rec) + 4 + _esz(drec)) + 1), "mh_masked_loss_v2", rec, target, mask_group,
+              n_masked, _F(weight), acc, drec, colsum_partial, _I(B), _I(Lm), _I(Lgroup), _I(tok_off), _I(PPC), _I(p))
+
+
+def gather_rows_v2(src, idx, dst, dst_bf16, B, src_L, n_idx, dim, dst_L, dst_off):
+    call("mh_gather_rows_v2", src, idx, dst, dst_bf16, _I(B), _I(src_L), _I(n_idx), _I(dim), _I(dst_L), _I(dst_off))
 
 
 COLSUM_ROWS = 16
```
